# PoloWlg/Joint-Multimodal-Transformer-6th-ABAW

Measured on AMD Instinct MI355X. Metric: train windows/sec + CCC parity, B=64 T=300 A/V fusion, 1/2/4/8 MI355X, higher is better.
Workload: dtype bf16; 1 GPU; configs[2]: FcLayer(1024,512) + Two_transformers(TRANSFORMER,FC,H=1,L=1,vision_in_ft=2048) + 2x CCCLoss + SGD-nesterov; global_batch=64, per_gpu_batch=64, seq_len=300, D_a=1024, D_v=2048, parallelism=dp1

## Files before the change

### include/jmt.h

```cpp
#ifndef JMT_H_
#define JMT_H_

#include <stddef.h>
#include <stdint.h>

#ifdef __cplusplus
extern "C" {
#endif

#define JMT_ABI_VERSION 7

enum { JMT_F32 = 0, JMT_BF16 = 1, JMT_F16 = 2 };
enum { JMT_OK = 0, JMT_ERR_ARG = -1, JMT_ERR_HIP = -2, JMT_ERR_UNSUPPORTED = -3 };

int jmt_abi_version(void);
const char* jmt_last_error(void);
int jmt_kernel_count(void);
long long jmt_bounds_violations(int reset);

typedef struct jmt_gemm_desc {
  int ab_dtype, c_dtype, aux_dtype;
  int M, N, K;
  const void* a[8];
  const void* b[8];
// ... 65 lines not shown
                              void* stream);
int jmt_layernorm_bwd_grouped(int dt_in, int dt_dy, int dt_dx, int G, int64_t rows, int D,
                              const void* x, int64_t ldx, int64_t sx, const void* r, int64_t ldr,
                              int64_t sr, const void* dy, int64_t lddy, int64_t sdy,
                              const float* mean, const float* rstd, const float* const* gamma,
                              void* dx, int64_t lddx, int64_t sdx, float* const* dgamma,
                              float* const* dbeta, float* const* dsum, int beta_acc,
                              float* partials, void* stream);
int jmt_layernorm_bwd_grouped_blocks(int64_t rows);

int jmt_softmax_fwd(int p_dt, int64_t rows, int n, const float* s, int64_t lds, float scale,
                    void* p, int64_t ldp, void* stream);
int jmt_softmax_bwd(int p_dt, int ds_dt, int64_t rows, int n, const void* p, int64_t ldp,
                    const float* dp, int64_t lddp, float scale, void* ds, int64_t ldds,
                    void* stream);

int jmt_attn_supported(int dt, int dh);
int jmt_attn_fwd(int dt, int N, int H, int Lq, int Lk, int dh, const void* q, int64_t sq_l,
                 int64_t sq_n, const void* k, int64_t sk_l, int64_t sk_n, const void* v,
                 int64_t sv_l, int64_t sv_n, void* o, int64_t so_l, int64_t so_n, float scale,
                 float* lse, void* stream);
int jmt_attn_bwd(int dt, int N, int H, int Lq, int Lk, int dh, const void* go, int64_t sgo_l,
                 int64_t sgo_n, const void* o, int64_t so_l, int64_t so_n, const void* q,
                 int64_t sq_l, int64_t sq_n, const void* k, int64_t sk_l, int64_t sk_n,
                 const void* v, int64_t sv_l, int64_t sv_n, const float* lse, void* p_out,
                 void* ds_out, int64_t ldp, void* dq, int64_t sdq_l, int64_t sdq_n, float scale,
                 void* stream);

int jmt_attn_dkdv_plan(int Lq, int Lk, int H, int64_t sdk_l, int64_t sdv_l, int64_t sdq_l,
                       int has_dq);
int jmt_attn_dkdv(int dt, int N, int H, int Lq, int Lk, int dh, const void* p, const void* ds,
                  int64_t ldp, const void* go, int64_t sgo_l, int64_t sgo_n, const void* q,
                  int64_t sq_l, int64_t sq_n, const void* k, int64_t sk_l, int64_t sk_n, void* dk,
                  int64_t sdk_l, int64_t sdk_n, void* dv, int64_t sdv_l, int64_t sdv_n, void* dq,
                  int64_t sdq_l, int64_t sdq_n, void* stream);

int jmt_attn_fwd_sq(int dt, int N, int H, int Lq, int Lk, int dh, const void* q, int64_t sq_l,
                    int64_t sq_n, const void* k, int64_t sk_l, int64_t sk_n, const void* v,
                    int64_t sv_l, int64_t sv_n, void* o, int64_t so_l, int64_t so_n, float scale,
                    float* lse, int spp, const int* qtab, int npair, void* stream);
int jmt_attn_bwd_sq(int dt, int N, int H, int Lq, int Lk, int dh, const void* go, int64_t sgo_l,
                    int64_t sgo_n, const void* o, int64_t so_l, int64_t so_n, const void* q,
                    int64_t sq_l, int64_t sq_n, const void* k, int64_t sk_l, int64_t sk_n,
                    const void* v, int64_t sv_l, int64_t sv_n, const float* lse, void* p_out,
                    void* ds_out, int64_t ldp, float scale, int spp, const int* qtab, int npair,
                    void* stream);
int jmt_attn_dkdv_sq(int dt, int N, int H, int Lq, int Lk, int dh, const void* p, const void* ds,
                     int64_t ldp, const void* go, int64_t sgo_l, int64_t sgo_n, const void* q,
                     int64_t sq_l, int64_t sq_n, const void* k, int64_t sk_l, int64_t sk_n,
                     void* dk, int64_t sdk_l, int64_t sdk_n, void* dv, int64_t sdv_l,
                     int64_t sdv_n, void* dq, int64_t sdq_l, int64_t sdq_n, int spp,
                     const int* qtab, int npair, int merge_dq, void* stream);

int jmt_attn_fwd_rows_ok(int N, int H, int Lq, int Lk, int64_t sk_l, int64_t sv_l);
int jmt_attn_bwd_pds_ok(int N, int H, int Lq, int Lk, int64_t ldp, int64_t sk_l, int64_t sv_l);
int jmt_attn_dkdv_ok(int N, int H, int Lq, int Lk, int64_t ldp, int64_t sgo_l, int64_t sq_l,
                     int64_t sk_l, int64_t sdk_l, int64_t sdv_l, int64_t sdq_l, int has_dq);

int jmt_attn_short_supported(int dt, int dh, int Lq, int Lk);
int jmt_attn_short_fwd(int dt, int N, int H, int Lq, int Lk, int dh, const void* q, int64_t sq_l,
                       int64_t sq_n, const void* k, int64_t sk_l, int64_t sk_n, const void* v,
                       int64_t sv_l, int64_t sv_n, void* o, int64_t so_l, int64_t so_n,
                       float scale, float* lse, void* stream);
int jmt_attn_short_bwd(int dt, int N, int H, int Lq, int Lk, int dh, const void* go,
                       int64_t sgo_l, int64_t sgo_n, const void* o, int64_t so_l, int64_t so_n,
                       const void* q, int64_t sq_l, int64_t sq_n, const void* k, int64_t sk_l,
                       int64_t sk_n, const void* v, int64_t sv_l, int64_t sv_n, const float* lse,
                       void* dq, int64_t sdq_l, int64_t sdq_n, void* dk, int64_t sdk_l,
                       int64_t sdk_n, void* dv, int64_t sdv_l, int64_t sdv_n, float scale,
                       void* stream);

int jmt_small_attn_fwd(int dt, int N, int H, int Lq, int Lk, int E, const void* q, int64_t sq_l,
                       int64_t sq_n, const void* k, int64_t sk_l, int64_t sk_n, const void* v,
                       int64_t sv_l, int64_t sv_n, void* o, int64_t so_l, int64_t so_n,
                       float scale, float* p_out, void* stream);
int jmt_small_attn_bwd(int dt, int N, int H, int Lq, int Lk, int E, const void* go,
                       int64_t sgo_l, int64_t sgo_n, const void* q, int64_t sq_l, int64_t sq_n,
                       const void* k, int64_t sk_l, int64_t sk_n, const void* v, int64_t sv_l,
                       int64_t sv_n, const float* p, void* dq, int64_t sdq_l, int64_t sdq_n,
                       void* dk, int64_t sdk_l, int64_t sdk_n, void* dv, int64_t sdv_l,
                       int64_t sdv_n, float scale, void* stream);

int jmt_colsum_blocks(int64_t rows);
int jmt_colsum(int dt, int64_t rows, int N, const void* dy, int64_t ld, float* db, int beta_acc,
               float* partials, void* stream);
int jmt_colsum_grouped(int dt, int G, int64_t rows, int N, const void* dy, int64_t ld,
                       int64_t sdy, float* const* db_tab, int beta_acc, float* partials,
                       void* stream);

int jmt_noop(void* stream);

int jmt_copy2d(int src_dt, int dst_dt, int64_t rows, int64_t cols, const void* src,
               int64_t src_rs, int64_t src_cs, void* dst, int64_t dst_rs, int64_t dst_cs,
               int accumulate, void* stream);

int jmt_head_fwd(int h_dt, int y_dt, int64_t rows, int hid, int k, const void* h, int64_t ldh,
                 const void* w2_0, const void* w2_1, const float* b2_0, const float* b2_1,
                 void* y_0, void* y_1, int64_t ldy, void* stream);
int jmt_head_bwd(int h_dt, int gy_dt, int64_t rows, int hid, int k, const void* h, int64_t ldh,
                 const void* w2_0, const void* w2_1, const void* gy_0, const void* gy_1,
                 int64_t ldgy, void* dh, int64_t lddh, float* dw2_0, float* dw2_1, float* db2_0,
                 float* db2_1, float* partials, void* stream);
size_t jmt_head_bwd_workspace_bytes(int64_t rows);

int jmt_dropout_next(uint32_t* state, uint32_t* out, void* stream);
int jmt_dropout(int dt, const void* x, int64_t ldx, void* y, int64_t ldy, int64_t rows,
// ... 81 lines not shown
```

### joint-multimodal-transformer-6th-abaw_amd/csrc/abi_check.cpp

```cpp
#include <stdio.h>
#include <string.h>

#include "../../include/jmt.h"

static int g_fail = 0;

static void expect_msg(const char* what, const char* needle) {
  const char* e = jmt_last_error();
  if (!e || !strstr(e, needle)) {
    fprintf(stderr, "FAIL %s: err='%s' lacks '%s'\n", what, e ? e : "(null)", needle);
    ++g_fail;
  }
}

static void expect_err(const char* what, int rc) {
  const char* e = jmt_last_error();
  const size_t n = e ? strnlen(e, 1024) : 0;
  if (rc >= 0 || n == 0 || n >= 512) {
    fprintf(stderr, "FAIL %s: rc=%d err='%s'\n", what, rc, e ? e : "(null)");
    ++g_fail;
  }
}

static void expect_eq(const char* what, int got, int want) {
// ... 322 lines not shown
  }
  {
    const int id2[2] = {0, 1}, fwd[2] = {1, 1}, chain[3] = {0, 0, 1}, three[3] = {0, 0, 0};
    const int big[9] = {0, 1, 2, 3, 4, 5, 6, 7, 8};
    expect_err("attn_fwd_sq fp32", jmt_attn_fwd_sq(JMT_F32, 2, 1, 300, 300, 512, algn, 512, 512,
                                                   algn, 512, 512, algn, 512, 512, algn, 512, 512,
                                                   0.1f, fnull, 1, id2, 2, nullptr));
    expect_err("attn_fwd_sq Lq 64", jmt_attn_fwd_sq(JMT_BF16, 2, 1, 64, 300, 512, algn, 512, 512,
                                                    algn, 512, 512, algn, 512, 512, algn, 512,
                                                    512, 0.1f, fnull, 1, id2, 2, nullptr));
    expect_err("attn_fwd_sq null table", jmt_attn_fwd_sq(JMT_BF16, 2, 1, 300, 300, 512, algn, 512,
                                                         512, algn, 512, 512, algn, 512, 512,
                                                         algn, 512, 512, 0.1f, fnull, 1, nullptr,
                                                         2, nullptr));
    expect_err("attn_fwd_sq N != npair spp", jmt_attn_fwd_sq(JMT_BF16, 3, 1, 300, 300, 512, algn,
                                                             512, 512, algn, 512, 512, algn, 512,
                                                             512, algn, 512, 512, 0.1f, fnull, 1,
                                                             id2, 2, nullptr));
    expect_err("attn_fwd_sq 9 pairs", jmt_attn_fwd_sq(JMT_BF16, 9, 1, 300, 300, 512, algn, 512,
                                                      512, algn, 512, 512, algn, 512, 512, algn,
                                                      512, 512, 0.1f, fnull, 1, big, 9, nullptr));
    expect_err("attn_fwd_sq forward source", jmt_attn_fwd_sq(JMT_BF16, 2, 1, 300, 300, 512, algn,
                                                             512, 512, algn, 512, 512, algn, 512,
                                                             512, algn, 512, 512, 0.1f, fnull, 1,
                                                             fwd, 2, nullptr));
    expect_err("attn_bwd_sq chained source", jmt_attn_bwd_sq(JMT_BF16, 3, 1, 300, 300, 512, algn,
                                                             512, 512, algn, 512, 512, algn, 512,
                                                             512, algn, 512, 512, algn, 512, 512,
                                                             fnull, algn, algn, 384, 0.1f, 1,
                                                             chain, 3, nullptr));
    expect_err("attn_bwd_sq ldp", jmt_attn_bwd_sq(JMT_BF16, 2, 1, 300, 300, 512, algn, 512, 512,
                                                  algn, 512, 512, algn, 512, 512, algn, 512, 512,
                                                  algn, 512, 512, fnull, algn, algn, 300, 0.1f, 1,
                                                  id2, 2, nullptr));
    expect_err("attn_dkdv_sq dq null", jmt_attn_dkdv_sq(JMT_BF16, 2, 1, 300, 300, 512, algn, algn,
                                                        384, algn, 512, 512, algn, 512, 512, algn,
                                                        512, 512, algn, 512, 512, algn, 512, 512,
                                                        nullptr, 0, 0, 1, id2, 2, 0, nullptr));
    expect_err("attn_dkdv_sq spp 0", jmt_attn_dkdv_sq(JMT_BF16, 2, 1, 300, 300, 512, algn, algn,
                                                      384, algn, 512, 512, algn, 512, 512, algn,
                                                      512, 512, algn, 512, 512, algn, 512, 512,
                                                      algn, 512, 512, 0, id2, 2, 0, nullptr));
    expect_err("attn_dkdv_sq merge 3 uses", jmt_attn_dkdv_sq(JMT_BF16, 3, 1, 300, 300, 512, algn,
                                                             algn, 384, algn, 512, 512, algn, 512,
                                                             512, algn, 512, 512, algn, 512, 512,
                                                             algn, 512, 512, algn, 512, 512, 1,
                                                             three, 3, 1, nullptr));
    expect_err("attn_dkdv_sq merge 1 use", jmt_attn_dkdv_sq(JMT_BF16, 2, 1, 300, 300, 512, algn,
                                                            algn, 384, algn, 512, 512, algn, 512,
                                                            512, algn, 512, 512, algn, 512, 512,
                                                            algn, 512, 512, algn, 512, 512, 1, id2,
                                                            2, 1, nullptr));
  }
  expect_err("small_attn_fwd null", jmt_small_attn_fwd(JMT_BF16, 4, 1, 6, 6, 512, nullptr, 512,
                                                       512, nullptr, 512, 512, nullptr, 512, 512,
                                                       nullptr, 512, 512, 0.1f, fnull, nullptr));

  expect_err("ccc_stats kind", jmt_ccc_stats(3, JMT_F32, 10, 1, misal, fnull, 0.f, -1.f, 1.f,
                                             nullptr, nullptr));
  expect_err("ccc_stats bins", jmt_ccc_stats(0, JMT_F32, 10, 100, misal, fnull, 0.f, -1.f, 1.f,
                                             (double*)buf, nullptr));
  expect_err("ccc_finish null", jmt_ccc_finish(0, 0, nullptr, 1, 1e-8f, fnull, nullptr, nullptr));
  expect_err("ccc_finish_add null", jmt_ccc_finish_add(0, 1, nullptr, 1, 1e-8f, fnull, fnull,
                                                       nullptr, nullptr));
  expect_err("ce_stats bins", jmt_ce_stats(JMT_F32, 10, 1, misal, fnull, -1.f, 1.f, fnull,
                                           (double*)buf, nullptr));
  expect_err("ce_bwd null", jmt_ce_bwd(JMT_F32, 10, 5, nullptr, fnull, -1.f, 1.f, fnull, nullptr,
                                       fnull, nullptr, nullptr));
  expect_err("ce_labels null", jmt_ce_labels(10, 5, fnull, -1.f, 1.f, nullptr, nullptr));
  expect_err("mask_indices null", jmt_mask_indices(10, fnull, -5.f, nullptr, nullptr, nullptr));

  expect_err("sgd null", jmt_sgd_step(10, fnull, fnull, fnull, 0.1f, 0.9f, 0.f, 0.f, 1, 1, 1.f,
                                      nullptr, JMT_BF16, nullptr));
  expect_err("sgd_zero null", jmt_sgd_step_zero(10, fnull, nullptr, fnull, 0.1f, 0.9f, 0.f, 0.f,
                                                1, 1, 1.f, nullptr, JMT_BF16, nullptr));
  expect_err("sgd_amp_zero null", jmt_sgd_step_amp_zero(10, fnull, fnull, fnull, 0.1f, 0.9f,
                                                        0.f, 0.f, 1, 1, nullptr, nullptr,
                                                        JMT_BF16, nullptr));
  float* fal = (float*)algn;
  expect_err("opt_tick null state", jmt_opt_tick(nullptr, 0.9, 0.999, nullptr, nullptr));
  expect_msg("opt_tick null state", "null state");
  expect_err("opt_tick beta", jmt_opt_tick(fal, 1.0, 0.999, nullptr, nullptr));
  expect_err("adam null param", jmt_adam_step(10, fnull, fal, fal, fal, nullptr, fal, 0.9, 0.999,
                                              1e-8f, 0.f, 1.f, nullptr, 0, nullptr, JMT_BF16,
                                              nullptr));
  expect_msg("adam null param", "null pointer");
  expect_err("adam null moments", jmt_adam_step(10, fal, fal, fnull, fnull, nullptr, fal, 0.9,
                                                0.999, 1e-8f, 0.f, 1.f, nullptr, 0, nullptr,
                                                JMT_BF16, nullptr));
  expect_err("adam null state", jmt_adam_step(10, fal, fal, fal, fal, nullptr, nullptr, 0.9,
                                              0.999, 1e-8f, 0.f, 1.f, nullptr, 0, nullptr,
                                              JMT_BF16, nullptr));
  expect_msg("adam null state", "null state");
  expect_err("adam amsgrad null state", jmt_adam_step(10, fal, fal, fal, fal, fal, nullptr, 0.9,
                                                      0.999, 1e-8f, 0.f, 1.f, nullptr, 1, nullptr,
                                                      JMT_BF16, nullptr));
  expect_msg("adam amsgrad null state", "null state");
  expect_err("adam misaligned param", jmt_adam_step(10, (float*)(buf + 4), fal, fal, fal, nullptr,
                                                    fal, 0.9, 0.999, 1e-8f, 0.f, 1.f, nullptr, 0,
                                                    nullptr, JMT_BF16, nullptr));
  expect_msg("adam misaligned param", "16-B aligned");
  expect_err("adam shadow_dt", jmt_adam_step(10, fal, fal, fal, fal, nullptr, fal, 0.9, 0.999,
                                             1e-8f, 0.f, 1.f, nullptr, 0, algn, JMT_F32, nullptr));
  expect_msg("adam shadow_dt", "shadow_dt");
  expect_err("adam misaligned shadow", jmt_adam_step(10, fal, fal, fal, fal, nullptr, fal, 0.9,
                                                     0.999, 1e-8f, 0.f, 1.f, nullptr, 0,
// ... 124 lines not shown
```

### joint-multimodal-transformer-6th-abaw_amd/csrc/attn.hip

```cpp
#include "attn_common.h"

namespace jmt {

constexpr int AT_QT = 64;
constexpr int AF_KT = 64;
constexpr int AB_KT = 32;
constexpr int AT_XCH = 4096;
constexpr int AF_LDS = 2 * AF_KT * AT_ROWB + 8 * AT_XCH;
constexpr int AB_LDS = 4 * AB_KT * AT_ROWB + 8 * AT_XCH;

struct AttnFwdArgs {
  const void* q;
  const void* k;
  const void* v;
  void* o;
  float* lse;
  int64_t sq_l, sq_n, sk_l, sk_n, sv_l, sv_n, so_l, so_n;
  int Lq, Lk, H, nitems;
  float scale_log2;
  uint64_t* stamps;
  QShare qs;
};

template <bool STAMP>
__device__ __forceinline__ void stamp(uint64_t* buf, int idx) {
  if constexpr (STAMP) {
    if (buf && blockIdx.x == gridDim.x / 2 && ((threadIdx.x >> 6) & 3) == 0) {
      const uint64_t t = __builtin_amdgcn_s_memtime();
      buf[((threadIdx.x >> 8) * 256 + idx) * 64 + (threadIdx.x & 63)] = t;
    }
  }
}

template <typename T, bool STAMP = false, int OPT = 0>
__global__ __launch_bounds__(512, 2) void attn_fwd_kernel(AttnFwdArgs p) {
  typedef typename Frag16<T>::t F;
  typedef typename Frag16<T>::h Hf;
  extern __shared__ __attribute__((aligned(16))) char smem[];
  char* kimg = smem;
  char* vimg = smem + AF_KT * AT_ROWB;
  char* xch = smem + 2 * AF_KT * AT_ROWB;

  const int lane = threadIdx.x & 63, w = threadIdx.x >> 6;
  const int g = lane >> 4, li = lane & 15, rg = w & 3, h = w >> 2;
  const int nqt = (p.Lq + AT_QT - 1) / AT_QT;
  const int nkt = (p.Lk + AF_KT - 1) / AF_KT;
  int item, iend, istride;
  item_range(p.nitems, item, iend, istride);
  if (item >= iend) return;
  if constexpr ((OPT & 2) != 0)
    if (__builtin_amdgcn_readfirstlane(threadIdx.x >> 6) >= 4) __builtin_amdgcn_s_setprio(1);

  int nh = item / nqt, n = nh / p.H, hd = nh % p.H, q0 = (item % nqt) * AT_QT;
  const T* kb = (const T*)p.k + (int64_t)n * p.sk_n + hd * AT_DH;
  const T* vb = (const T*)p.v + (int64_t)n * p.sv_n + hd * AT_DH;

  F qf[8];
  auto load_q = [&](int n_, int hd_, int q0_) {
    const T* qrow = (const T*)p.q + (int64_t)n_ * p.sq_n + hd_ * AT_DH +
                    (int64_t)min(q0_ + 16 * rg + li, p.Lq - 1) * p.sq_l + 256 * h + 8 * g;
#pragma unroll
    for (int ks = 0; ks < 8; ++ks) qf[ks] = *(const F*)(qrow + 32 * ks);
  };
  load_q(n, hd, q0);
  stage_rows<T, AF_KT, 8, true>(kimg, kb, p.sk_l, 0, p.Lk);
  stage_rows<T, AF_KT, 8, true>(vimg, vb, p.sv_l, 0, p.Lk);

  f32x4* xmine = (f32x4*)(xch + w * AT_XCH) + lane;
  const f32x4* xpart = (const f32x4*)(xch + (w ^ 4) * AT_XCH) + lane;
  int kb4[4], tb8[8];
#pragma unroll
  for (int m = 0; m < 4; ++m) kb4[m] = row_base(m, li, g, h);
#pragma unroll
  for (int c = 0; c < 8; ++c) tb8[c] = tr_base(c, li, g, h);
// ... 382 lines not shown
          else *(uint2*)(prow_ds + key) = *(const uint2*)ds4;
        }
      }
      if constexpr ((OPT & 16) != 0) pend_on = true;
      {
        F fa[4], fb[4];
        auto kbatch = [&](F* dst, int b) {
#pragma unroll
          for (int i = 0; i < 4; ++i) {
            const int t = 4 * b + i;
            const char* a = kimg + tb8[t & 7] + 256 * (t >> 3);
            const Hf lo = tr_read<Hf>(a);
            const Hf hi = tr_read<Hf>(a + 16384);
            dst[i] = __builtin_shufflevector(lo, hi, 0, 1, 2, 3, 4, 5, 6, 7);
          }
        };
        kbatch(fa, 0);
#pragma unroll
        for (int b = 0; b < 4; b += 2) {
          kbatch(fb, b + 1);
          __builtin_amdgcn_sched_barrier(0);
#pragma unroll
          for (int i = 0; i < 4; ++i) acc[4 * b + i] = mfma16(fa[i], dsf, acc[4 * b + i]);
          __builtin_amdgcn_sched_barrier(0);
          if (b + 2 < 4) kbatch(fa, b + 2);
          __builtin_amdgcn_sched_barrier(0);
#pragma unroll
          for (int i = 0; i < 4; ++i) acc[4 * b + 4 + i] = mfma16(fb[i], dsf, acc[4 * b + 4 + i]);
          __builtin_amdgcn_sched_barrier(0);
        }
      }
      if (j + 1 < nkt) {
        wait_vmcnt<0>();
        lds_barrier();
      }
      buf ^= 1;
    }
    if constexpr ((OPT & 16) != 0) flush();
    store_acc_direct<T>(acc, 1.f,
                        (T*)p.dq + (int64_t)n * p.sdq_n + hd * AT_DH + (int64_t)qr * p.sdq_l +
                            256 * h,
                        qr < p.Lq);
    if (!more) break;
    load_o(n2, hd2, q02);
    lds_barrier();
    item = nxt; nh = nh2; n = n2; hd = hd2; q0 = q02; kb = kb2; vb = vb2;
  }
}

constexpr int AP_QT = 128;
constexpr int AP_KT = 32;
constexpr int AP_LDS = 4 * AP_KT * AT_ROWB;

template <typename T, int DBG = 0, bool SQ = false>
__global__ __launch_bounds__(512, 2) void attn_bwd_pds_kernel(AttnBwdArgs p) {
  int tcount = 0;
  auto st = [&](int phase) {
    if constexpr ((DBG & 64) != 0) {
      if (tcount < 31) stamp<true>((uint64_t*)p.dq, 8 * tcount + phase);
    }
  };
  typedef typename Frag16<T>::t F;
  typedef unsigned u32x4 __attribute__((ext_vector_type(4)));
  extern __shared__ __attribute__((aligned(16))) char smem[];
  constexpr int IMG = AP_KT * AT_ROWB;

  const int lane = threadIdx.x & 63, w = threadIdx.x >> 6;
  const int g = lane >> 4, li = lane & 15;
  const int nqt = (p.Lq + AP_QT - 1) / AP_QT;
  const int nkt = (p.Lk + AP_KT - 1) / AP_KT;
  int item, iend, istride;
  item_range(p.nitems, item, iend, istride);
  if (item >= iend) return;

  int nh = item / nqt, n = nh / p.H, hd = nh % p.H, q0 = (item % nqt) * AP_QT;
  const T* kb = (const T*)p.k + (int64_t)n * p.sk_n + hd * AT_DH;
  const T* vb = (const T*)p.v + (int64_t)n * p.sv_n + hd * AT_DH;

  F qf[16], df[16], of[16];
  auto load_qd = [&](int n_, int hd_, int q0_) {
    const int64_t qc_ = min(q0_ + 16 * w + li, p.Lq - 1), coff = (int64_t)hd_ * AT_DH + 8 * g;
    const T* qrow = (const T*)p.q + (int64_t)q_seq<SQ>(p.qs, n_) * p.sq_n + qc_ * p.sq_l + coff;
    const T* drow = (const T*)p.go + (int64_t)n_ * p.sgo_n + qc_ * p.sgo_l + coff;
#pragma unroll
    for (int ks = 0; ks < 16; ++ks) {
      qf[ks] = *(const F*)(qrow + 32 * ks);
      df[ks] = *(const F*)(drow + 32 * ks);
    }
  };
  auto load_o = [&](int n_, int hd_, int q0_) {
    const int64_t qc_ = min(q0_ + 16 * w + li, p.Lq - 1), coff = (int64_t)hd_ * AT_DH + 8 * g;
    const T* orow = (const T*)p.o + (int64_t)n_ * p.so_n + qc_ * p.so_l + coff;
#pragma unroll
    for (int ks = 0; ks < 16; ++ks) of[ks] = *(const F*)(orow + 32 * ks);
  };
  load_qd(n, hd, q0);
  load_o(n, hd, q0);
  int buf = 0;
  const int wu = __builtin_amdgcn_readfirstlane(w);
  const uint32_t lbase = (uint32_t)(uintptr_t)(__attribute__((address_space(3))) char*)smem;
  unsigned loff[4];
#pragma unroll
  for (int i = 0; i < 4; ++i) loff[i] = (unsigned)(lane ^ (((4 * wu + i) & 7) << 1)) << 4;
  const int ldk = (int)(p.sk_l * (int64_t)sizeof(T)), ldv = (int)(p.sv_l * (int64_t)sizeof(T));
  auto stage_tile = [&](int b, const T* kbase, const T* vbase, int k0) {
#pragma unroll
    for (int i = 0; i < 4; ++i) {
      const int r = 4 * wu + i;
      const int src = min(k0 + r, p.Lk - 1);
      const uint32_t dst = lbase + b * 2 * IMG + r * AT_ROWB;
      glds16_at((const char*)kbase + (unsigned)(src * ldk) + loff[i], dst);
      glds16_at((const char*)vbase + (unsigned)(src * ldv) + loff[i], dst + IMG);
    }
  };
  stage_tile(0, kb, vb, 0);

  int kb4[4];
#pragma unroll
  for (int m = 0; m < 4; ++m) kb4[m] = row_base(m, li, g, 0);

  while (true) {
    const int qr = q0 + 16 * w + li;
    const int qc = min(qr, p.Lq - 1);
    const bool wact = __builtin_amdgcn_readfirstlane(q0 + 16 * w) < p.Lq;
    const int nxt = item + istride;
    const bool more = nxt < iend;
    const int nh2 = nxt / nqt, n2 = nh2 / p.H, hd2 = nh2 % p.H, q02 = (nxt % nqt) * AP_QT;
    const T* kb2 = (const T*)p.k + (int64_t)n2 * p.sk_n + hd2 * AT_DH;
    const T* vb2 = (const T*)p.v + (int64_t)n2 * p.sv_n + hd2 * AT_DH;

    float delta;
    {
      float dp = 0.f;
#pragma unroll
      for (int ks = 0; ks < 16; ++ks)
#pragma unroll
        for (int e = 0; e < 8; ++e) dp += (float)of[ks][e] * (float)df[ks][e];
      delta = pl_pair_sum(dp);
    }
    const float lse2 = p.lse[(int64_t)nh * p.Lq + qc] * 1.4426950408889634f;
    const int64_t region = (int64_t)nh * p.Lq * p.ldp;
    const int nbytes = (int)((int64_t)p.Lq * p.ldp * (int64_t)sizeof(T));
    auto mk_rsrc = [&](void* base) {
      const uint64_t ba = (uint64_t)(uintptr_t)((T*)base + region);
      const uint32_t lo = __builtin_amdgcn_readfirstlane((uint32_t)ba);
      const uint32_t hi = __builtin_amdgcn_readfirstlane((uint32_t)(ba >> 32));
      return __builtin_amdgcn_make_buffer_rsrc((void*)(((uint64_t)hi << 32) | lo), 0,
                                               __builtin_amdgcn_readfirstlane(nbytes), 0x00020000);
    };
    const auto rs_p = mk_rsrc(p.pbuf);
    const auto rs_ds = mk_rsrc(p.dsbuf);
    const int rowoff = qr * AP_KT;

    wait_vmcnt<0>();
    lds_barrier();
    auto tile = [&](int j, auto last_c) {
      constexpr bool LAST = decltype(last_c)::value;
      st(0);
      const char* kimg = smem + buf * 2 * IMG;
      const char* vimg = kimg + IMG;
      if ((DBG & 8) == 0 && (!LAST || more))
        stage_tile(buf ^ 1, LAST ? kb2 : kb, LAST ? vb2 : vb, LAST ? 0 : AP_KT * (j + 1));
      st(1);
      f32x4 s[2], d[2];
#pragma unroll
      for (int kt = 0; kt < 2; ++kt) {
        s[kt] = f32x4{0.f, 0.f, 0.f, 0.f};
        d[kt] = f32x4{0.f, 0.f, 0.f, 0.f};
      }
      if ((DBG & 2) == 0 && wact) {
        F fa[4], fb[4];
        auto batch = [&](F* dst, int ks) {
#pragma unroll
          for (int kt = 0; kt < 2; ++kt) {
            const int o = kb4[ks & 3] + 256 * (ks >> 2) + 16384 * kt;
            dst[kt] = *(const F*)(kimg + o);
            dst[2 + kt] = *(const F*)(vimg + o);
          }
        };
        batch(fa, 0);
#pragma unroll
        for (int ks = 0; ks < 16; ks += 2) {
          batch(fb, ks + 1);
          __builtin_amdgcn_sched_barrier(0);
#pragma unroll
          for (int kt = 0; kt < 2; ++kt) {
            s[kt] = mfma16(fa[kt], qf[ks], s[kt]);
            d[kt] = mfma16(fa[2 + kt], df[ks], d[kt]);
          }
          __builtin_amdgcn_sched_barrier(0);
          if (ks + 2 < 16) batch(fa, ks + 2);
          __builtin_amdgcn_sched_barrier(0);
#pragma unroll
          for (int kt = 0; kt < 2; ++kt) {
            s[kt] = mfma16(fb[kt], qf[ks + 1], s[kt]);
            d[kt] = mfma16(fb[2 + kt], df[ks + 1], d[kt]);
          }
          __builtin_amdgcn_sched_barrier(0);
        }
      }
      st(2);
      if constexpr (LAST && (DBG & 1) == 0) {
        if (more) load_qd(n2, hd2, q02);
      }
      if ((DBG & 4) == 0 && wact) {
        const int kbase = AP_KT * j + 4 * g;
        uint32_t pk[2][2][2];
#pragma unroll
        for (int kt = 0; kt < 2; ++kt) {
          T pv4[4], ds4[4];
#pragma unroll
          for (int r = 0; r < 4; ++r) {
            const bool in = kbase + 16 * kt + r < p.Lk;
            const float pv = in ? __builtin_amdgcn_exp2f(s[kt][r] * p.scale_log2 - lse2) : 0.f;
            pv4[r] = from_f<T>(pv);
            ds4[r] = from_f<T>(p.scale * pv * (d[kt][r] - delta));
          }
#pragma unroll
          for (int q = 0; q < 2; ++q) {
            pk[0][kt][q] = ((const uint32_t*)pv4)[q];
            pk[1][kt][q] = ((const uint32_t*)ds4)[q];
          }
        }
        const int off = qr < p.Lq ? (rowoff + j * p.Lq * AP_KT + 16 * (g & 1) + 8 * (g >> 1)) *
                                        (int)sizeof(T)
                                  : 0x7ffffff0;
        JMT_DCHECK(AP_KT * j + AP_KT <= p.ldp);
#pragma unroll
        for (int a = 0; a < 2; ++a) {
          const auto r0 = __builtin_amdgcn_permlane16_swap(pk[a][0][0], pk[a][1][0], false, false);
          const auto r1 = __builtin_amdgcn_permlane16_swap(pk[a][0][1], pk[a][1][1], false, false);
          const u32x4 v = {r0[0], r1[0], r0[1], r1[1]};
          if constexpr ((DBG & 16) != 0) {
            asm volatile("" ::"v"(v[0]), "v"(v[1]), "v"(v[2]), "v"(v[3]));
          } else {
            __builtin_amdgcn_raw_buffer_store_b128(v, a == 0 ? rs_p : rs_ds, off, 0,
                                                   (DBG & 32) ? 2 : 0);
          }
        }
      }
      st(3);
      if constexpr (!LAST) {
        if ((DBG & 20) == 0 && wact) wait_vmcnt<2>();
        else wait_vmcnt<0>();
        st(4);
        lds_barrier();
        st(5);
      }
      ++tcount;
      buf ^= 1;
    };
    for (int j = 0; j + 1 < nkt; ++j) tile(j, std::false_type{});
    tile(nkt - 1, std::true_type{});
    if (!more) break;
    if constexpr ((DBG & 1) == 0) load_o(n2, hd2, q02);
    item = nxt; nh = nh2; n = n2; hd = hd2; q0 = q02; kb = kb2; vb = vb2;
  }
}

constexpr int AR_QT = 128;
constexpr int AR_KT = 32;
constexpr int AR_LDS = 4 * AR_KT * AT_ROWB;
constexpr int AR_VB = 4;

template <typename T, int DBG = 0, bool SQ = false>
__global__ __launch_bounds__(512, 2) void attn_fwd_rows_kernel(AttnFwdArgs p) {
  typedef typename Frag16<T>::t F;
  typedef typename Frag16<T>::h Hf;
  extern __shared__ __attribute__((aligned(16))) char smem[];
  constexpr int IMG = AR_KT * AT_ROWB;

  const int lane = threadIdx.x & 63, w = threadIdx.x >> 6;
  const int g = lane >> 4, li = lane & 15;
  const int nqt = (p.Lq + AR_QT - 1) / AR_QT;
  const int nkt = (p.Lk + AR_KT - 1) / AR_KT;
  int item, iend, istride;
  item_range(p.nitems, item, iend, istride);
  if (item >= iend) return;

  int nh = item / nqt, n = nh / p.H, hd = nh % p.H, q0 = (item % nqt) * AR_QT;
  const T* kb = (const T*)p.k + (int64_t)n * p.sk_n + hd * AT_DH;
  const T* vb = (const T*)p.v + (int64_t)n * p.sv_n + hd * AT_DH;

  F qf[16];
  auto load_q = [&](int n_, int hd_, int q0_) {
    const T* qrow = (const T*)p.q + (int64_t)q_seq<SQ>(p.qs, n_) * p.sq_n + hd_ * AT_DH +
                    (int64_t)min(q0_ + 16 * w + li, p.Lq - 1) * p.sq_l + 8 * g;
#pragma unroll
    for (int ks = 0; ks < 16; ++ks) qf[ks] = *(const F*)(qrow + 32 * ks);
  };
  load_q(n, hd, q0);
  int buf = 0;
  const int wu = __builtin_amdgcn_readfirstlane(w);
  const uint32_t lbase = (uint32_t)(uintptr_t)(__attribute__((address_space(3))) char*)smem;
  unsigned loff[4];
#pragma unroll
  for (int i = 0; i < 4; ++i) loff[i] = (unsigned)(lane ^ (((4 * wu + i) & 7) << 1)) << 4;
  const int ldk = (int)(p.sk_l * (int64_t)sizeof(T)), ldv = (int)(p.sv_l * (int64_t)sizeof(T));
  auto stage_tile = [&](int b, const T* kbase, const T* vbase, int k0) {
#pragma unroll
    for (int i = 0; i < 4; ++i) {
      const int r = 4 * wu + i;
      const int src = min(k0 + r, p.Lk - 1);
      JMT_DCHECK(src >= 0 && src < p.Lk);
      const uint32_t dst = lbase + b * 2 * IMG + r * AT_ROWB;
      glds16_sv((const char*)kbase + (unsigned)(src * ldk), loff[i], dst);
      glds16_sv((const char*)vbase + (unsigned)(src * ldv), loff[i], dst + IMG);
    }
  };
  stage_tile(0, kb, vb, 0);
  const int kb0 = row_base(0, li, g, 0), tb0 = tr_base(0, li, g, 0);
  auto lane_base = [](int base, int bits) __attribute__((always_inline)) {
#if !defined(__OPTIMIZE__)
    return base ^ bits;
#else
    int r;
    asm volatile("v_xor_b32 %0, %2, %1" : "=v"(r) : "v"(base), "i"(bits));
    return r;
#endif
  };

  while (true) {
    const int qr = q0 + 16 * w + li;
    const bool wact = __builtin_amdgcn_readfirstlane(q0 + 16 * w) < p.Lq;
    const int nxt = item + istride;
    const bool more = nxt < iend;
    const int nh2 = nxt / nqt, n2 = nh2 / p.H, hd2 = nh2 % p.H, q02 = (nxt % nqt) * AR_QT;
    const T* kb2 = (const T*)p.k + (int64_t)n2 * p.sk_n + hd2 * AT_DH;
    const T* vb2 = (const T*)p.v + (int64_t)n2 * p.sv_n + hd2 * AT_DH;

    f32x4 o[32];
#pragma unroll
    for (int t = 0; t < 32; ++t) o[t] = f32x4{0.f, 0.f, 0.f, 0.f};
    float m_run = -INFINITY, l_run = 0.f;

    wait_vmcnt<0>();
#pragma unroll
    for (int ks = 0; ks < 16; ++ks) asm volatile("" : "+v"(qf[ks]));
    lds_barrier();
    auto tile = [&](int j, auto last_c) {
      constexpr bool LAST = decltype(last_c)::value;
      const char* kimg = smem + buf * 2 * IMG;
      const char* vimg = kimg + IMG;
      if ((!LAST && (DBG & 8) == 0) || (LAST && more))
        stage_tile(buf ^ 1, LAST ? kb2 : kb, LAST ? vb2 : vb, LAST ? 0 : AR_KT * (j + 1));
      f32x4 sl[2], sh[2];
#pragma unroll
      for (int kt = 0; kt < 2; ++kt) {
        sl[kt] = f32x4{0.f, 0.f, 0.f, 0.f};
        sh[kt] = f32x4{0.f, 0.f, 0.f, 0.f};
      }
      if ((DBG & 2) == 0 && wact) {
        F fa[2], fb[2];
        auto batch = [&](F* dst, const char* a) {
#pragma unroll
          for (int kt = 0; kt < 2; ++kt) dst[kt] = *(const F*)(a + 16384 * kt);
        };
        const char* a = kimg + lane_base(kb0, 0);
        batch(fa, a);
#pragma unroll
        for (int ks = 0; ks < 8; ++ks) {
          batch(fb, a + 512);
          __builtin_amdgcn_sched_barrier(0);
#pragma unroll
          for (int kt = 0; kt < 2; ++kt) sl[kt] = mfma16(fa[kt], qf[ks], sl[kt]);
          __builtin_amdgcn_sched_barrier(0);
          if (ks + 1 < 8) {
            a = kimg + lane_base(kb0, ((ks + 1) & 3) << 6) + 256 * ((ks + 1) >> 2);
            batch(fa, a);
          }
          __builtin_amdgcn_sched_barrier(0);
#pragma unroll
          for (int kt = 0; kt < 2; ++kt) sh[kt] = mfma16(fb[kt], qf[ks + 8], sh[kt]);
          __builtin_amdgcn_sched_barrier(0);
        }
      }
      if constexpr (LAST) {
        if (more) load_q(n2, hd2, q02);
      }
      if (wact) {
        F pf;
        if constexpr ((DBG & 4) != 0) {
#pragma unroll
          for (int e = 0; e < 8; ++e) pf[e] = from_f<T>(0.f);
#pragma unroll
          for (int kt = 0; kt < 2; ++kt)
            asm volatile("" ::"v"(sl[kt][0]), "v"(sl[kt][3]), "v"(sh[kt][0]), "v"(sh[kt][3]));
        } else {
        const int kbase = AR_KT * j + 4 * g;
        float mx = -INFINITY;
#pragma unroll
        for (int kt = 0; kt < 2; ++kt) {
          const f32x4 full = sl[kt] + sh[kt];
#pragma unroll
          for (int r = 0; r < 4; ++r) {
            const float x = (kbase + 16 * kt + r < p.Lk) ? full[r] * p.scale_log2 : -INFINITY;
// ... 124 lines not shown
    if (hipGetDevice(&dev) != hipSuccess ||
        hipDeviceGetAttribute(&v, hipDeviceAttributeMultiprocessorCount, dev) != hipSuccess || v < 8)
      v = 8;
    ncu = v / 8 * 8;
    const char* e = getenv("JMT_ATTN_PERSIST");
    if (e && e[0] == '0') ncu = 1 << 30;
  }
  return (unsigned)(nitems > ncu ? ncu : nitems);
}

extern "C" int jmt_attn_set_stamps(void* buf) {
#if JMT_DIAG
  g_stamps = buf;
  return JMT_OK;
#else
  return buf ? set_error(JMT_ERR_UNSUPPORTED, "jmt_attn_set_stamps: diagnostic build only "
                                              "(make diag)") : JMT_OK;
#endif
}

static int g_fwd_rows = -1;
static bool fwd_rows_on() {
  static const bool env_on = [] {
    const char* e = getenv("JMT_ATTN_FWD_ROWS");
    return !(e && e[0] == '0');
  }();
  return g_fwd_rows < 0 ? env_on : g_fwd_rows != 0;
}
extern "C" int jmt_attn_set_fwd_rows(int on) {
  g_fwd_rows = on < 0 ? -1 : (on != 0);
  return JMT_OK;
}

extern "C" int jmt_attn_supported(int dt, int dh) {
  return (dt == JMT_BF16 || dt == JMT_F16) && dh == AT_DH;
}

static bool fwd_rows(int Lq, int Lk, int64_t sk_l, int64_t sv_l) {
  return fwd_rows_on() && Lq > AT_QT && rows_fit(Lk, sk_l) && rows_fit(Lk, sv_l);
}

extern "C" int jmt_attn_fwd_rows_ok(int N, int H, int Lq, int Lk, int64_t sk_l, int64_t sv_l) {
  return fwd_rows(Lq, Lk, sk_l, sv_l) && sizes_ok(N, H, Lq, Lk, AR_QT);
}

extern "C" int jmt_attn_bwd_pds_ok(int N, int H, int Lq, int Lk, int64_t ldp, int64_t sk_l,
                                   int64_t sv_l) {
  return pds_range(N, H, Lq, Lk, ldp, sk_l, sv_l) == nullptr;
}

static int attn_fwd_impl(int dt, int N, int H, int Lq, int Lk, int dh, const void* q,
                         int64_t sq_l, int64_t sq_n, const void* k, int64_t sk_l, int64_t sk_n,
                         const void* v, int64_t sv_l, int64_t sv_n, void* o, int64_t so_l,
                         int64_t so_n, float scale, float* lse, const QShare* qs, void* stream) {
  if (N == 0 || Lq == 0) return JMT_OK;
  if (!jmt_attn_supported(dt, dh))
    return set_error(JMT_ERR_UNSUPPORTED, "jmt_attn_fwd: dtype %d / head dim %d not supported",
                     dt, dh);
  const void* ptrs[] = {q, k, v, o};
  const int64_t strides[] = {sq_l, sq_n, sk_l, sk_n, sv_l, sv_n, so_l, so_n};
  const bool rows = fwd_rows(Lq, Lk, sk_l, sv_l);
  if (qs && !rows)
    return set_error(JMT_ERR_UNSUPPORTED, "jmt_attn_fwd_sq: the whole-row kernel only (Lq > %d, "
                                          "Lk K / V rows below 2 GiB, JMT_ATTN_FWD_ROWS on)",
                     AT_QT);
  const int qt = rows ? AR_QT : AT_QT;
  int rc = check_common("jmt_attn_fwd", N, H, Lq, Lk, qt, ptrs, 4, strides, 8);
  if (rc != JMT_OK) return rc;
  AttnFwdArgs a = {};
  if (qs) a.qs = *qs;
  a.q = q; a.k = k; a.v = v; a.o = o; a.lse = lse;
  a.sq_l = sq_l; a.sq_n = sq_n; a.sk_l = sk_l; a.sk_n = sk_n; a.sv_l = sv_l; a.sv_n = sv_n;
  a.so_l = so_l; a.so_n = so_n;
  a.Lq = Lq; a.Lk = Lk; a.H = H;
  a.scale_log2 = scale * 1.4426950408889634f;
  hipStream_t st = as_stream(stream);
  a.nitems = ((Lq + qt - 1) / qt) * N * H;
  const dim3 grid(persistent_grid(a.nitems));
  const char* name = qs ? "jmt_attn_fwd_sq" : "jmt_attn_fwd";
#if JMT_DIAG
  static const int dbg =
      getenv("JMT_ATTN_FWD_ROWS_DBG") ? atoi(getenv("JMT_ATTN_FWD_ROWS_DBG")) : 0;
  if (rows && dbg && dt == JMT_BF16) {
#define JMT_ROWS_DBG(D) \
  case D: attn_launch<attn_fwd_rows_kernel<__bf16, D>, AR_LDS>(grid, st, a); break;
    switch (dbg) {
      JMT_ROWS_DBG(2) JMT_ROWS_DBG(4) JMT_ROWS_DBG(8) JMT_ROWS_DBG(16) JMT_ROWS_DBG(32)
      JMT_ROWS_DBG(18) JMT_ROWS_DBG(22) JMT_ROWS_DBG(54) JMT_ROWS_DBG(62)
      default: return set_error(JMT_ERR_ARG, "JMT_ATTN_FWD_ROWS_DBG=%d not built", dbg);
    }
#undef JMT_ROWS_DBG
    JMT_LAUNCH_CHECK("jmt_attn_fwd");
    return JMT_OK;
  }
  if (!rows && g_stamps && dt == JMT_BF16) {
    a.stamps = (uint64_t*)g_stamps;
    attn_launch<attn_fwd_kernel<__bf16, true, ATTN_FWD_OPT>, AF_LDS>(grid, st, a);
    JMT_LAUNCH_CHECK("jmt_attn_fwd");
    return JMT_OK;
  }
#endif
  by_elem(dt, [&](auto e) {
    using T = typename decltype(e)::type;
    if (!rows) attn_launch<attn_fwd_kernel<T, false, ATTN_FWD_OPT>, AF_LDS>(grid, st, a);
    else if (qs) attn_launch<attn_fwd_rows_kernel<T, 0, true>, AR_LDS>(grid, st, a);
    else attn_launch<attn_fwd_rows_kernel<T>, AR_LDS>(grid, st, a);
  });
  JMT_LAUNCH_CHECK(name);
  return JMT_OK;
}

extern "C" int jmt_attn_fwd(int dt, int N, int H, int Lq, int Lk, int dh, const void* q,
                            int64_t sq_l, int64_t sq_n, const void* k, int64_t sk_l, int64_t sk_n,
                            const void* v, int64_t sv_l, int64_t sv_n, void* o, int64_t so_l,
                            int64_t so_n, float scale, float* lse, void* stream) {
  return attn_fwd_impl(dt, N, H, Lq, Lk, dh, q, sq_l, sq_n, k, sk_l, sk_n, v, sv_l, sv_n, o, so_l,
                       so_n, scale, lse, nullptr, stream);
}

extern "C" int jmt_attn_fwd_sq(int dt, int N, int H, int Lq, int Lk, int dh, const void* q,
                               int64_t sq_l, int64_t sq_n, const void* k, int64_t sk_l,
                               int64_t sk_n, const void* v, int64_t sv_l, int64_t sv_n, void* o,
                               int64_t so_l, int64_t so_n, float scale, float* lse, int spp,
                               const int* qtab, int npair, void* stream) {
  if (N == 0 || Lq == 0) return JMT_OK;
  if (!jmt_attn_supported(dt, dh))
    return set_error(JMT_ERR_UNSUPPORTED, "jmt_attn_fwd_sq: dtype %d / head dim %d not supported",
                     dt, dh);
  QShare qs = {};
  int rc = qshare_pack("jmt_attn_fwd_sq", N, spp, qtab, npair, &qs);
  if (rc != JMT_OK) return rc;
  return attn_fwd_impl(dt, N, H, Lq, Lk, dh, q, sq_l, sq_n, k, sk_l, sk_n, v, sv_l, sv_n, o, so_l,
                       so_n, scale, lse, &qs, stream);
}

static int attn_bwd_impl(int dt, int N, int H, int Lq, int Lk, int dh, const void* go,
                         int64_t sgo_l, int64_t sgo_n, const void* o, int64_t so_l, int64_t so_n,
                         const void* q, int64_t sq_l, int64_t sq_n, const void* k, int64_t sk_l,
                         int64_t sk_n, const void* v, int64_t sv_l, int64_t sv_n,
                         const float* lse, void* p_out, void* ds_out, int64_t ldp, void* dq,
                         int64_t sdq_l, int64_t sdq_n, float scale, const QShare* qs,
                         void* stream) {
  if (N == 0 || Lq == 0) return JMT_OK;
  if (!jmt_attn_supported(dt, dh))
    return set_error(JMT_ERR_UNSUPPORTED, "jmt_attn_bwd: dtype %d / head dim %d not supported",
                     dt, dh);
  const void* ptrs[] = {go, o, q, k, v, p_out, ds_out, dq};
  const int64_t strides[] = {sgo_l, sgo_n, so_l, so_n, sq_l, sq_n, sk_l, sk_n, sv_l, sv_n, ldp,
                             sdq_l, sdq_n};
  const bool pds = dq == nullptr;
  const int qt = pds ? AP_QT : AT_QT;
  int rc = check_common("jmt_attn_bwd", N, H, Lq, Lk, qt, ptrs, pds ? 7 : 8, strides,
                        pds ? 11 : 13);
  if (rc != JMT_OK) return rc;
  JMT_CHECK_ARG(lse && ldp >= Lk, "jmt_attn_bwd: lse missing or ldp < Lk");
  if (pds) {
    const char* why = pds_range(N, H, Lq, Lk, ldp, sk_l, sv_l);
    JMT_CHECK_ARG(!why, "jmt_attn_bwd (dq = NULL): %s", why);
  }
  AttnBwdArgs a = {};
  if (qs) a.qs = *qs;
  a.go = go; a.o = o; a.q = q; a.k = k; a.v = v; a.lse = lse;
  a.pbuf = p_out; a.dsbuf = ds_out; a.dq = dq;
  a.sgo_l = sgo_l; a.sgo_n = sgo_n; a.so_l = so_l; a.so_n = so_n; a.sq_l = sq_l; a.sq_n = sq_n;
  a.sk_l = sk_l; a.sk_n = sk_n; a.sv_l = sv_l; a.sv_n = sv_n;
  if (!pds) { a.sdq_l = sdq_l; a.sdq_n = sdq_n; }
  a.ldp = ldp;
  a.Lq = Lq; a.Lk = Lk; a.H = H;
  a.scale = scale;
  a.scale_log2 = scale * 1.4426950408889634f;
  a.nitems = ((Lq + qt - 1) / qt) * N * H;
  const dim3 grid(persistent_grid(a.nitems));
  hipStream_t st = as_stream(stream);
  const char* name = qs ? "jmt_attn_bwd_sq" : "jmt_attn_bwd";
#if JMT_DIAG
  static const int dbg = getenv("JMT_ATTN_PDS_DBG") ? atoi(getenv("JMT_ATTN_PDS_DBG")) : 0;
  if (pds && dbg && dt == JMT_BF16) {
    if (dbg & 64) a.dq = g_stamps;
#define JMT_PDS_DBG(D) \
  case D: attn_launch<attn_bwd_pds_kernel<__bf16, D>, AP_LDS>(grid, st, a); break;
    switch (dbg) {
      JMT_PDS_DBG(1) JMT_PDS_DBG(2) JMT_PDS_DBG(3) JMT_PDS_DBG(4) JMT_PDS_DBG(6)
      JMT_PDS_DBG(7) JMT_PDS_DBG(8) JMT_PDS_DBG(15) JMT_PDS_DBG(16) JMT_PDS_DBG(32)
      JMT_PDS_DBG(17) JMT_PDS_DBG(18) JMT_PDS_DBG(64)
      default: return set_error(JMT_ERR_ARG, "JMT_ATTN_PDS_DBG=%d not built", dbg);
    }
#undef JMT_PDS_DBG
    JMT_LAUNCH_CHECK("jmt_attn_bwd");
    return JMT_OK;
  }
#endif
  by_elem(dt, [&](auto e) {
    using T = typename decltype(e)::type;
    if (!pds) attn_launch<attn_bwd_kernel<T, ATTN_BWD_OPT>, AB_LDS>(grid, st, a);
    else if (qs) attn_launch<attn_bwd_pds_kernel<T, 0, true>, AP_LDS>(grid, st, a);
    else attn_launch<attn_bwd_pds_kernel<T>, AP_LDS>(grid, st, a);
  });
  JMT_LAUNCH_CHECK(name);
  return JMT_OK;
}

extern "C" int jmt_attn_bwd(int dt, int N, int H, int Lq, int Lk, int dh, const void* go,
                            int64_t sgo_l, int64_t sgo_n, const void* o, int64_t so_l,
                            int64_t so_n, const void* q, int64_t sq_l, int64_t sq_n,
                            const void* k, int64_t sk_l, int64_t sk_n, const void* v,
                            int64_t sv_l, int64_t sv_n, const float* lse, void* p_out,
                            void* ds_out, int64_t ldp, void* dq, int64_t sdq_l, int64_t sdq_n,
                            float scale, void* stream) {
  return attn_bwd_impl(dt, N, H, Lq, Lk, dh, go, sgo_l, sgo_n, o, so_l, so_n, q, sq_l, sq_n, k,
                       sk_l, sk_n, v, sv_l, sv_n, lse, p_out, ds_out, ldp, dq, sdq_l, sdq_n, scale,
                       nullptr, stream);
}

extern "C" int jmt_attn_bwd_sq(int dt, int N, int H, int Lq, int Lk, int dh, const void* go,
                               int64_t sgo_l, int64_t sgo_n, const void* o, int64_t so_l,
                               int64_t so_n, const void* q, int64_t sq_l, int64_t sq_n,
                               const void* k, int64_t sk_l, int64_t sk_n, const void* v,
                               int64_t sv_l, int64_t sv_n, const float* lse, void* p_out,
                               void* ds_out, int64_t ldp, float scale, int spp, const int* qtab,
                               int npair, void* stream) {
  if (N == 0 || Lq == 0) return JMT_OK;
  if (!jmt_attn_supported(dt, dh))
    return set_error(JMT_ERR_UNSUPPORTED, "jmt_attn_bwd_sq: dtype %d / head dim %d not supported",
                     dt, dh);
  QShare qs = {};
  int rc = qshare_pack("jmt_attn_bwd_sq", N, spp, qtab, npair, &qs);
  if (rc != JMT_OK) return rc;
  return attn_bwd_impl(dt, N, H, Lq, Lk, dh, go, sgo_l, sgo_n, o, so_l, so_n, q, sq_l, sq_n, k,
                       sk_l, sk_n, v, sv_l, sv_n, lse, p_out, ds_out, ldp, nullptr, 0, 0, scale,
                       &qs, stream);
}
```

### joint-multimodal-transformer-6th-abaw_amd/csrc/attn_common.h

```cpp
#pragma once
#include "common.h"

namespace jmt {

constexpr int AT_DH = 512;
constexpr int AT_ROWB = 1024;

struct QShare {
  int spp;
  uint32_t tab;
};
template <bool SQ>
__device__ __forceinline__ int q_seq(const QShare& s, int n) {
  if constexpr (!SQ) return n;
  const int p = n / s.spp;
  return (int)((s.tab >> (4 * p)) & 15u) * s.spp + (n - p * s.spp);
}

static inline int qshare_pack(const char* name, int N, int spp, const int* tab, int npair,
                              QShare* out) {
  JMT_CHECK_ARG(tab != nullptr && spp > 0 && npair >= 1 && npair <= 8 &&
                    (int64_t)spp * npair == N,
                "%s: query table needs 1-8 pairs of spp sequences with npair * spp == N", name);
  uint32_t bits = 0;
  for (int p = 0; p < npair; ++p) {
    JMT_CHECK_ARG(tab[p] >= 0 && tab[p] <= p && tab[tab[p]] == tab[p],
                  "%s: query table entry %d (%d) is not an earlier first use", name, p, tab[p]);
    bits |= (uint32_t)tab[p] << (4 * p);
  }
  out->spp = spp;
  out->tab = bits;
  return JMT_OK;
}

template <auto K, int LDS, int BLOCK = 512, typename A>
static void attn_launch(dim3 grid, hipStream_t st, const A& a) {
  static bool once = ((void)hipFuncSetAttribute((const void*)K,
                                                hipFuncAttributeMaxDynamicSharedMemorySize, LDS),
                      true);
  (void)once;
  hipLaunchKernelGGL(K, grid, dim3(BLOCK), (size_t)LDS, st, a);
}
template <typename T>
struct Elem {
  using type = T;
};
template <typename F>
static void by_elem(int dt, F f) {
  if (dt == JMT_BF16) f(Elem<__bf16>{});
  else f(Elem<_Float16>{});
}

struct AttnBwdArgs {
  const void* go;
  const void* o;
  const void* q;
  const void* k;
  const void* v;
  const float* lse;
  void* pbuf;
  void* dsbuf;
  void* dq;
  int64_t sgo_l, sgo_n, so_l, so_n, sq_l, sq_n, sk_l, sk_n, sv_l, sv_n, sdq_l, sdq_n, ldp;
  int Lq, Lk, H, nitems;
  float scale, scale_log2;
  QShare qs;
};

__device__ __forceinline__ int img_off(int row, int b) {
  return row * AT_ROWB + ((((b >> 4) ^ ((row & 7) << 1))) << 4) + (b & 15);
}
__device__ __forceinline__ int row_base(int m, int li, int g, int h) {
  return li * AT_ROWB + ((((4 * m + g) ^ ((li & 7) << 1))) << 4) + 512 * h;
}
__device__ __forceinline__ int tr_base(int c, int li, int g, int h) {
  const int r = 4 * g + (li >> 2);
  return r * AT_ROWB + ((((2 * c + ((li & 3) >> 1)) ^ ((r & 7) << 1))) << 4) + 8 * (li & 1) +
         512 * h;
}

__device__ __forceinline__ void lds_barrier() {
  asm volatile("s_waitcnt lgkmcnt(0)" ::: "memory");
  __builtin_amdgcn_s_barrier();
}

template <typename T, int R, int NW = 8, bool ASM = false>
__device__ __forceinline__ void stage_rows(char* img, const T* base, int64_t ld, int k0, int Lk) {
  constexpr int NI = R / NW;
  const int lane = threadIdx.x & 63;
  const int wu = __builtin_amdgcn_readfirstlane(threadIdx.x >> 6);
#pragma unroll
  for (int i = 0; i < NI; ++i) {
    const int r = wu * NI + i;
    const int src = min(k0 + r, Lk - 1);
    JMT_DCHECK(src >= 0 && src < Lk);
    const char* row = (const char*)(base + (int64_t)src * ld);
    const unsigned off = (unsigned)(lane ^ ((r & 7) << 1)) << 4;
    if constexpr (ASM) glds16_asm(row + off, img + r * AT_ROWB);
    else glds16(row + off, img + r * AT_ROWB);
  }
}

template <typename T, int R, int NW = 8, bool ASM = false>
__device__ __forceinline__ void stage_rows_part(char* img, const T* base, int64_t ld, int k0,
                                                int Lk, int i0, int i1) {
  constexpr int NI = R / NW;
  const int lane = threadIdx.x & 63;
  const int wu = __builtin_amdgcn_readfirstlane(threadIdx.x >> 6);
#pragma unroll
  for (int i = 0; i < NI; ++i) {
    if (i < i0 || i >= i1) continue;
    const int r = wu * NI + i;
    const int src = min(k0 + r, Lk - 1);
    JMT_DCHECK(src >= 0 && src < Lk);
    const char* row = (const char*)(base + (int64_t)src * ld);
    const unsigned off = (unsigned)(lane ^ ((r & 7) << 1)) << 4;
    if constexpr (ASM) glds16_asm(row + off, img + r * AT_ROWB);
    else glds16(row + off, img + r * AT_ROWB);
  }
// ... 68 lines not shown
```

### joint-multimodal-transformer-6th-abaw_amd/csrc/attn_dkdv.hip

```cpp
#include "attn_common.h"

namespace jmt {

constexpr int DK_QC = 32;
constexpr int DK_IMG = DK_QC * AT_ROWB;
#ifndef JMT_DKDV_NS
#define JMT_DKDV_NS 4
#endif

template <int NKG>
struct DkGeo {
  static constexpr int KT = 16 * NKG;
  static constexpr int PROW = 2 * KT;
  static constexpr int PIMG = DK_QC * PROW;
  static constexpr int STAGE = DK_IMG + PIMG;
  static constexpr int NS = NKG == 8 ? JMT_DKDV_NS : 3;
  static constexpr int LDS = NS * STAGE;
  static constexpr int NPD = (PIMG / 1024 + 7) / 8;
  static constexpr int PLANES = PIMG / 16 / 8 / NPD;
  static constexpr int NDMA = DK_QC / 8 + NPD;
  static constexpr int NST = 2 * NKG;
  static_assert(NKG == 8 || NKG == 10, "128- or 160-row items");
  static_assert(NS >= 2 && NS <= 4, "2-4 stages (the wait table covers 0-2 later stages)");
  static_assert(LDS <= 160 * 1024, "stages exceed the LDS");
  static_assert(8 * NPD * PLANES * 16 == PIMG && PLANES <= 64, "P / dS DMA split");
  static_assert((NS - 2) * NDMA + (NS - 1) * NST < 64, "vmcnt range");
};

struct AttnDkdvArgs {
  const void* p;
  const void* ds;
  const void* go;
  const void* q;
  const void* k;
  void* dk;
  void* dv;
  void* dq;
  int64_t ldp, sgo_l, sgo_n, sq_l, sq_n, sk_l, sk_n, sdk_l, sdk_n, sdv_l, sdv_n, sdq_l, sdq_n;
  int Lq, Lk, H, nkt, nqd, ipn, nitems;
  QShare qs;
  int mrg;
  uint32_t mg_first, mg_second;
};

__device__ __forceinline__ int pimg_off(int r, int c) {
  return r * DkGeo<8>::PROW + ((c ^ ((r & 7) << 1)) << 4);
}

__device__ __forceinline__ int simg_off(int r, int c) {
  return r * 64 + ((c ^ ((r >> 1) & 2)) << 4);
}

__device__ __forceinline__ int qimg_off(int r, int c) {
  return r * 64 + ((c ^ ((r >> 2) & 3)) << 4);
}

struct DkItem {
  int nh, n, hd, role, k0, nch, nch1, n2, nh2;
};
template <int KT, bool SQ>
__device__ __forceinline__ DkItem dk_decode(const AttnDkdvArgs& a, int it) {
  DkItem d;
  if (SQ && a.mrg) {
    const int gi = it / a.ipn;
    int r = it - gi * a.ipn;
    const int sb = gi / a.H;
    d.hd = gi - sb * a.H;
    const int u = sb / a.qs.spp, b = sb - u * a.qs.spp;
    const int n1 = (int)((a.mg_first >> (4 * u)) & 15u) * a.qs.spp + b;
    const int n2 = (int)((a.mg_second >> (4 * u)) & 15u) * a.qs.spp + b;
    if (r < a.nqd) {
      d.role = 2;
      d.k0 = r * KT;
      d.nch1 = (a.Lk + DK_QC - 1) / DK_QC;
      d.nch = 2 * d.nch1;
      d.n = n1;
      d.n2 = n2;
    } else {
      r -= a.nqd;
      const int second = r >= 2 * a.nkt;
      r -= second * 2 * a.nkt;
      d.role = r >= a.nkt;
      d.k0 = (r - d.role * a.nkt) * KT;
      d.nch = d.nch1 = (a.Lq + DK_QC - 1) / DK_QC;
      d.n = d.n2 = second ? n2 : n1;
    }
    d.nh = d.n * a.H + d.hd;
    d.nh2 = d.n2 * a.H + d.hd;
    return d;
  }
  d.nh = it / a.ipn;
  const int r = it - d.nh * a.ipn;
  if (r < 2 * a.nkt) {
    d.role = r >= a.nkt;
    d.k0 = (r - d.role * a.nkt) * KT;
    d.nch = (a.Lq + DK_QC - 1) / DK_QC;
  } else {
    d.role = 2;
    d.k0 = (r - 2 * a.nkt) * KT;
    d.nch = (a.Lk + DK_QC - 1) / DK_QC;
  }
  d.n = d.nh / a.H;
  d.hd = d.nh - d.n * a.H;
  d.nch1 = d.nch;
  d.n2 = d.n;
  d.nh2 = d.nh;
  return d;
}

template <typename T, bool SQ>
__device__ __forceinline__ void dkdv_stage(char* st, const AttnDkdvArgs& a, const DkItem& d,
                                           int c) {
  const int lane = threadIdx.x & 63;
  const int wu = __builtin_amdgcn_readfirstlane(threadIdx.x >> 6);
  const bool second = SQ && c >= d.nch1;
  const int q0 = DK_QC * (second ? c - d.nch1 : c);
  if (d.role == 2) {
    const int sn = second ? d.n2 : d.n, snh = second ? d.nh2 : d.nh;
    const char* kb = (const char*)((const T*)a.k + (int64_t)sn * a.sk_n + d.hd * AT_DH);
    const int ldk = (int)(a.sk_l * (int64_t)sizeof(T));
#pragma unroll
    for (int i = 0; i < DK_QC / 8; ++i) {
      const int r = wu * (DK_QC / 8) + i;
      const int src = min(q0 + r, a.Lk - 1);
      const unsigned off = (unsigned)(lane ^ ((r & 7) << 1)) << 4;
      glds16_asm(kb + (unsigned)(src * ldk) + off, st + r * AT_ROWB);
    }
    const int r = 16 * wu + (lane >> 2);
    const int lc = (lane & 3) ^ ((r >> 2) & 3);
    const int src_row = min(d.k0 + r, a.Lq - 1);
    JMT_DCHECK(src_row >= 0 && q0 + 8 * lc + 8 <= a.ldp);
    const char* pb = (const char*)((const T*)a.ds + (int64_t)snh * a.Lq * a.ldp);
    glds16_asm(pb + (unsigned)(((q0 >> 5) * a.Lq + src_row) * 64) + 16 * lc,
               st + DK_IMG + wu * 1024);
    return;
  }
  const char* rb;
  int ldb;
  if (d.role == 0) {
    rb = (const char*)((const T*)a.go + (int64_t)d.n * a.sgo_n + d.hd * AT_DH);
    ldb = (int)(a.sgo_l * (int64_t)sizeof(T));
  } else {
    rb = (const char*)((const T*)a.q + (int64_t)q_seq<SQ>(a.qs, d.n) * a.sq_n + d.hd * AT_DH);
    ldb = (int)(a.sq_l * (int64_t)sizeof(T));
  }
#pragma unroll
  for (int i = 0; i < DK_QC / 8; ++i) {
    const int r = wu * (DK_QC / 8) + i;
    const int src = min(q0 + r, a.Lq - 1);
    const unsigned off = (unsigned)(lane ^ ((r & 7) << 1)) << 4;
    glds16_asm(rb + (unsigned)(src * ldb) + off, st + r * AT_ROWB);
  }
  const int r = 4 * wu + (lane >> 4);
  const int cs = (lane & 15) ^ ((r & 7) << 1);
  const int src_row = min(q0 + r, a.Lq - 1);
  JMT_DCHECK(src_row >= 0 && d.k0 + 8 * cs + 8 <= a.ldp);
  if (a.dq) {
    const char* pb = (const char*)((const T*)(d.role == 0 ? a.p : a.ds) +
                                   (int64_t)d.nh * a.Lq * a.ldp);
    glds16_asm(pb + (unsigned)((((d.k0 >> 5) + (cs >> 2)) * a.Lq + src_row) * 64) +
                   16 * (cs & 3),
               st + DK_IMG + wu * 1024);
    return;
  }
  const char* pb = (const char*)((const T*)(d.role == 0 ? a.p : a.ds) +
                                 (int64_t)d.nh * a.Lq * a.ldp + d.k0);
  glds16_asm(pb + (unsigned)(src_row * (int)(a.ldp * sizeof(T))) + 16 * cs,
             st + DK_IMG + wu * 1024);
}

template <typename T, bool SQ>
__device__ __forceinline__ void dkdv_stage160(uint32_t st, const AttnDkdvArgs& a, const DkItem& d,
                                              int ch) {
  typedef DkGeo<10> G;
  const int lane = threadIdx.x & 63;
  const int wu = __builtin_amdgcn_readfirstlane(threadIdx.x >> 6);
  const bool second = SQ && ch >= d.nch1;
  const int q0 = DK_QC * (second ? ch - d.nch1 : ch);
  const int snh = second ? d.nh2 : d.nh;
  const char* rb;
  int ldb, clen;
  if (d.role == 0) {
    rb = (const char*)((const T*)a.go + (int64_t)d.n * a.sgo_n + d.hd * AT_DH);
    ldb = (int)(a.sgo_l * (int64_t)sizeof(T));
    clen = a.Lq;
  } else if (d.role == 1) {
    rb = (const char*)((const T*)a.q + (int64_t)q_seq<SQ>(a.qs, d.n) * a.sq_n + d.hd * AT_DH);
    ldb = (int)(a.sq_l * (int64_t)sizeof(T));
    clen = a.Lq;
  } else {
    rb = (const char*)((const T*)a.k + (int64_t)(second ? d.n2 : d.n) * a.sk_n + d.hd * AT_DH);
    ldb = (int)(a.sk_l * (int64_t)sizeof(T));
    clen = a.Lk;
  }
#pragma unroll
  for (int i = 0; i < DK_QC / 8; ++i) {
    const int r = wu * (DK_QC / 8) + i;
    const int src = min(q0 + r, clen - 1);
    JMT_DCHECK(src >= 0 && src < clen);
    const unsigned off = (unsigned)(lane ^ ((r & 7) << 1)) << 4;
    glds16_sv(rb + (unsigned)(src * ldb), off, st + r * AT_ROWB);
  }
  const char* pb = (const char*)((const T*)(d.role == 0 ? a.p : a.ds) +
                                 (int64_t)snh * a.Lq * a.ldp);
  const int ntile = (int)(a.ldp >> 5);
  if (lane < G::PLANES) {
#pragma unroll
    for (int j = 0; j < G::NPD; ++j) {
      const int b0 = (wu * G::NPD + j) * (16 * G::PLANES);
      const int b = b0 + 16 * lane;
      const int pc = (b >> 4) & 3;
      int tile, row, c;
      if (d.role == 2) {
        const int r = b >> 6;
        c = pc ^ ((r >> 2) & 3);
        tile = q0 >> 5;
        row = min(d.k0 + r, a.Lq - 1);
      } else {
        const int r = (b >> 6) & 31;
        c = pc ^ ((r >> 1) & 2);
        tile = min((d.k0 >> 5) + (b >> 11), ntile - 1);
        row = min(q0 + r, a.Lq - 1);
      }
      JMT_DCHECK(row >= 0 && tile >= 0 && tile < ntile);
      glds16_sv(pb, (unsigned)((tile * a.Lq + row) * 64 + 16 * c), st + DK_IMG + b0);
    }
  }
}

template <int NKG, int S>
__device__ __forceinline__ void dkdv_wait_s(int stores) {
  typedef DkGeo<NKG> G;
  if constexpr (S <= G::NS - 2) {
    if (stores == 0) wait_vmcnt<S * G::NDMA>();
    else if (stores == 1 || G::NS == 2) wait_vmcnt<S * G::NDMA + G::NST>();
    else if constexpr (G::NS >= 3) {
      if (stores == 2 || G::NS == 3) wait_vmcnt<S * G::NDMA + 2 * G::NST>();
      else if constexpr (G::NS >= 4) wait_vmcnt<S * G::NDMA + 3 * G::NST>();
    }
  } else {
    wait_vmcnt<0>();
  }
}
template <int NKG>
__device__ __forceinline__ void dkdv_wait(int stages, int stores) {
  if (stages == 0) dkdv_wait_s<NKG, 0>(stores);
  else if (stages == 1) dkdv_wait_s<NKG, 1>(stores);
  else dkdv_wait_s<NKG, 2>(stores);
}

#define DK_NO_MERGE() asm volatile("" ::: "memory")

template <typename T, int NKG, bool SQ>
__global__ __launch_bounds__(512, 2) void attn_dkdv_kernel(AttnDkdvArgs a) {
  typedef typename Frag16<T>::t F;
  typedef typename Frag16<T>::h Hf;
  typedef unsigned u32x4 __attribute__((ext_vector_type(4)));
  typedef DkGeo<NKG> G;
  constexpr int KT = G::KT, NS = G::NS, STAGE = G::STAGE;
  constexpr int KB = NKG == 8 ? 8 : 5;
  extern __shared__ __attribute__((aligned(16))) char smem[];
  const int lane = threadIdx.x & 63, w = threadIdx.x >> 6;
  const int g = lane >> 4, li = lane & 15;
  int item, iend, istride;
  item_range(a.nitems, item, iend, istride);
  if (item >= iend) return;

  int tb[NKG == 8 ? 4 : 1], pb[NKG == 8 ? 8 : 1];
  if constexpr (NKG == 8) {
#pragma unroll
    for (int t = 0; t < 4; ++t) tb[t] = tr_base(4 * (w & 1) + t, li, g, 0) + 256 * (w >> 1);
#pragma unroll
    for (int kg = 0; kg < 8; ++kg)
      pb[kg] = pimg_off(4 * g + (li >> 2), 2 * kg + ((li & 3) >> 1)) + 8 * (li & 1);
  } else {
    tb[0] = tr_base(4 * (w & 1), li, g, 0) + 256 * (w >> 1);
    pb[0] = simg_off(4 * g + (li >> 2), (li & 3) >> 1) + 8 * (li & 1);
  }
  auto lane_base = [](int base, int bits) __attribute__((always_inline)) {
#if !defined(__OPTIMIZE__)
    return base ^ bits;
#else
    int r;
    asm volatile("v_xor_b32 %0, %2, %1" : "=v"(r) : "v"(base), "i"(bits));
    return r;
#endif
  };
  const int qb0 = qimg_off(li, g >> 1) + 8 * (g & 1);
  const int qb1 = NKG == 8 ? qimg_off(li, 2 + (g >> 1)) + 8 * (g & 1) : 0;
  const uint32_t lbase = (uint32_t)(uintptr_t)(__attribute__((address_space(3))) char*)smem;

  int is_item = item, is_c = 0;
  DkItem is_d = dk_decode<KT, SQ>(a, item);
  bool is_ok = true;
  int is_buf = 0;
  unsigned after = 0;
  int inflight = 0;
  auto issue = [&]() {
    if (is_ok) {
      if constexpr (NKG == 8) dkdv_stage<T, SQ>(smem + is_buf * STAGE, a, is_d, is_c);
      else dkdv_stage160<T, SQ>(lbase + is_buf * STAGE, a, is_d, is_c);
      after &= ~(15u << (4 * is_buf));
      ++inflight;
      if (++is_c == is_d.nch) {
        is_c = 0;
        is_item += istride;
        is_ok = is_item < iend;
        if (is_ok) is_d = dk_decode<KT, SQ>(a, is_item);
      }
    }
    is_buf = is_buf == NS - 1 ? 0 : is_buf + 1;
  };
  for (int i = 0; i < NS - 1; ++i) issue();
  int buf = 0;

  while (true) {
    const DkItem d = dk_decode<KT, SQ>(a, item);
    const bool more = item + istride < iend;
    f32x4 acc[NKG][4];
#pragma unroll
    for (int kg = 0; kg < NKG; ++kg)
#pragma unroll
      for (int t = 0; t < 4; ++t) acc[kg][t] = f32x4{0.f, 0.f, 0.f, 0.f};

    for (int c = 0; c < d.nch; ++c) {
      const char* cur = smem + buf * STAGE;
      dkdv_wait<NKG>(inflight - 1, (after >> (4 * buf)) & 15);
      --inflight;
      lds_barrier();
      issue();
      const int c0 = DK_QC * (SQ && c >= d.nch1 ? c - d.nch1 : c);
      const int clen = d.role == 2 ? a.Lk : a.Lq;
      F df[4];
#pragma unroll
      for (int k0 = 0; k0 < NKG; k0 += KB) {
        F kf[KB];
        if (d.role != 2) {
#pragma unroll
          for (int j = 0; j < KB; ++j) {
            const int kg = k0 + j;
            const char* pa;
            if constexpr (NKG == 8) pa = cur + DK_IMG + pb[kg];
            else pa = cur + DK_IMG + lane_base(pb[0], (kg & 1) << 5) + 2048 * (kg >> 1);
            const Hf lo = tr_read<Hf>(pa);
            const Hf hi = tr_read<Hf>(pa + (NKG == 8 ? 16 * G::PROW : 16 * 64));
            kf[j] = __builtin_shufflevector(lo, hi, 0, 1, 2, 3, 4, 5, 6, 7);
          }
        } else {
          const char* qa0 = cur + DK_IMG + qb0;
          const char* qa1;
          if constexpr (NKG == 8) qa1 = cur + DK_IMG + qb1;
          else qa1 = cur + DK_IMG + lane_base(qb0, 32);
#pragma unroll
          for (int j = 0; j < KB; ++j) {
            const Hf lo = *(const Hf*)(qa0 + 1024 * (k0 + j));
            DK_NO_MERGE();
            const Hf hi = *(const Hf*)(qa1 + 1024 * (k0 + j));
            DK_NO_MERGE();
            kf[j] = __builtin_shufflevector(lo, hi, 0, 1, 2, 3, 4, 5, 6, 7);
          }
        }
        if (c0 + DK_QC > clen) {
#pragma unroll
          for (int e = 0; e < 8; ++e) {
            const bool in = c0 + 16 * (e >> 2) + 4 * g + (e & 3) < clen;
#pragma unroll
            for (int j = 0; j < KB; ++j) kf[j][e] = in ? kf[j][e] : from_f<T>(0.f);
          }
        }
        if (k0 == 0) {
// ... 68 lines not shown
  }
  return nitems > ncu ? ncu : nitems;
}

static int64_t dkdv_cost(int Lq, int Lk, int KT) {
  const auto cdiv = [](int x, int d) { return ((int64_t)x + d - 1) / d; };
  return (2 * cdiv(Lk, KT) * cdiv(Lq, DK_QC) + cdiv(Lq, KT) * cdiv(Lk, DK_QC)) * KT;
}

static int g_dkdv_tile = -1;
static int dkdv_tile_pref() {
  static const int env = [] {
    const char* e = getenv("JMT_ATTN_DKDV_KT");
    const int v = e ? atoi(e) : 0;
    return v == 128 || v == 160 ? v : 0;
  }();
  return g_dkdv_tile < 0 ? env : g_dkdv_tile;
}

static int dkdv_plan(int Lq, int Lk, int64_t sdk_l, int64_t sdv_l, int64_t sdq_l, bool has_dq) {
  constexpr int64_t KT = DkGeo<10>::KT;
  if (!has_dq || Lq <= 0 || Lk <= 0 || KT * sdk_l * 2 >= (1LL << 31) ||
      KT * sdv_l * 2 >= (1LL << 31) || KT * sdq_l * 2 >= (1LL << 31))
    return 128;
  const int pref = dkdv_tile_pref();
  if (pref) return pref;
  return dkdv_cost(Lq, Lk, 160) < dkdv_cost(Lq, Lk, 128) ? 160 : 128;
}

static const char* dkdv_range(int N, int H, int Lq, int Lk, int64_t ldp, int64_t sgo_l,
                              int64_t sq_l, int64_t sk_l, int64_t sdk_l, int64_t sdv_l,
                              int64_t sdq_l, bool has_dq) {
  constexpr int64_t DK_KT = DkGeo<8>::KT;
  constexpr int64_t LIM = 1LL << 31;
  if (!(N > 0 && H > 0 && Lq > 0 && Lk > 0)) return "bad sizes";
  if (ldp < (Lk + DK_KT - 1) / DK_KT * DK_KT) return "ldp must cover 128-key tiles";
  if (sdk_l < H * AT_DH || sdv_l < H * AT_DH || DK_KT * sdk_l * 2 >= LIM ||
      DK_KT * sdv_l * 2 >= LIM)
    return "dK / dV row stride out of range";
  if (has_dq) {
    if (sdq_l < H * AT_DH || DK_KT * sdq_l * 2 >= LIM || Lk * sk_l * 2 >= LIM)
      return "dQ / K row stride out of range";
    if (ldp % 32 != 0) return "tile-major P / dS need ldp % 32 == 0";
  }
  const int kt = dkdv_plan(Lq, Lk, sdk_l, sdv_l, has_dq ? sdq_l : 0, has_dq);
  const int nkt = (Lk + kt - 1) / kt;
  const int nqd = has_dq ? (Lq + kt - 1) / kt : 0;
  if ((int64_t)N * H * (2 * nkt + nqd) >= LIM) return "too many items";
  if (Lq * sgo_l * 2 >= LIM || Lq * sq_l * 2 >= LIM || Lq * ldp * 2 >= LIM)
    return "Lq rows of dO / Q / P exceed 2 GiB";
  return nullptr;
}

template <typename T, int NKG, bool SQ>
static void dkdv_launch_sq(const AttnDkdvArgs& a, int grid, hipStream_t st) {
  constexpr int lds = DkGeo<NKG>::LDS;
  static bool once = ((void)hipFuncSetAttribute((const void*)attn_dkdv_kernel<T, NKG, SQ>,
                                                hipFuncAttributeMaxDynamicSharedMemorySize, lds),
                      true);
  (void)once;
  hipLaunchKernelGGL((attn_dkdv_kernel<T, NKG, SQ>), dim3(grid), dim3(512), (size_t)lds, st, a);
}
template <typename T, int NKG>
static void dkdv_launch(const AttnDkdvArgs& a, int grid, hipStream_t st, bool sq) {
  if (sq) dkdv_launch_sq<T, NKG, true>(a, grid, st);
  else dkdv_launch_sq<T, NKG, false>(a, grid, st);
}

}

using namespace jmt;

extern "C" int jmt_attn_dkdv_set_tile(int kt) {
  if (!(kt < 0 || kt == 0 || kt == 128 || kt == 160))
    return set_error(JMT_ERR_ARG, "jmt_attn_dkdv_set_tile: %d is not 0, 128 or 160", kt);
  g_dkdv_tile = kt < 0 ? -1 : kt;
  return JMT_OK;
}

extern "C" int jmt_attn_dkdv_plan(int Lq, int Lk, int H, int64_t sdk_l, int64_t sdv_l,
                                  int64_t sdq_l, int has_dq) {
  (void)H;
  return dkdv_plan(Lq, Lk, sdk_l, sdv_l, sdq_l, has_dq != 0);
}

extern "C" int jmt_attn_dkdv_ok(int N, int H, int Lq, int Lk, int64_t ldp, int64_t sgo_l,
                                int64_t sq_l, int64_t sk_l, int64_t sdk_l, int64_t sdv_l,
                                int64_t sdq_l, int has_dq) {
  return dkdv_range(N, H, Lq, Lk, ldp, sgo_l, sq_l, sk_l, sdk_l, sdv_l, sdq_l, has_dq != 0) ==
         nullptr;
}

static int dkdv_impl(int dt, int N, int H, int Lq, int Lk, int dh, const void* p, const void* ds,
                     int64_t ldp, const void* go, int64_t sgo_l, int64_t sgo_n, const void* q,
                     int64_t sq_l, int64_t sq_n, const void* k, int64_t sk_l, int64_t sk_n,
                     void* dk, int64_t sdk_l, int64_t sdk_n, void* dv, int64_t sdv_l,
                     int64_t sdv_n, void* dq, int64_t sdq_l, int64_t sdq_n, const QShare* qs,
                     const int* qtab, int npair, int merge, void* stream) {
  if (N == 0 || Lk == 0) return JMT_OK;
  if (!((dt == JMT_BF16 || dt == JMT_F16) && dh == AT_DH))
    return set_error(JMT_ERR_UNSUPPORTED, "jmt_attn_dkdv: dtype %d / head dim %d not supported",
                     dt, dh);
  const void* ptrs[] = {p, ds, go, q, dk, dv};
  for (int i = 0; i < 6; ++i)
    JMT_CHECK_ARG(ptrs[i] != nullptr && ((uintptr_t)ptrs[i] & 15) == 0,
                  "jmt_attn_dkdv: operand %d null or not 16-B aligned", i);
  const int64_t strides[] = {ldp, sgo_l, sgo_n, sq_l, sq_n, sdk_l, sdk_n, sdv_l, sdv_n};
  for (int i = 0; i < 9; ++i)
    JMT_CHECK_ARG(strides[i] % 8 == 0, "jmt_attn_dkdv: stride %d not a multiple of 8", i);
  if (dq)
    JMT_CHECK_ARG(k != nullptr && ((uintptr_t)k & 15) == 0 && ((uintptr_t)dq & 15) == 0 &&
                      sk_l % 8 == 0 && sk_n % 8 == 0 && sdq_l % 8 == 0 && sdq_n % 8 == 0,
                  "jmt_attn_dkdv: k / dq null, misaligned or strides not multiples of 8");
  const char* why = dkdv_range(N, H, Lq, Lk, ldp, sgo_l, sq_l, sk_l, sdk_l, sdv_l, sdq_l,
                               dq != nullptr);
  JMT_CHECK_ARG(!why, "jmt_attn_dkdv: %s", why);
  const int kt = dkdv_plan(Lq, Lk, sdk_l, sdv_l, dq ? sdq_l : 0, dq != nullptr);
  const int nkt = (Lk + kt - 1) / kt;
  const int nqd = dq ? (Lq + kt - 1) / kt : 0;
  AttnDkdvArgs a = {};
  if (qs) a.qs = *qs;
  a.p = p; a.ds = ds; a.go = go; a.q = q; a.k = k; a.dk = dk; a.dv = dv; a.dq = dq;
  a.ldp = ldp; a.sgo_l = sgo_l; a.sgo_n = sgo_n; a.sq_l = sq_l; a.sq_n = sq_n;
  a.sk_l = sk_l; a.sk_n = sk_n;
  a.sdk_l = sdk_l; a.sdk_n = sdk_n; a.sdv_l = sdv_l; a.sdv_n = sdv_n;
  a.sdq_l = sdq_l; a.sdq_n = sdq_n;
  a.Lq = Lq; a.Lk = Lk; a.H = H; a.nkt = nkt; a.nqd = nqd; a.ipn = 2 * nkt + nqd;
  a.nitems = N * H * a.ipn;
  if (merge) {
    int ng = 0;
    for (int f = 0; f < npair; ++f) {
      if (qtab[f] != f) continue;
      int second = -1, uses = 0;
      for (int j = 0; j < npair; ++j)
        if (j != f && qtab[j] == f) { second = j; ++uses; }
      if (uses != 1)
        return set_error(JMT_ERR_UNSUPPORTED, "jmt_attn_dkdv_sq: merged dQ needs every query "
                                              "used exactly twice (pair %d: %d more uses)",
                         f, uses);
      a.mg_first |= (uint32_t)f << (4 * ng);
      a.mg_second |= (uint32_t)second << (4 * ng);
      ++ng;
    }
    a.mrg = 1;
    a.ipn = nqd + 4 * nkt;
    a.nitems = ng * a.qs.spp * H * a.ipn;
  }
  const int grid = dkdv_grid(a.nitems);
  hipStream_t st = as_stream(stream);
  if (kt == 160) {
    if (dt == JMT_BF16) dkdv_launch<__bf16, 10>(a, grid, st, qs != nullptr);
    else dkdv_launch<_Float16, 10>(a, grid, st, qs != nullptr);
  } else {
    if (dt == JMT_BF16) dkdv_launch<__bf16, 8>(a, grid, st, qs != nullptr);
    else dkdv_launch<_Float16, 8>(a, grid, st, qs != nullptr);
  }
  JMT_LAUNCH_CHECK("jmt_attn_dkdv");
  return JMT_OK;
}

extern "C" int jmt_attn_dkdv(int dt, int N, int H, int Lq, int Lk, int dh, const void* p,
                             const void* ds, int64_t ldp, const void* go, int64_t sgo_l,
                             int64_t sgo_n, const void* q, int64_t sq_l, int64_t sq_n,
                             const void* k, int64_t sk_l, int64_t sk_n, void* dk, int64_t sdk_l,
                             int64_t sdk_n, void* dv, int64_t sdv_l, int64_t sdv_n, void* dq,
                             int64_t sdq_l, int64_t sdq_n, void* stream) {
  return dkdv_impl(dt, N, H, Lq, Lk, dh, p, ds, ldp, go, sgo_l, sgo_n, q, sq_l, sq_n, k, sk_l,
                   sk_n, dk, sdk_l, sdk_n, dv, sdv_l, sdv_n, dq, sdq_l, sdq_n, nullptr, nullptr,
                   0, 0, stream);
}

extern "C" int jmt_attn_dkdv_sq(int dt, int N, int H, int Lq, int Lk, int dh, const void* p,
                                const void* ds, int64_t ldp, const void* go, int64_t sgo_l,
                                int64_t sgo_n, const void* q, int64_t sq_l, int64_t sq_n,
                                const void* k, int64_t sk_l, int64_t sk_n, void* dk,
                                int64_t sdk_l, int64_t sdk_n, void* dv, int64_t sdv_l,
                                int64_t sdv_n, void* dq, int64_t sdq_l, int64_t sdq_n, int spp,
                                const int* qtab, int npair, int merge_dq, void* stream) {
  if (N == 0 || Lk == 0) return JMT_OK;
  if (!((dt == JMT_BF16 || dt == JMT_F16) && dh == AT_DH))
    return set_error(JMT_ERR_UNSUPPORTED,
                     "jmt_attn_dkdv_sq: dtype %d / head dim %d not supported", dt, dh);
  if (dq == nullptr)
    return set_error(JMT_ERR_UNSUPPORTED, "jmt_attn_dkdv_sq: the tile-major form only (dq != "
                                          "NULL: P / dS from jmt_attn_bwd_sq)");
  QShare qs = {};
  int rc = qshare_pack("jmt_attn_dkdv_sq", N, spp, qtab, npair, &qs);
  if (rc != JMT_OK) return rc;
  return dkdv_impl(dt, N, H, Lq, Lk, dh, p, ds, ldp, go, sgo_l, sgo_n, q, sq_l, sq_n, k, sk_l,
                   sk_n, dk, sdk_l, sdk_n, dv, sdv_l, sdv_n, dq, sdq_l, sdq_n, &qs, qtab, npair,
                   merge_dq != 0, stream);
}
```

### joint-multimodal-transformer-6th-abaw_amd/jmt/_lib.py

```python
from __future__ import annotations

import ctypes as C
import os

_HERE = os.path.dirname(os.path.abspath(__file__))
LIB_PATH = os.environ.get("JMT_LIB") or os.path.join(_HERE, "libjmt_hip.so")

F32, BF16, F16 = 0, 1, 2
OK, ERR_ARG, ERR_HIP, ERR_UNSUPPORTED = 0, -1, -2, -3

c_i64 = C.c_int64
c_vp = C.c_void_p
c_int = C.c_int
c_f = C.c_float
c_fp = C.POINTER(C.c_float)


class GemmDesc(C.Structure):
    _fields_ = [
        ("ab_dtype", c_int), ("c_dtype", c_int), ("aux_dtype", c_int),
        ("M", c_int), ("N", c_int), ("K", c_int),
        ("a", c_vp * 8), ("b", c_vp * 8), ("c", c_vp * 8),
        ("n_a", c_int), ("n_b", c_int), ("n_c", c_int),
        ("a_mode", c_int), ("b_mode", c_int), ("c_mode", c_int),
# ... 31 lines not shown
    "jmt_l2norm_fwd": (c_int, [c_int, c_int, c_i64, c_int, c_vp, c_i64, c_vp, c_i64, c_vp, c_f,
                               c_vp]),
    "jmt_l2norm_bwd": (c_int, [c_int, c_int, c_int, c_i64, c_int, c_vp, c_i64, c_vp, c_i64, c_vp,
                               c_f, c_vp, c_i64, c_vp]),
    "jmt_layernorm_fwd": (c_int, [c_int, c_int, c_i64, c_int, c_vp, c_i64, c_vp, c_i64, c_vp,
                                  c_vp, c_f, c_vp, c_i64, c_vp, c_vp, c_vp]),
    "jmt_layernorm_bwd_blocks": (c_int, [c_i64]),
    "jmt_layernorm_bwd": (c_int, [c_int, c_int, c_int, c_i64, c_int, c_vp, c_i64, c_vp, c_i64,
                                  c_vp, c_i64, c_vp, c_vp, c_vp, c_vp, c_i64, c_vp, c_vp, c_int,
                                  c_vp, c_vp]),
    "jmt_layernorm_bwd_dsum": (c_int, [c_int, c_int, c_int, c_i64, c_int, c_vp, c_i64, c_vp,
                                       c_i64, c_vp, c_i64, c_vp, c_vp, c_vp, c_vp, c_i64, c_vp,
                                       c_vp, c_vp, c_int, c_vp, c_vp]),
    "jmt_layernorm_fwd_grouped": (c_int, [c_int, c_int, c_int, c_i64, c_int, c_vp, c_i64, c_i64,
                                          c_vp, c_i64, c_i64, c_vp, c_vp, c_f, c_vp, c_i64, c_i64,
                                          c_vp, c_vp, c_vp]),
    "jmt_layernorm_bwd_grouped": (c_int, [c_int, c_int, c_int, c_int, c_i64, c_int, c_vp, c_i64,
                                          c_i64, c_vp, c_i64, c_i64, c_vp, c_i64, c_i64, c_vp,
                                          c_vp, c_vp, c_vp, c_i64, c_i64, c_vp, c_vp, c_vp, c_int,
                                          c_vp, c_vp]),
    "jmt_softmax_fwd": (c_int, [c_int, c_i64, c_int, c_vp, c_i64, c_f, c_vp, c_i64, c_vp]),
    "jmt_softmax_bwd": (c_int, [c_int, c_int, c_i64, c_int, c_vp, c_i64, c_vp, c_i64, c_f, c_vp,
                                c_i64, c_vp]),
    "jmt_attn_supported": (c_int, [c_int, c_int]),
    "jmt_attn_fwd": (c_int, [c_int, c_int, c_int, c_int, c_int, c_int, c_vp, c_i64, c_i64, c_vp,
                             c_i64, c_i64, c_vp, c_i64, c_i64, c_vp, c_i64, c_i64, c_f, c_vp,
                             c_vp]),
    "jmt_attn_set_fwd_rows": (c_int, [c_int]),
    "jmt_attn_bwd": (c_int, [c_int, c_int, c_int, c_int, c_int, c_int, c_vp, c_i64, c_i64, c_vp,
                             c_i64, c_i64, c_vp, c_i64, c_i64, c_vp, c_i64, c_i64, c_vp, c_i64,
                             c_i64, c_vp, c_vp, c_vp, c_i64, c_vp, c_i64, c_i64, c_f, c_vp]),
    "jmt_attn_short_supported": (c_int, [c_int, c_int, c_int, c_int]),
    "jmt_attn_short_fwd": (c_int, [c_int, c_int, c_int, c_int, c_int, c_int, c_vp, c_i64, c_i64,
                                   c_vp, c_i64, c_i64, c_vp, c_i64, c_i64, c_vp, c_i64, c_i64,
                                   c_f, c_vp, c_vp]),
    "jmt_attn_short_bwd": (c_int, [c_int, c_int, c_int, c_int, c_int, c_int, c_vp, c_i64, c_i64,
                                   c_vp, c_i64, c_i64, c_vp, c_i64, c_i64, c_vp, c_i64, c_i64,
                                   c_vp, c_i64, c_i64, c_vp, c_vp, c_i64, c_i64, c_vp, c_i64,
                                   c_i64, c_vp, c_i64, c_i64, c_f, c_vp]),
    "jmt_attn_dkdv": (c_int, [c_int, c_int, c_int, c_int, c_int, c_int, c_vp, c_vp, c_i64, c_vp,
                              c_i64, c_i64, c_vp, c_i64, c_i64, c_vp, c_i64, c_i64, c_vp, c_i64,
                              c_i64, c_vp, c_i64, c_i64, c_vp, c_i64, c_i64, c_vp]),
    "jmt_attn_fwd_sq": (c_int, [c_int, c_int, c_int, c_int, c_int, c_int, c_vp, c_i64, c_i64,
                                c_vp, c_i64, c_i64, c_vp, c_i64, c_i64, c_vp, c_i64, c_i64, c_f,
                                c_vp, c_int, C.POINTER(c_int), c_int, c_vp]),
    "jmt_attn_bwd_sq": (c_int, [c_int, c_int, c_int, c_int, c_int, c_int, c_vp, c_i64, c_i64,
                                c_vp, c_i64, c_i64, c_vp, c_i64, c_i64, c_vp, c_i64, c_i64, c_vp,
                                c_i64, c_i64, c_vp, c_vp, c_vp, c_i64, c_f, c_int,
                                C.POINTER(c_int), c_int, c_vp]),
    "jmt_attn_dkdv_sq": (c_int, [c_int, c_int, c_int, c_int, c_int, c_int, c_vp, c_vp, c_i64,
                                 c_vp, c_i64, c_i64, c_vp, c_i64, c_i64, c_vp, c_i64, c_i64, c_vp,
                                 c_i64, c_i64, c_vp, c_i64, c_i64, c_vp, c_i64, c_i64, c_int,
                                 C.POINTER(c_int), c_int, c_int, c_vp]),
    "jmt_attn_dkdv_plan": (c_int, [c_int, c_int, c_int, c_i64, c_i64, c_i64, c_int]),
    "jmt_attn_fwd_rows_ok": (c_int, [c_int, c_int, c_int, c_int, c_i64, c_i64]),
    "jmt_attn_bwd_pds_ok": (c_int, [c_int, c_int, c_int, c_int, c_i64, c_i64, c_i64]),
    "jmt_attn_dkdv_ok": (c_int, [c_int, c_int, c_int, c_int, c_i64, c_i64, c_i64, c_i64, c_i64,
                                 c_i64, c_i64, c_int]),
    "jmt_attn_dkdv_set_tile": (c_int, [c_int]),
    "jmt_noop": (c_int, [c_vp]),
    "jmt_small_attn_fwd": (c_int, [c_int, c_int, c_int, c_int, c_int, c_int, c_vp, c_i64, c_i64,
                                   c_vp, c_i64, c_i64, c_vp, c_i64, c_i64, c_vp, c_i64, c_i64,
                                   c_f, c_vp, c_vp]),
    "jmt_small_attn_bwd": (c_int, [c_int, c_int, c_int, c_int, c_int, c_int, c_vp, c_i64, c_i64,
                                   c_vp, c_i64, c_i64, c_vp, c_i64, c_i64, c_vp, c_i64, c_i64,
                                   c_vp, c_vp, c_i64, c_i64, c_vp, c_i64, c_i64, c_vp, c_i64,
                                   c_i64, c_f, c_vp]),
    "jmt_colsum_blocks": (c_int, [c_i64]),
    "jmt_layernorm_bwd_grouped_blocks": (c_int, [c_i64]),
    "jmt_colsum": (c_int, [c_int, c_i64, c_int, c_vp, c_i64, c_vp, c_int, c_vp, c_vp]),
    "jmt_colsum_grouped": (c_int, [c_int, c_int, c_i64, c_int, c_vp, c_i64, c_i64, c_vp, c_int,
                                   c_vp, c_vp]),
    "jmt_copy2d": (c_int, [c_int, c_int, c_i64, c_i64, c_vp, c_i64, c_i64, c_vp, c_i64, c_i64,
                           c_int, c_vp]),
    "jmt_ccc_stats": (c_int, [c_int, c_int, c_i64, c_int, c_vp, c_vp, c_f, c_f, c_f, c_vp, c_vp]),
    "jmt_ccc_finish": (c_int, [c_int, c_int, c_vp, c_i64, c_f, c_vp, c_vp, c_vp]),
    "jmt_ccc_finish_add": (c_int, [c_int, c_int, c_vp, c_i64, c_f, c_vp, c_vp, c_vp, c_vp]),
    "jmt_ccc_bwd": (c_int, [c_int, c_int, c_i64, c_int, c_vp, c_vp, c_f, c_f, c_f, c_vp, c_vp,
                            c_vp, c_vp]),
    "jmt_mask_indices": (c_int, [c_i64, c_vp, c_f, c_vp, c_vp, c_vp]),
    "jmt_vp_scatter": (c_int, [c_i64] + [c_vp] * 9 + [c_f, c_i64] + [c_vp] * 6),
    "jmt_vp_smooth": (c_int, [c_i64, c_int, c_vp, c_vp, c_vp, c_int, c_vp, c_vp]),
    "jmt_head_fwd": (c_int, [c_int, c_int, c_i64, c_int, c_int, c_vp, c_i64, c_vp, c_vp, c_vp,
                             c_vp, c_vp, c_vp, c_i64, c_vp]),
    "jmt_head_bwd": (c_int, [c_int, c_int, c_i64, c_int, c_int, c_vp, c_i64, c_vp, c_vp, c_vp,
                             c_vp, c_i64, c_vp, c_i64, c_vp, c_vp, c_vp, c_vp, c_vp, c_vp]),
    "jmt_head_bwd_workspace_bytes": (C.c_size_t, [c_i64]),
    "jmt_dropout_next": (c_int, [c_vp, c_vp, c_vp]),
    "jmt_dropout": (c_int, [c_int, c_vp, c_i64, c_vp, c_i64, c_i64, c_i64, c_i64, c_f, c_f, c_vp,
                            c_vp]),
    "jmt_head_fwd_drop": (c_int, [c_int, c_int, c_i64, c_int, c_int, c_vp, c_i64, c_vp, c_vp,
                                  c_vp, c_vp, c_vp, c_vp, c_i64, c_f, c_f, c_vp, c_vp]),
    "jmt_head_bwd_drop": (c_int, [c_int, c_int, c_i64, c_int, c_int, c_vp, c_i64, c_vp, c_vp,
                                  c_vp, c_vp, c_i64, c_vp, c_i64, c_vp, c_vp, c_vp, c_vp, c_vp,
                                  c_f, c_f, c_vp, c_vp]),
    "jmt_dropout_reference": (c_int, [C.POINTER(C.c_uint32), c_i64, c_i64, c_i64, c_f, c_f,
                                      c_fp]),
    "jmt_ce_stats": (c_int, [c_int, c_i64, c_int, c_vp, c_vp, c_f, c_f, c_vp, c_vp, c_vp]),
    "jmt_ce_finish": (c_int, [c_int, c_vp, c_vp, c_vp, c_vp]),
    "jmt_ce_bwd": (c_int, [c_int, c_i64, c_int, c_vp, c_vp, c_f, c_f, c_vp, c_vp, c_vp, c_vp,
                           c_vp]),
    "jmt_ce_labels": (c_int, [c_i64, c_int, c_vp, c_f, c_f, c_vp, c_vp]),
    "jmt_vp_ccc": (c_int, [c_i64] + [c_vp] * 6),
    "jmt_amp_check": (c_int, [c_i64, c_vp, c_vp, c_vp]),
    "jmt_sgd_step_amp": (c_int, [c_i64, c_vp, c_vp, c_vp, c_f, c_f, c_f, c_f, c_int, c_int, c_vp,
                                 c_vp, c_int, c_vp]),
# ... 60 lines not shown
```

### joint-multimodal-transformer-6th-abaw_amd/jmt/functional.py

```python
from __future__ import annotations

import collections
import contextlib

import math
import os
from typing import NamedTuple, Optional

import torch
from torch.autograd import Function
from torch.autograd.function import once_differentiable

from . import linear_gemm as lg
from . import ops
from . import streams
from ._lib import F32, JMTError

_policy = {"dtype": None}


def set_compute_dtype(dtype: Optional[torch.dtype]):
    assert dtype in (None, torch.float32, torch.bfloat16, torch.float16)
    _policy["dtype"] = dtype

# ... 601 lines not shown
    def forward(ctx, q_src, k_src, v_src, E, H, qcol, kcol, vcol):
        o, saved = attn_forward(q_src, k_src, v_src, E, H, qcol, kcol, vcol)
        owner = (0, 0 if k_src is q_src else 1,
                 0 if v_src is q_src else (1 if v_src is k_src else 2))
        ctx.save_for_backward(*saved[0])
        ctx.meta = (saved[1], owner)
        return o

    @staticmethod
    @once_differentiable
    def backward(ctx, go):
        tensors = ctx.saved_tensors
        meta, owner = ctx.meta
        q_src, k_src, v_src = tensors[:3]
        cd = meta.cd
        srcs = (q_src, k_src, v_src)
        bufs = [None, None, None]
        E, cols = meta.E, (meta.qcol, meta.kcol, meta.vcol)
        for i in range(3):
            if owner[i] == i:
                width = srcs[i].shape[-1]
                bufs[i] = Rows(srcs[i]).like(width, cd)
                covered = set()
                for j in range(3):
                    if owner[j] == i:
                        covered.update(range(cols[j], cols[j] + E))
                if len(covered) < width:
                    bufs[i].zero_()
        attn_backward((tensors, meta), go, bufs[owner[0]], bufs[owner[1]], bufs[owner[2]])
        grads = [bufs[i] if owner[i] == i else None for i in range(3)]
        return (*grads, None, None, None, None, None)


def _small_aligned(t, col, cd):
    es = t.element_size()
    return ((t.data_ptr() + col * es) % (32 if es == 4 else 16) == 0
            and t.stride(0) % 8 == 0 and t.stride(1) % 8 == 0)


class AttnOperand(NamedTuple):
    aligned: bool
    stride: int


def _operand(t, col, cd) -> AttnOperand:
    return AttnOperand(_small_aligned(t, col, cd), t.stride(0))


class AttnPlan(NamedTuple):
    fwd: str
    rows: bool
    bwd: Optional[str]
    shared_q: bool


AttnMeta = collections.namedtuple("AttnMeta", "E H qcol kcol vcol ldS scale cd fwd")


def attn_plan(cd, N, H, Lq, Lk, E, q, k, v, o, go=None, dq=None, dk=None, dv=None,
              fwd=None) -> AttnPlan:
    dh = E // H
    half = cd != torch.float32
    if fwd is None:
        aligned = q.aligned and k.aligned and v.aligned and o.aligned
        if aligned and ops.small_attn_ok(E, H, Lq, Lk):
            fwd = "small"
        elif half and aligned and ops.attn_short_ok(_dc(cd), dh, Lq, Lk):
            fwd = "short"
        elif half and ops.attn_supported(_dc(cd), dh):
            fwd = "fused"
        else:
            fwd = "gemm"
    rows = fwd == "fused" and ops.attn_fwd_rows_ok(N, H, Lq, Lk, k.stride, v.stride)
    bwd = None
    if None not in (go, dq, dk, dv):
        bwd = fwd
        if fwd == "fused":
            ldp = ops.attn_dkdv_ldp(Lk)
            bwd = "bwd64_gemm"
            if (ops._attn_dkdv["on"] and dk.aligned and dv.aligned and
                    ops.attn_dkdv_ok(N, H, Lq, Lk, ldp, go.stride, q.stride, dk.stride,
                                     dv.stride)):
                bwd = "bwd64_dkdv"
                if (ops._attn_pds["on"] and dq.aligned and k.aligned and
                        ops.attn_bwd_pds_ok(N, H, Lq, Lk, ldp, k.stride, v.stride) and
                        ops.attn_dkdv_ok(N, H, Lq, Lk, ldp, go.stride, q.stride, dk.stride,
                                         dv.stride, k.stride, dq.stride)):
                    bwd = "pds_dkdv"
    return AttnPlan(fwd, rows, bwd, rows and bwd == "pds_dkdv")


def attn_forward(q_src, k_src, v_src, E, H, qcol, kcol, vcol, qshare=None):
    cd = compute_dtype()
    for t in (q_src, k_src, v_src):
        assert t.dtype == cd and t.stride(-1) == 1
    Lq, N = q_src.shape[0], q_src.shape[1]
    Lk = k_src.shape[0]
    dh = E // H
    dev = q_src.device
    ldS = _round_up(Lk, 8)
    bS = (H * Lq * ldS, Lq * ldS)
    scale = 1.0 / math.sqrt(dh)
    o = Rows(q_src).like(E, cd)
    plan = attn_plan(cd, N, H, Lq, Lk, E, _operand(q_src, qcol, cd), _operand(k_src, kcol, cd),
                     _operand(v_src, vcol, cd), _operand(o, 0, cd))
    if qshare is not None and not (plan.fwd == "fused" and plan.rows):
        raise JMTError("attn_forward: qshare on an unsupported shape")
    if plan.fwd == "small":
        P = torch.empty(N * H * Lq * Lk, dtype=torch.float32, device=dev)
        ops.small_attn_fwd(_dc(cd), N, H, Lq, Lk, E,
                           _ptr(q_src, qcol), (q_src.stride(0), q_src.stride(1)),
                           _ptr(k_src, kcol), (k_src.stride(0), k_src.stride(1)),
                           _ptr(v_src, vcol), (v_src.stride(0), v_src.stride(1)),
                           o.data_ptr(), (o.stride(0), o.stride(1)), scale, P)
        tensors = (q_src, k_src, v_src, P, None, None)
    elif plan.fwd in ("short", "fused"):
        lse = torch.empty(N * H * Lq, dtype=torch.float32, device=dev)
        (ops.attn_short_fwd if plan.fwd == "short" else
         ops.attn_fwd_sq if qshare is not None else ops.attn_fwd)(
                     _dc(cd), N, H, Lq, Lk, dh,
                     _ptr(q_src, qcol), (q_src.stride(0), q_src.stride(1)),
                     _ptr(k_src, kcol), (k_src.stride(0), k_src.stride(1)),
                     _ptr(v_src, vcol), (v_src.stride(0), v_src.stride(1)),
                     o.data_ptr(), (o.stride(0), o.stride(1)), scale, lse,
                     *(qshare if qshare is not None else ()))
        tensors = (q_src, k_src, v_src, None, o, lse)
    else:
        P = AttnCoreFn._probs(q_src, k_src, E, H, qcol, kcol, ldS, scale, cd)
        ops.gemm(M=Lq, N=dh, K=Lk, ab_dtype=_dc(cd), c_dtype=_dc(cd),
                 a=[P.data_ptr()], lda=ldS, a_kmajor=True, sA=bS,
                 b=[_ptr(v_src, vcol)], ldb=v_src.stride(0), b_kmajor=False,
                 sB=(v_src.stride(1), dh),
                 c=[o.data_ptr()], ldc=o.stride(0), sC=(o.stride(1), dh),
                 batch0=N, batch1=H, device=dev)
        tensors = (q_src, k_src, v_src, P, None, None)
    return o, (tensors, AttnMeta(E, H, qcol, kcol, vcol, ldS, scale, cd, plan.fwd))


def attn_backward(saved, go, dq, dk, dv, qshare=None, merge_dq=False):
    (q_src, k_src, v_src, *_), meta = saved
    E, H, qcol, kcol, vcol, _, _, cd, fwd = meta
    Lq, N = q_src.shape[0], q_src.shape[1]
    Lk = k_src.shape[0]
    v8 = _vec(cd)
    if go.dtype != cd or go.stride(-1) != 1 or go.stride(0) % v8 or go.stride(1) % v8:
        go = _cast_keep_layout(go if go.stride(-1) == 1 else go.contiguous(), cd)
    if fwd != "gemm" and not _small_aligned(go, 0, cd):
        go = go.clone(memory_format=torch.contiguous_format)
    bwd = attn_plan(cd, N, H, Lq, Lk, E, _operand(q_src, qcol, cd), _operand(k_src, kcol, cd),
                    _operand(v_src, vcol, cd), None, _operand(go, 0, cd), _operand(dq, qcol, cd),
                    _operand(dk, kcol, cd), _operand(dv, vcol, cd), fwd=fwd).bwd
    if qshare is not None and bwd != "pds_dkdv":
        raise JMTError("attn_backward: qshare with buffers the P / dS + dK / dV / dQ kernels "
                       f"do not take (attn_plan: {bwd})")
    outs, tmps = [], {}
    for buf, col in ((dq, qcol), (dk, kcol), (dv, vcol)):
        if bwd == "gemm" or _small_aligned(buf, col, cd):
            outs.append(buf)
            continue
        key = (buf.data_ptr(), tuple(buf.shape), tuple(buf.stride()))
        if key not in tmps:
            tmps[key] = (buf, buf.clone(memory_format=torch.contiguous_format))
        outs.append(tmps[key][1])
    _attn_backward_launch(bwd, saved, go, *outs, qshare, merge_dq)
    for buf, tmp in tmps.values():
        buf.copy_(tmp)


def _attn_backward_launch(bwd, saved, go, dq, dk, dv, qshare, merge_dq):
    (q_src, k_src, v_src, P, o, lse), meta = saved
    E, H, qcol, kcol, vcol, ldS, scale, cd, _ = meta
    Lq, N = q_src.shape[0], q_src.shape[1]
    Lk = k_src.shape[0]
    dh = E // H
    dev = q_src.device
    sq_l, sq_n = q_src.stride(0), q_src.stride(1)
    sk_l, sk_n = k_src.stride(0), k_src.stride(1)
    sv_l, sv_n = v_src.stride(0), v_src.stride(1)
    so_l, so_n = go.stride(0), go.stride(1)
    if bwd in ("small", "short"):
        gouts = [a for t, c in ((dq, qcol), (dk, kcol), (dv, vcol))
                 for a in (_ptr(t, c), (t.stride(0), t.stride(1)))]
        if bwd == "small":
            ops.small_attn_bwd(_dc(cd), N, H, Lq, Lk, E, go.data_ptr(), (so_l, so_n),
                               _ptr(q_src, qcol), (sq_l, sq_n), _ptr(k_src, kcol), (sk_l, sk_n),
                               _ptr(v_src, vcol), (sv_l, sv_n), P, *gouts, scale)
        else:
            ops.attn_short_bwd(_dc(cd), N, H, Lq, Lk, dh, go.data_ptr(), (so_l, so_n),
                               o.data_ptr(), (o.stride(0), o.stride(1)),
                               _ptr(q_src, qcol), (sq_l, sq_n), _ptr(k_src, kcol), (sk_l, sk_n),
                               _ptr(v_src, vcol), (sv_l, sv_n), lse, *gouts, scale)
        return
    if bwd in ("pds_dkdv", "bwd64_dkdv"):
        ldp = ops.attn_dkdv_ldp(Lk)
        P = torch.empty(N * H * Lq * ldp, dtype=cd, device=dev)
        dS = torch.empty(N * H * Lq * ldp, dtype=cd, device=dev)
        pds = bwd == "pds_dkdv"
        dq_args = (_ptr(dq, qcol), (dq.stride(0), dq.stride(1)))
        if qshare is not None:
            ops.attn_bwd_sq(_dc(cd), N, H, Lq, Lk, dh, go.data_ptr(), (so_l, so_n),
                            o.data_ptr(), (o.stride(0), o.stride(1)),
                            _ptr(q_src, qcol), (sq_l, sq_n), _ptr(k_src, kcol), (sk_l, sk_n),
                            _ptr(v_src, vcol), (sv_l, sv_n), lse, P, dS, ldp, scale, *qshare)
            ops.attn_dkdv_sq(_dc(cd), N, H, Lq, Lk, dh, P, dS, ldp, go.data_ptr(), (so_l, so_n),
                             _ptr(q_src, qcol), (sq_l, sq_n), _ptr(dk, kcol),
                             (dk.stride(0), dk.stride(1)), _ptr(dv, vcol),
                             (dv.stride(0), dv.stride(1)), _ptr(k_src, kcol), (sk_l, sk_n),
                             *dq_args, *qshare, merge_dq)
            return
        ops.attn_bwd(_dc(cd), N, H, Lq, Lk, dh, go.data_ptr(), (so_l, so_n),
                     o.data_ptr(), (o.stride(0), o.stride(1)),
                     _ptr(q_src, qcol), (sq_l, sq_n), _ptr(k_src, kcol), (sk_l, sk_n),
                     _ptr(v_src, vcol), (sv_l, sv_n), lse, P, dS, ldp,
                     *((None, (0, 0)) if pds else dq_args), scale)
        ops.attn_dkdv(_dc(cd), N, H, Lq, Lk, dh, P, dS, ldp, go.data_ptr(), (so_l, so_n),
                      _ptr(q_src, qcol), (sq_l, sq_n), _ptr(dk, kcol),
                      (dk.stride(0), dk.stride(1)), _ptr(dv, vcol), (dv.stride(0), dv.stride(1)),
                      *((_ptr(k_src, kcol), (sk_l, sk_n)) + dq_args if pds else ()))
        return
    bS = (H * Lq * ldS, Lq * ldS)
    dS = torch.empty(N * H * Lq * ldS, dtype=cd, device=dev)
    if bwd == "bwd64_gemm":
        P = torch.empty(N * H * Lq * ldS, dtype=cd, device=dev)
        ops.attn_bwd(_dc(cd), N, H, Lq, Lk, dh, go.data_ptr(), (so_l, so_n),
                     o.data_ptr(), (o.stride(0), o.stride(1)),
                     _ptr(q_src, qcol), (sq_l, sq_n), _ptr(k_src, kcol), (sk_l, sk_n),
                     _ptr(v_src, vcol), (sv_l, sv_n), lse, P, dS, ldS,
                     _ptr(dq, qcol), (dq.stride(0), dq.stride(1)), scale)
    else:
        dP = torch.empty(N * H * Lq * ldS, dtype=torch.float32, device=dev)
        ops.gemm(M=Lq, N=Lk, K=dh, ab_dtype=_dc(cd), c_dtype=F32,
                 a=[go.data_ptr()], lda=so_l, a_kmajor=True, sA=(so_n, dh),
                 b=[_ptr(v_src, vcol)], ldb=sv_l, b_kmajor=True, sB=(sv_n, dh),
                 c=[dP.data_ptr()], ldc=ldS, sC=bS, batch0=N, batch1=H, device=dev)
        ops.softmax_bwd(P, ldS, dP, ldS, N * H * Lq, Lk, scale, dS, ldS)
        del dP
        ops.gemm(M=Lq, N=dh, K=Lk, ab_dtype=_dc(cd), c_dtype=_dc(cd),
                 a=[dS.data_ptr()], lda=ldS, a_kmajor=True, sA=bS,
                 b=[_ptr(k_src, kcol)], ldb=sk_l, b_kmajor=False, sB=(sk_n, dh),
                 c=[_ptr(dq, qcol)], ldc=dq.stride(0), sC=(dq.stride(1), dh), batch0=N,
                 batch1=H, device=dev)
    ops.gemm(M=Lk, N=dh, K=Lq, ab_dtype=_dc(cd), c_dtype=_dc(cd),
             a=[dS.data_ptr()], lda=ldS, a_kmajor=False, sA=bS,
             b=[_ptr(q_src, qcol)], ldb=sq_l, b_kmajor=False, sB=(sq_n, dh),
             c=[_ptr(dk, kcol)], ldc=dk.stride(0), sC=(dk.stride(1), dh), batch0=N,
             batch1=H, device=dev)
    ops.gemm(M=Lk, N=dh, K=Lq, ab_dtype=_dc(cd), c_dtype=_dc(cd),
             a=[P.data_ptr()], lda=ldS, a_kmajor=False, sA=bS,
             b=[go.data_ptr()], ldb=so_l, b_kmajor=False, sB=(so_n, dh),
             c=[_ptr(dv, vcol)], ldc=dv.stride(0), sC=(dv.stride(1), dh), batch0=N,
             batch1=H, device=dev)
# ... 240 lines not shown
```

### joint-multimodal-transformer-6th-abaw_amd/jmt/grouped.py

```python
from __future__ import annotations

import functools
import os
from typing import List

import torch
from torch.autograd import Function

from . import linear_gemm as lg
from . import ops, streams
from .functional import (AttnOperand, Rows, _cast_keep_layout, _grad_buffer, _grad_done, _match,
                         _operand, _out, _ptr, attn_backward, attn_forward, attn_plan,
                         compute_dtype, weight_as, wgrad_defer_ok, wgrad_scope)

_enabled = {"on": os.environ.get("JMT_GROUPED", "1") != "0"}
_PAR_STREAM_DGRAD = os.environ.get("JMT_PAR_STREAM_DGRAD", "0") == "1"

CROSS_PAIRS = ((0, 0, 1), (1, 1, 0), (2, 2, 0), (0, 0, 2), (2, 2, 1), (1, 1, 2))


def enabled() -> bool:
    return _enabled["on"]


def set_enabled(on: bool) -> None:
    _enabled["on"] = bool(on)


def _kcat_ok(rows: int, n_ptrs: int, cd) -> bool:
    return (_merge_wgrads["on"] and cd != torch.float32 and rows % 64 == 0 and n_ptrs <= 8)


_merge_wgrads = {"on": os.environ.get("JMT_WGRAD_MERGE", "1") != "0"}


def _contig(t: torch.Tensor, cd) -> torch.Tensor:
    if t.dtype != cd:
        t = ops.cast(t.contiguous(), cd)
    return t if t.is_contiguous() else t.contiguous()


class StackGroupsFn(Function):

    @staticmethod
    def forward(ctx, *xs):
        cd = compute_dtype()
        x0 = xs[0]
        B, T, E = x0.shape
        X = torch.empty(len(xs), B, T, E, dtype=cd, device=x0.device)
        for g, x in enumerate(xs):
            assert tuple(x.shape) == (B, T, E), "StackGroupsFn: streams must share (B, T, E)"
            if x.stride(-1) != 1 or x.stride(1) != E * x.stride(2) or x.stride(0) != T * x.stride(1):
                x = x.contiguous()
            ops.copy2d(x.data_ptr(), ops.dt(x), X[g].data_ptr(), ops.dt(X), B * T, E,
                       x.stride(1), 1, E, 1)
        return X

    @staticmethod
    def backward(ctx, dX):
        return tuple(dX[g] for g in range(dX.shape[0]))


def stack_groups(*xs) -> torch.Tensor:
    return StackGroupsFn.apply(*xs)


class StackJointFn(Function):

    @staticmethod
    def forward(ctx, v, p, W, b):
        cd = compute_dtype()
        B, T, E = v.shape
        assert tuple(p.shape) == (B, T, E) and W.shape == (E, 2 * E), (v.shape, p.shape, W.shape)
        X = torch.empty(3, B, T, E, dtype=cd, device=v.device)
        for g, x in enumerate((v, p)):
            if x.stride(-1) != 1 or x.stride(1) != E * x.stride(2) or \
                    x.stride(0) != T * x.stride(1):
                x = x.contiguous()
            ops.copy2d(x.data_ptr(), ops.dt(x), X[g].data_ptr(), ops.dt(X), B * T, E,
                       x.stride(1), 1, E, 1)
        lg.fwd(lg.kcat([X[0], X[1]], E, E), B * T, W, b, lg.strided(X[2], E), cd)
        ctx.save_for_backward(X, W, b)
        ctx.meta = (cd, v.dtype, p.dtype)
        return X

    @staticmethod
    def backward(ctx, dX):
        X, W, b = ctx.saved_tensors
        cd, vdt, pdt = ctx.meta
        G3, B, T, E = X.shape
        dX = _contig(dX, cd)
        G = Rows(dX[2])
# ... 67 lines not shown
        cd, xdt, xperm, xlperm, operm = ctx.meta
        L, N, E = x.shape
        O = Rows(o)
        G = _match(gy.unsqueeze(0), Rows(O.like(E, cd)), cd)
        do = O.like(E, cd)
        lg.dgrad(G.op(), G.rows, E, Wout, _out(do, O.perm), cd)
        lg.wgrad(G.op(), O.op(), G.rows, E, Wout, cd, bout)
        X = Rows(x)
        dkv = X.like(2 * E, cd)
        dq = Rows(q).like(E, cd)
        attn_backward(ctx.asaved, do, dq, dkv, dkv)
        DKV = Rows(dkv)
        dx = X.like(E, cd)
        lg.dgrad(DKV.op(), DKV.rows, 2 * E, Win, _out(dx, X.perm), cd, E)
        lg.wgrad(DKV.op(), X.op(), DKV.rows, 2 * E, Win, cd, bin_, E)
        DQ = Rows(dq)
        XL = Rows(x[-1:])
        dxl = dx[-1:]
        lg.dgrad(DQ.op(), DQ.rows, E, Win, _out(dxl, XL.perm), cd, beta=1.0)
        lg.wgrad(DQ.op(), XL.op(), DQ.rows, E, Win, cd, bin_)
        if xdt != cd:
            dx = _cast_keep_layout(dx, xdt)
        ctx.asaved = None
        return dx, None, None, None, None, None


def last_query_mha(enc, mha) -> torch.Tensor:
    return LastQueryMHAFn.apply(enc, mha.in_proj_weight, mha.in_proj_bias, mha.out_proj.weight,
                                mha.out_proj.bias, mha.num_heads)


def encoder_layer_params(layer) -> List[torch.Tensor]:
    a, ff = layer.attention, layer.feed_forward
    return [a.in_proj_weight, a.in_proj_bias, a.out_proj.weight, a.out_proj.bias,
            ff[0].weight, ff[0].bias, ff[len(ff) - 1].weight, ff[len(ff) - 1].bias,
            layer.layer_norm1.weight, layer.layer_norm1.bias,
            layer.layer_norm2.weight, layer.layer_norm2.bias]


class EncoderGroupFn(Function):

    @staticmethod
    def forward(ctx, X, meta, *params):
        H, eps1, eps2, batch_axis = meta
        cd = compute_dtype()
        X = _contig(X, cd)
        G, B, T, E = X.shape
        R = B * T
        dev = X.device
        P = [params[12 * g:12 * g + 12] for g in range(G)]
        hid = P[0][4].shape[0]
        col = lambda k: [p[k] for p in P]
        sd = lambda t: lg.strided(t, t.shape[-1], R * t.shape[-1])
        QKV = torch.empty(G, B, T, 3 * E, dtype=cd, device=dev)
        lg.fwd(sd(X), R, col(0), col(1), sd(QKV), cd)
        if batch_axis:
            outs = [attn_forward(QKV[g], QKV[g], QKV[g], E, H, 0, E, 2 * E) for g in range(G)]
            O = [o for o, _ in outs]
            asaved = [sv for _, sv in outs]
        else:
            sf = QKV.view(G * B, T, 3 * E).permute(1, 0, 2)
            o, asaved = attn_forward(sf, sf, sf, E, H, 0, E, 2 * E)
            O = o.permute(1, 0, 2)
        A1 = torch.empty(G, B, T, E, dtype=cd, device=dev)
        lg.fwd(lg.table(O, E) if batch_axis else lg.strided(O, E, R * E), R, col(2), col(3),
               sd(A1), cd)
        H1 = torch.empty_like(A1)
        st1 = torch.empty(2, G * R, dtype=torch.float32, device=dev)
        if not ops.layernorm_fwd_grouped(X, A1, [p[8] for p in P], [p[9] for p in P], eps1, H1,
                                         st1[0], st1[1]):
            for g in range(G):
                ops.layernorm_fwd(X[g], E, A1[g], E, P[g][8], P[g][9], eps1, H1[g], E,
                                  st1[0, g * R:], st1[1, g * R:], R, E)
        F1 = torch.empty(G, B, T, hid, dtype=cd, device=dev)
        lg.fwd(sd(H1), R, col(4), col(5), sd(F1), cd, relu=True)
        F2 = torch.empty(G, B, T, E, dtype=cd, device=dev)
        lg.fwd(sd(F1), R, col(6), col(7), sd(F2), cd)
        Y = torch.empty_like(A1)
        st2 = torch.empty(2, G * R, dtype=torch.float32, device=dev)
        if not ops.layernorm_fwd_grouped(H1, F2, [p[10] for p in P], [p[11] for p in P], eps2, Y,
                                         st2[0], st2[1]):
            for g in range(G):
                ops.layernorm_fwd(H1[g], E, F2[g], E, P[g][10], P[g][11], eps2, Y[g], E,
                                  st2[0, g * R:], st2[1, g * R:], R, E)
        ctx.params = params
        ctx.state = (X, QKV, asaved, O, A1, H1, st1, F1, F2, st2)
        ctx.meta = (G, B, T, E, hid, cd, batch_axis)
        return Y

    @staticmethod
    def backward(ctx, dY):
        G, B, T, E, hid, cd, batch_axis = ctx.meta
        X, QKV, asaved, O, A1, H1, st1, F1, F2, st2 = ctx.state
        o_reads = tuple(O) if batch_axis else (O,)
        params = ctx.params
        P = [params[12 * g:12 * g + 12] for g in range(G)]
        R = B * T
        dev = X.device
        col = lambda k: [p[k] for p in P]
        sd = lambda t: lg.strided(t, t.shape[-1], R * t.shape[-1])
        dY = _contig(dY, cd)

        def ln_bwd(x, r, dy, st, gamma, beta, dx, bias=None):
            fused = bias is not None
            gb = [_grad_buffer(t) for t in gamma]
            bb = [_grad_buffer(t) for t in beta]
            sb = [_grad_buffer(t) for t in bias] if fused else []
            if all(t is not None for t in gb + bb + sb) and ops.layernorm_bwd_grouped(
                    x, r, dy, st[0], st[1], gamma, dx, gb, bb, sb if fused else None,
                    True) is not None:
                for g in range(G):
                    _grad_done(gamma[g], beta[g], *([bias[g]] if fused else []))
                return fused
            for g in range(G):
                bufs = [_grad_buffer(gamma[g]), _grad_buffer(beta[g])]
                if fused:
                    bufs.append(_grad_buffer(bias[g]))
                tmp = None
                if any(b is None for b in bufs):
                    tmp = torch.zeros(3, E, dtype=torch.float32, device=dev)
                outs = bufs if tmp is None else [tmp[0], tmp[1], tmp[2]]
                args = (x[g], E, r[g], E, dy[g], E, st[0, g * R:], st[1, g * R:], gamma[g], dx[g],
                        E, outs[0], outs[1])
                done = fused and ops.layernorm_bwd_dsum(
                    *args, outs[2] if tmp is None else tmp[2], tmp is None, R, E) is not None
                if not done:
                    ops.layernorm_bwd(*args, tmp is None, R, E)
                if tmp is not None:
                    for b, t in zip(bufs[:3 if done else 2], tmp):
                        if b is not None:
                            b.add_(t)
                if done:
                    _grad_done(gamma[g], beta[g], bias[g])
                    continue
                _grad_done(gamma[g], beta[g])
                if fused:
                    lg.bias_grad(lg.strided(dx[g].view(R, E), E), R, E, [bias[g]])
            return fused

        dS = torch.empty(G, B, T, E, dtype=cd, device=dev)
        b2_done = ln_bwd(H1, F2, dY, st2, [p[10] for p in P], [p[11] for p in P], dS,
                         bias=[p[7] for p in P])
        dF1 = torch.empty(G, B, T, hid, dtype=cd, device=dev)
        lg.dgrad(sd(dS), R, E, col(6), sd(dF1), cd, aux=F1, ldaux=hid)
        merged = _merge_wgrads["on"] and hid == E and 2 * G <= 8 and cd != torch.float32
        late = wgrad_defer_ok(cd)
        if merged:
            bsw = ([None] * G if b2_done else col(7)) + col(5)
            each = lambda *ts: lg.table([(t, g * R * E) for t in ts for g in range(G)], E)
            if not lg.wgrad(each(dS, dF1), each(F1, H1), R, E, col(6) + col(4), cd, bsw,
                            intact=late, fallback=False):
                if not b2_done:
                    lg.bias_grad(sd(dS), R, E, col(7))
                lg.bias_grad(sd(dF1), R, hid, col(5))
        else:
            lg.wgrad(sd(dS), sd(F1), R, E, col(6), cd, None if b2_done else col(7), intact=late)
        dH1 = torch.empty_like(dS) if late else dS
        lg.dgrad(sd(dF1), R, hid, col(4), sd(dH1), cd, beta=1.0, c_in=dS if late else None)

        def w1_grads():
            lg.wgrad(sd(dF1), sd(H1), R, hid, col(4), cd, col(5), intact=late)

        if not merged:
            streams.run_side(w1_grads, reads=(dF1, H1))
        dS1 = torch.empty_like(dS)
        bo_done = ln_bwd(X, A1, dH1, st1, [p[8] for p in P], [p[9] for p in P], dS1,
                         bias=[p[3] for p in P])
        dO = dH1
        lg.dgrad(sd(dS1), R, E, col(2), sd(dO), cd)

        def out_proj_grads():
            lg.wgrad(sd(dS1), lg.table(O, E) if batch_axis else lg.strided(O, E, R * E), R, E,
                     col(2), cd, None if bo_done else col(3), intact=late)

        streams.run_side(out_proj_grads, reads=(dS1,) + o_reads)
        dQKV = torch.empty(G, B, T, 3 * E, dtype=cd, device=dev)
        if batch_axis:
            for g in range(G):
                attn_backward(asaved[g], dO[g], dQKV[g], dQKV[g], dQKV[g])
        else:
            dsf = dQKV.view(G * B, T, 3 * E).permute(1, 0, 2)
            attn_backward(asaved, dO.view(G * B, T, E).permute(1, 0, 2), dsf, dsf, dsf)
        streams.wait_side()
        dX = torch.empty_like(dS1) if late else dS1
        lg.dgrad(sd(dQKV), R, 3 * E, col(0), sd(dX), cd, beta=1.0, c_in=dS1 if late else None)

        def in_proj_grads():
            lg.wgrad(sd(dQKV), sd(X), R, 3 * E, col(0), cd, col(1), intact=late)

        streams.run_side(in_proj_grads, reads=(dQKV, X))
        ctx.state = None
        return (dX, None) + (None,) * len(params)


def encoder_group(X, layers, num_heads: int, batch_axis: bool = False):
    params = [p for layer in layers for p in encoder_layer_params(layer)]
    meta = (num_heads, layers[0].layer_norm1.eps, layers[0].layer_norm2.eps, bool(batch_axis))
    return EncoderGroupFn.apply(X, meta, *params)


CROSS_PAIRS_WO_JR = ((0, 0, 1), (1, 1, 0))


def mha_params(mha) -> List[torch.Tensor]:
    return [mha.in_proj_weight, mha.in_proj_bias, mha.out_proj.weight, mha.out_proj.bias]


_shared_q = {"on": os.environ.get("JMT_CA_SHARED_Q", "1") != "0",
             "merge": os.environ.get("JMT_CA_DQ_MERGE", "1") != "0"}


def shared_query_table(pairs):
    first, qtab = {}, []
    for i, (m, q, _) in enumerate(pairs):
        qtab.append(first.setdefault((m, q), i))
    return qtab if any(t != i for i, t in enumerate(qtab)) and len(pairs) <= 8 else None


class CrossAttention6Fn(Function):

    @staticmethod
    def forward(ctx, Y, meta, *params):
        H, pairs = meta
        cd = compute_dtype()
        Y = _contig(Y, cd)
        S, B, T, E = Y.shape
        R = B * T
        dev = Y.device
# ... 214 lines not shown
```

### joint-multimodal-transformer-6th-abaw_amd/jmt/ops.py

```python
from __future__ import annotations

import ctypes as C
import math
import os
from typing import Optional, Sequence

import torch

from . import _lib
from ._lib import BF16, F16, F32, GemmDesc

_DT = {torch.float32: F32, torch.bfloat16: BF16, torch.float16: F16}


def dt(t_or_dtype) -> int:
    d = t_or_dtype if isinstance(t_or_dtype, torch.dtype) else t_or_dtype.dtype
    try:
        return _DT[d]
    except KeyError:
        raise _lib.JMTError(f"unsupported dtype {d}") from None


def stream() -> int:
    return torch.cuda.current_stream().cuda_stream
# ... 465 lines not shown
    _hooked({"family": "attn_dkdv", "flops": 2.0 * nprod * N * H * Lq * Lk * dh,
             "bytes": float(N * H) * ((2 * Lq + 2 * Lk) * dh * es +
                                      2 * Lq * attn_dkdv_ldp(Lk) * es + extra)}, launch)


def _qtab(qtab):
    return (C.c_int * len(qtab))(*qtab), len(qtab)


def attn_fwd_sq(dtype, N, H, Lq, Lk, dh, q_ptr, sq, k_ptr, sk, v_ptr, sv, o_ptr, so, scale, lse,
                spp, qtab):
    tab, npair = _qtab(qtab)
    launch = lambda: _lib.call("jmt_attn_fwd_sq", dtype, N, H, Lq, Lk, dh, q_ptr, sq[0], sq[1],
                               k_ptr, sk[0], sk[1], v_ptr, sv[0], sv[1], o_ptr, so[0], so[1],
                               scale, lse.data_ptr() if lse is not None else None, spp, tab,
                               npair, stream())
    es = 4 if dtype == F32 else 2
    _hooked({"family": "attn_fwd", "flops": 4.0 * N * H * Lq * Lk * dh, "shared_q": True,
             "bytes": float(N * H) * ((2 * Lq + 2 * Lk) * dh * es + 4 * Lq)}, launch)


def attn_bwd_sq(dtype, N, H, Lq, Lk, dh, go_ptr, sgo, o_ptr, so, q_ptr, sq, k_ptr, sk, v_ptr, sv,
                lse, p, ds, ldp, scale, spp, qtab):
    tab, npair = _qtab(qtab)
    launch = lambda: _lib.call("jmt_attn_bwd_sq", dtype, N, H, Lq, Lk, dh, go_ptr, sgo[0],
                               sgo[1], o_ptr, so[0], so[1], q_ptr, sq[0], sq[1], k_ptr, sk[0],
                               sk[1], v_ptr, sv[0], sv[1], lse.data_ptr(), p.data_ptr(),
                               ds.data_ptr(), ldp, scale, spp, tab, npair, stream())
    es = 4 if dtype == F32 else 2
    lw = -(-Lk // 32) * 32
    _hooked({"family": "attn_bwd", "flops": 4.0 * N * H * Lq * Lk * dh, "shared_q": True,
             "bytes": float(N * H) * ((3 * Lq + 2 * Lk) * dh * es + 4 * Lq +
                                      2 * Lq * lw * es)}, launch)


def attn_dkdv_sq(dtype, N, H, Lq, Lk, dh, p, ds, ldp, go_ptr, sgo, q_ptr, sq, dk_ptr, sdk, dv_ptr,
                 sdv, k_ptr, sk, dq_ptr, sdq, spp, qtab, merge_dq):
    tab, npair = _qtab(qtab)
    launch = lambda: _lib.call("jmt_attn_dkdv_sq", dtype, N, H, Lq, Lk, dh, p.data_ptr(),
                               ds.data_ptr(), ldp, go_ptr, sgo[0], sgo[1], q_ptr, sq[0], sq[1],
                               k_ptr, sk[0], sk[1], dk_ptr, sdk[0], sdk[1], dv_ptr, sdv[0],
                               sdv[1], dq_ptr, sdq[0], sdq[1], spp, tab, npair, int(merge_dq),
                               stream())
    es = 4 if dtype == F32 else 2
    nq = N // 2 if merge_dq else N
    extra = (Lk + Lq) * dh * es + Lq * (-(-Lk // 32) * 32) * es
    _hooked({"family": "attn_dkdv", "flops": 6.0 * N * H * Lq * Lk * dh, "shared_q": True,
             "merge_dq": bool(merge_dq),
             "bytes": float(N * H) * ((2 * Lq + 2 * Lk) * dh * es +
                                      2 * Lq * attn_dkdv_ldp(Lk) * es + extra) -
                      float((N - nq) * H) * Lq * dh * es}, launch)


def attn_short_ok(dtype: int, dh: int, Lq: int, Lk: int) -> bool:
    return (_attn_fused["on"] and _attn_short["on"] and
            bool(_lib.load().jmt_attn_short_supported(dtype, dh, Lq, Lk)))


_attn_short = {"on": os.environ.get("JMT_ATTN_SHORT", "1") != "0"}


def attn_short_fwd(dtype, N, H, Lq, Lk, dh, q_ptr, sq, k_ptr, sk, v_ptr, sv, o_ptr, so, scale,
                   lse):
    launch = lambda: _lib.call("jmt_attn_short_fwd", dtype, N, H, Lq, Lk, dh, q_ptr, sq[0], sq[1],
                               k_ptr, sk[0], sk[1], v_ptr, sv[0], sv[1], o_ptr, so[0], so[1],
                               scale, lse.data_ptr(), stream())
    es = 4 if dtype == F32 else 2
    _hooked({"family": "attn_short_fwd", "flops": 4.0 * N * H * Lq * Lk * dh,
             "bytes": float(N * H) * ((2 * Lq + 2 * Lk) * dh * es + 4 * Lq)}, launch)


def attn_short_bwd(dtype, N, H, Lq, Lk, dh, go_ptr, sgo, o_ptr, so, q_ptr, sq, k_ptr, sk, v_ptr,
                   sv, lse, dq_ptr, sdq, dk_ptr, sdk, dv_ptr, sdv, scale):
    launch = lambda: _lib.call("jmt_attn_short_bwd", dtype, N, H, Lq, Lk, dh, go_ptr, sgo[0],
                               sgo[1], o_ptr, so[0], so[1], q_ptr, sq[0], sq[1], k_ptr, sk[0],
                               sk[1], v_ptr, sv[0], sv[1], lse.data_ptr(), dq_ptr, sdq[0], sdq[1],
                               dk_ptr, sdk[0], sdk[1], dv_ptr, sdv[0], sdv[1], scale, stream())
    es = 4 if dtype == F32 else 2
    _hooked({"family": "attn_short_bwd", "flops": 8.0 * N * H * Lq * Lk * dh,
             "bytes": float(N * H) * ((4 * Lq + 4 * Lk) * dh * es + 4 * Lq)}, launch)


SMALL_ATTN_MAX_L = 8


def small_attn_ok(E: int, H: int, Lq: int, Lk: int) -> bool:
    g = E // 8 // H if H > 0 and E % (8 * H) == 0 else 0
    return (_attn_fused["on"] and E == 512 and g > 0 and (g & (g - 1)) == 0 and 1 <= Lq <= SMALL_ATTN_MAX_L
            and 1 <= Lk <= SMALL_ATTN_MAX_L)


def small_attn_fwd(dtype, N, H, Lq, Lk, E, q_ptr, sq, k_ptr, sk, v_ptr, sv, o_ptr, so, scale,
                   p):
    launch = lambda: _lib.call("jmt_small_attn_fwd", dtype, N, H, Lq, Lk, E, q_ptr, sq[0],
                               sq[1], k_ptr, sk[0], sk[1], v_ptr, sv[0], sv[1], o_ptr, so[0],
                               so[1], scale, p.data_ptr() if p is not None else None, stream())
    es = 4 if dtype == F32 else 2
    nbytes = float(N) * (2 * Lq + 2 * Lk) * E * es + (4.0 * N * H * Lq * Lk if p is not None
                                                       else 0.0)
    _hooked({"family": "small_attn_fwd", "flops": 4.0 * N * Lq * Lk * E, "bytes": nbytes},
            launch)


def small_attn_bwd(dtype, N, H, Lq, Lk, E, go_ptr, sgo, q_ptr, sq, k_ptr, sk, v_ptr, sv, p,
                   dq_ptr, sdq, dk_ptr, sdk, dv_ptr, sdv, scale):
    launch = lambda: _lib.call("jmt_small_attn_bwd", dtype, N, H, Lq, Lk, E, go_ptr, sgo[0],
# ... 170 lines not shown
```

Measured before the change: 18030 windows/s.

## Fold K/V projections into Q and output weights for single-head self-attention

```diff
diff --git a/include/jmt.h b/include/jmt.h
--- a/include/jmt.h
+++ b/include/jmt.h
@@ -141,6 +141,24 @@
                      int64_t sdv_n, void* dq, int64_t sdq_l, int64_t sdq_n, int spp,
                      const int* qtab, int npair, int merge_dq, void* stream);
 
+int jmt_attn_fwd_kt(int dt, int N, int H, int Lq, int Lk, int dh, const void* q, int64_t sq_l,
+                    int64_t sq_n, const void* k, int64_t sk_l, int64_t sk_n, void* o, int64_t so_l,
+                    int64_t so_n, float scale, float* lse, int spp, const int* qtab,
+                    const int* ktab, int npair, int kgroups, void* stream);
+int jmt_attn_bwd_kt(int dt, int N, int H, int Lq, int Lk, int dh, const void* go, int64_t sgo_l,
+                    int64_t sgo_n, const void* o, int64_t so_l, int64_t so_n, const void* q,
+                    int64_t sq_l, int64_t sq_n, const void* k, int64_t sk_l, int64_t sk_n,
+                    const float* lse, void* p_out, void* ds_out, int64_t ldp, float scale, int spp,
+                    const int* qtab, const int* ktab, int npair, int kgroups, void* stream);
+int jmt_attn_dkdv_kt(int dt, int N, int H, int Lq, int Lk, int dh, const void* p, const void* ds,
+                     int64_t ldp, const void* go, int64_t sgo_l, int64_t sgo_n, const void* q,
+                     int64_t sq_l, int64_t sq_n, const void* k, int64_t sk_l, int64_t sk_n,
+                     void* t, int64_t st_l, int64_t st_n, void* dq, int64_t sdq_l, int64_t sdq_n,
+                     int spp, const int* qtab, const int* ktab, int npair, int kgroups,
+                     int merge_dq, void* stream);
+int jmt_attn_kt_ok(int dt, int N, int H, int Lq, int Lk, int dh, int64_t ldp, int64_t sk_l,
+                   int npair, int kgroups);
+
 int jmt_attn_fwd_rows_ok(int N, int H, int Lq, int Lk, int64_t sk_l, int64_t sv_l);
 int jmt_attn_bwd_pds_ok(int N, int H, int Lq, int Lk, int64_t ldp, int64_t sk_l, int64_t sv_l);
 int jmt_attn_dkdv_ok(int N, int H, int Lq, int Lk, int64_t ldp, int64_t sgo_l, int64_t sq_l,
diff --git a/joint-multimodal-transformer-6th-abaw_amd/csrc/abi_check.cpp b/joint-multimodal-transformer-6th-abaw_amd/csrc/abi_check.cpp
--- a/joint-multimodal-transformer-6th-abaw_amd/csrc/abi_check.cpp
+++ b/joint-multimodal-transformer-6th-abaw_amd/csrc/abi_check.cpp
@@ -398,6 +398,40 @@
                                                             algn, 512, 512, algn, 512, 512, 1, id2,
                                                             2, 1, nullptr));
   }
+  {
+    const int id4[4] = {0, 1, 2, 3}, kt4[4] = {1, 0, 0, 2}, kbad[4] = {1, 0, 3, 2};
+    const int big[9] = {0, 1, 2, 3, 4, 5, 6, 7, 8};
+#define FWD_KT(dt, N, Lq, dh, ktab, np, kg)                                                   \
+    jmt_attn_fwd_kt(dt, N, 1, Lq, 300, dh, algn, 512, 512, algn, 512, 512, algn, 512, 512, 0.1f, \
+                    fnull, 1, np == 9 ? big : id4, ktab, np, kg, nullptr)
+#define BWD_KT(dt, N, Lq, dh, ktab, np, kg)                                                   \
+    jmt_attn_bwd_kt(dt, N, 1, Lq, 300, dh, algn, 512, 512, algn, 512, 512, algn, 512, 512, algn, \
+                    512, 512, fnull, algn, algn, 384, 0.1f, 1, np == 9 ? big : id4, ktab, np, kg, \
+                    nullptr)
+#define DKDV_KT(dt, N, Lq, dh, ktab, np, kg)                                                  \
+    jmt_attn_dkdv_kt(dt, N, 1, Lq, 300, dh, algn, algn, 384, algn, 512, 512, algn, 512, 512,  \
+                     algn, 512, 512, algn, 512, 512, algn, 512, 512, 1, np == 9 ? big : id4,  \
+                     ktab, np, kg, 0, nullptr)
+#define KT_ALL(what, dt, N, Lq, dh, ktab, np, kg, needle)                                     \
+    expect_rc("fwd_kt " what, FWD_KT(dt, N, Lq, dh, ktab, np, kg), JMT_ERR_UNSUPPORTED, needle); \
+    expect_rc("bwd_kt " what, BWD_KT(dt, N, Lq, dh, ktab, np, kg), JMT_ERR_UNSUPPORTED, needle); \
+    expect_rc("dkdv_kt " what, DKDV_KT(dt, N, Lq, dh, ktab, np, kg), JMT_ERR_UNSUPPORTED, needle)
+    KT_ALL("fp32", JMT_F32, 4, 300, 512, kt4, 4, 3, "16-bit");
+    KT_ALL("dh 256", JMT_BF16, 4, 300, 256, kt4, 4, 3, "16-bit");
+    KT_ALL("Lq 64", JMT_BF16, 4, 64, 512, kt4, 4, 3, "16-bit");
+    KT_ALL("entry >= groups", JMT_BF16, 4, 300, 512, kbad, 4, 3, "outside the key buffer");
+    KT_ALL("9 pairs", JMT_BF16, 9, 300, 512, big, 9, 9, "at most 8 pairs");
+    expect_eq("kt_ok in", jmt_attn_kt_ok(JMT_BF16, 4, 1, 300, 300, 512, 384, 512, 4, 3), 1);
+    expect_eq("kt_ok fp32", jmt_attn_kt_ok(JMT_F32, 4, 1, 300, 300, 512, 384, 512, 4, 3), 0);
+    expect_eq("kt_ok Lq 64", jmt_attn_kt_ok(JMT_BF16, 4, 1, 64, 300, 512, 384, 512, 4, 3), 0);
+    expect_eq("kt_ok 2 heads", jmt_attn_kt_ok(JMT_BF16, 4, 2, 300, 300, 512, 384, 1024, 4, 3), 0);
+    expect_eq("kt_ok 9 pairs", jmt_attn_kt_ok(JMT_BF16, 9, 1, 300, 300, 512, 384, 512, 9, 9), 0);
+    expect_err("fwd_kt null key table", FWD_KT(JMT_BF16, 4, 300, 512, nullptr, 4, 3));
+#undef KT_ALL
+#undef DKDV_KT
+#undef BWD_KT
+#undef FWD_KT
+  }
   expect_err("small_attn_fwd null", jmt_small_attn_fwd(JMT_BF16, 4, 1, 6, 6, 512, nullptr, 512,
                                                        512, nullptr, 512, 512, nullptr, 512, 512,
                                                        nullptr, 512, 512, 0.1f, fnull, nullptr));
diff --git a/joint-multimodal-transformer-6th-abaw_amd/csrc/attn.hip b/joint-multimodal-transformer-6th-abaw_amd/csrc/attn.hip
--- a/joint-multimodal-transformer-6th-abaw_amd/csrc/attn.hip
+++ b/joint-multimodal-transformer-6th-abaw_amd/csrc/attn.hip
@@ -20,6 +20,7 @@
   float scale_log2;
   uint64_t* stamps;
   QShare qs;
+  QShare ks;
 };
 
 template <bool STAMP>
@@ -508,7 +509,7 @@
 constexpr int AP_KT = 32;
 constexpr int AP_LDS = 4 * AP_KT * AT_ROWB;
 
-template <typename T, int DBG = 0, bool SQ = false>
+template <typename T, int DBG = 0, bool SQ = false, bool KV = false>
 __global__ __launch_bounds__(512, 2) void attn_bwd_pds_kernel(AttnBwdArgs p) {
   int tcount = 0;
   auto st = [&](int phase) {
@@ -530,8 +531,8 @@
   if (item >= iend) return;
 
   int nh = item / nqt, n = nh / p.H, hd = nh % p.H, q0 = (item % nqt) * AP_QT;
-  const T* kb = (const T*)p.k + (int64_t)n * p.sk_n + hd * AT_DH;
-  const T* vb = (const T*)p.v + (int64_t)n * p.sv_n + hd * AT_DH;
+  const T* kb = (const T*)p.k + (int64_t)k_seq<KV>(p.ks, n) * p.sk_n + hd * AT_DH;
+  const T* vb = KV ? kb : (const T*)p.v + (int64_t)n * p.sv_n + hd * AT_DH;
 
   F qf[16], df[16], of[16];
   auto load_qd = [&](int n_, int hd_, int q0_) {
@@ -566,7 +567,7 @@
       const int src = min(k0 + r, p.Lk - 1);
       const uint32_t dst = lbase + b * 2 * IMG + r * AT_ROWB;
       glds16_at((const char*)kbase + (unsigned)(src * ldk) + loff[i], dst);
-      glds16_at((const char*)vbase + (unsigned)(src * ldv) + loff[i], dst + IMG);
+      if constexpr (!KV) glds16_at((const char*)vbase + (unsigned)(src * ldv) + loff[i], dst + IMG);
     }
   };
   stage_tile(0, kb, vb, 0);
@@ -582,8 +583,8 @@
     const int nxt = item + istride;
     const bool more = nxt < iend;
     const int nh2 = nxt / nqt, n2 = nh2 / p.H, hd2 = nh2 % p.H, q02 = (nxt % nqt) * AP_QT;
-    const T* kb2 = (const T*)p.k + (int64_t)n2 * p.sk_n + hd2 * AT_DH;
-    const T* vb2 = (const T*)p.v + (int64_t)n2 * p.sv_n + hd2 * AT_DH;
+    const T* kb2 = (const T*)p.k + (int64_t)k_seq<KV>(p.ks, more ? n2 : n) * p.sk_n + hd2 * AT_DH;
+    const T* vb2 = KV ? kb2 : (const T*)p.v + (int64_t)n2 * p.sv_n + hd2 * AT_DH;
 
     float delta;
     {
@@ -631,7 +632,8 @@
           for (int kt = 0; kt < 2; ++kt) {
             const int o = kb4[ks & 3] + 256 * (ks >> 2) + 16384 * kt;
             dst[kt] = *(const F*)(kimg + o);
-            dst[2 + kt] = *(const F*)(vimg + o);
+            if constexpr (KV) dst[2 + kt] = dst[kt];
+            else dst[2 + kt] = *(const F*)(vimg + o);
           }
         };
         batch(fa, 0);
@@ -719,7 +721,7 @@
 constexpr int AR_LDS = 4 * AR_KT * AT_ROWB;
 constexpr int AR_VB = 4;
 
-template <typename T, int DBG = 0, bool SQ = false>
+template <typename T, int DBG = 0, bool SQ = false, bool KV = false>
 __global__ __launch_bounds__(512, 2) void attn_fwd_rows_kernel(AttnFwdArgs p) {
   typedef typename Frag16<T>::t F;
   typedef typename Frag16<T>::h Hf;
@@ -735,8 +737,8 @@
   if (item >= iend) return;
 
   int nh = item / nqt, n = nh / p.H, hd = nh % p.H, q0 = (item % nqt) * AR_QT;
-  const T* kb = (const T*)p.k + (int64_t)n * p.sk_n + hd * AT_DH;
-  const T* vb = (const T*)p.v + (int64_t)n * p.sv_n + hd * AT_DH;
+  const T* kb = (const T*)p.k + (int64_t)k_seq<KV>(p.ks, n) * p.sk_n + hd * AT_DH;
+  const T* vb = KV ? kb : (const T*)p.v + (int64_t)n * p.sv_n + hd * AT_DH;
 
   F qf[16];
   auto load_q = [&](int n_, int hd_, int q0_) {
@@ -761,7 +763,7 @@
       JMT_DCHECK(src >= 0 && src < p.Lk);
       const uint32_t dst = lbase + b * 2 * IMG + r * AT_ROWB;
       glds16_sv((const char*)kbase + (unsigned)(src * ldk), loff[i], dst);
-      glds16_sv((const char*)vbase + (unsigned)(src * ldv), loff[i], dst + IMG);
+      if constexpr (!KV) glds16_sv((const char*)vbase + (unsigned)(src * ldv), loff[i], dst + IMG);
     }
   };
   stage_tile(0, kb, vb, 0);
@@ -782,8 +784,8 @@
     const int nxt = item + istride;
     const bool more = nxt < iend;
     const int nh2 = nxt / nqt, n2 = nh2 / p.H, hd2 = nh2 % p.H, q02 = (nxt % nqt) * AR_QT;
-    const T* kb2 = (const T*)p.k + (int64_t)n2 * p.sk_n + hd2 * AT_DH;
-    const T* vb2 = (const T*)p.v + (int64_t)n2 * p.sv_n + hd2 * AT_DH;
+    const T* kb2 = (const T*)p.k + (int64_t)k_seq<KV>(p.ks, more ? n2 : n) * p.sk_n + hd2 * AT_DH;
+    const T* vb2 = KV ? kb2 : (const T*)p.v + (int64_t)n2 * p.sv_n + hd2 * AT_DH;
 
     f32x4 o[32];
 #pragma unroll
@@ -797,7 +799,7 @@
     auto tile = [&](int j, auto last_c) {
       constexpr bool LAST = decltype(last_c)::value;
       const char* kimg = smem + buf * 2 * IMG;
-      const char* vimg = kimg + IMG;
+      const char* vimg = KV ? kimg : kimg + IMG;
       if ((!LAST && (DBG & 8) == 0) || (LAST && more))
         stage_tile(buf ^ 1, LAST ? kb2 : kb, LAST ? vb2 : vb, LAST ? 0 : AR_KT * (j + 1));
       f32x4 sl[2], sh[2];
@@ -1028,7 +1030,8 @@
 static int attn_fwd_impl(int dt, int N, int H, int Lq, int Lk, int dh, const void* q,
                          int64_t sq_l, int64_t sq_n, const void* k, int64_t sk_l, int64_t sk_n,
                          const void* v, int64_t sv_l, int64_t sv_n, void* o, int64_t so_l,
-                         int64_t so_n, float scale, float* lse, const QShare* qs, void* stream) {
+                         int64_t so_n, float scale, float* lse, const QShare* qs, void* stream,
+                         const QShare* ks = nullptr) {
   if (N == 0 || Lq == 0) return JMT_OK;
   if (!jmt_attn_supported(dt, dh))
     return set_error(JMT_ERR_UNSUPPORTED, "jmt_attn_fwd: dtype %d / head dim %d not supported",
@@ -1045,6 +1048,7 @@
   if (rc != JMT_OK) return rc;
   AttnFwdArgs a = {};
   if (qs) a.qs = *qs;
+  if (ks) a.ks = *ks;
   a.q = q; a.k = k; a.v = v; a.o = o; a.lse = lse;
   a.sq_l = sq_l; a.sq_n = sq_n; a.sk_l = sk_l; a.sk_n = sk_n; a.sv_l = sv_l; a.sv_n = sv_n;
   a.so_l = so_l; a.so_n = so_n;
@@ -1053,7 +1057,7 @@
   hipStream_t st = as_stream(stream);
   a.nitems = ((Lq + qt - 1) / qt) * N * H;
   const dim3 grid(persistent_grid(a.nitems));
-  const char* name = qs ? "jmt_attn_fwd_sq" : "jmt_attn_fwd";
+  const char* name = ks ? "jmt_attn_fwd_kt" : qs ? "jmt_attn_fwd_sq" : "jmt_attn_fwd";
 #if JMT_DIAG
   static const int dbg =
       getenv("JMT_ATTN_FWD_ROWS_DBG") ? atoi(getenv("JMT_ATTN_FWD_ROWS_DBG")) : 0;
@@ -1079,6 +1083,7 @@
   by_elem(dt, [&](auto e) {
     using T = typename decltype(e)::type;
     if (!rows) attn_launch<attn_fwd_kernel<T, false, ATTN_FWD_OPT>, AF_LDS>(grid, st, a);
+    else if (ks) attn_launch<attn_fwd_rows_kernel<T, 0, true, true>, AR_LDS>(grid, st, a);
     else if (qs) attn_launch<attn_fwd_rows_kernel<T, 0, true>, AR_LDS>(grid, st, a);
     else attn_launch<attn_fwd_rows_kernel<T>, AR_LDS>(grid, st, a);
   });
@@ -1116,7 +1121,7 @@
                          int64_t sk_n, const void* v, int64_t sv_l, int64_t sv_n,
                          const float* lse, void* p_out, void* ds_out, int64_t ldp, void* dq,
                          int64_t sdq_l, int64_t sdq_n, float scale, const QShare* qs,
-                         void* stream) {
+                         void* stream, const QShare* ks = nullptr) {
   if (N == 0 || Lq == 0) return JMT_OK;
   if (!jmt_attn_supported(dt, dh))
     return set_error(JMT_ERR_UNSUPPORTED, "jmt_attn_bwd: dtype %d / head dim %d not supported",
@@ -1136,6 +1141,7 @@
   }
   AttnBwdArgs a = {};
   if (qs) a.qs = *qs;
+  if (ks) a.ks = *ks;
   a.go = go; a.o = o; a.q = q; a.k = k; a.v = v; a.lse = lse;
   a.pbuf = p_out; a.dsbuf = ds_out; a.dq = dq;
   a.sgo_l = sgo_l; a.sgo_n = sgo_n; a.so_l = so_l; a.so_n = so_n; a.sq_l = sq_l; a.sq_n = sq_n;
@@ -1148,7 +1154,7 @@
   a.nitems = ((Lq + qt - 1) / qt) * N * H;
   const dim3 grid(persistent_grid(a.nitems));
   hipStream_t st = as_stream(stream);
-  const char* name = qs ? "jmt_attn_bwd_sq" : "jmt_attn_bwd";
+  const char* name = ks ? "jmt_attn_bwd_kt" : qs ? "jmt_attn_bwd_sq" : "jmt_attn_bwd";
 #if JMT_DIAG
   static const int dbg = getenv("JMT_ATTN_PDS_DBG") ? atoi(getenv("JMT_ATTN_PDS_DBG")) : 0;
   if (pds && dbg && dt == JMT_BF16) {
@@ -1169,6 +1175,7 @@
   by_elem(dt, [&](auto e) {
     using T = typename decltype(e)::type;
     if (!pds) attn_launch<attn_bwd_kernel<T, ATTN_BWD_OPT>, AB_LDS>(grid, st, a);
+    else if (ks) attn_launch<attn_bwd_pds_kernel<T, 0, true, true>, AP_LDS>(grid, st, a);
     else if (qs) attn_launch<attn_bwd_pds_kernel<T, 0, true>, AP_LDS>(grid, st, a);
     else attn_launch<attn_bwd_pds_kernel<T>, AP_LDS>(grid, st, a);
   });
@@ -1206,3 +1213,57 @@
                        sk_l, sk_n, v, sv_l, sv_n, lse, p_out, ds_out, ldp, nullptr, 0, 0, scale,
                        &qs, stream);
 }
+
+static bool kt_range(int dt, int dh, int H, int Lq) {
+  return (dt == JMT_BF16 || dt == JMT_F16) && dh == AT_DH && H == 1 && Lq > AT_QT;
+}
+
+extern "C" int jmt_attn_kt_ok(int dt, int N, int H, int Lq, int Lk, int dh, int64_t ldp,
+                              int64_t sk_l, int npair, int kgroups) {
+  return kt_range(dt, dh, H, Lq) && npair >= 1 && npair <= 8 && kgroups >= 1 && kgroups <= 16 &&
+         N % npair == 0 && fwd_rows(Lq, Lk, sk_l, sk_l) && sizes_ok(N, H, Lq, Lk, AR_QT) &&
+         pds_range(N, H, Lq, Lk, ldp, sk_l, sk_l) == nullptr;
+}
+
+static int kt_tables(const char* name, int dt, int N, int H, int Lq, int dh, int spp,
+                     const int* qtab, const int* ktab, int npair, int kgroups, QShare* qs,
+                     QShare* ks) {
+  if (!kt_range(dt, dh, H, Lq))
+    return set_error(JMT_ERR_UNSUPPORTED, "%s: 16-bit, one head of dim %d and Lq > %d only "
+                                          "(dtype %d, H %d, dh %d, Lq %d)",
+                     name, AT_DH, AT_QT, dt, H, dh, Lq);
+  int rc = kshare_pack(name, N, spp, ktab, npair, kgroups, ks);
+  if (rc != JMT_OK) return rc;
+  return qshare_pack(name, N, spp, qtab, npair, qs);
+}
+
+extern "C" int jmt_attn_fwd_kt(int dt, int N, int H, int Lq, int Lk, int dh, const void* q,
+                               int64_t sq_l, int64_t sq_n, const void* k, int64_t sk_l,
+                               int64_t sk_n, void* o, int64_t so_l, int64_t so_n, float scale,
+                               float* lse, int spp, const int* qtab, const int* ktab, int npair,
+                               int kgroups, void* stream) {
+  if (N == 0 || Lq == 0) return JMT_OK;
+  QShare qs = {}, ks = {};
+  int rc = kt_tables("jmt_attn_fwd_kt", dt, N, H, Lq, dh, spp, qtab, ktab, npair, kgroups, &qs,
+                     &ks);
+  if (rc != JMT_OK) return rc;
+  return attn_fwd_impl(dt, N, H, Lq, Lk, dh, q, sq_l, sq_n, k, sk_l, sk_n, k, sk_l, sk_n, o, so_l,
+                       so_n, scale, lse, &qs, stream, &ks);
+}
+
+extern "C" int jmt_attn_bwd_kt(int dt, int N, int H, int Lq, int Lk, int dh, const void* go,
+                               int64_t sgo_l, int64_t sgo_n, const void* o, int64_t so_l,
+                               int64_t so_n, const void* q, int64_t sq_l, int64_t sq_n,
+                               const void* k, int64_t sk_l, int64_t sk_n, const float* lse,
+                               void* p_out, void* ds_out, int64_t ldp, float scale, int spp,
+                               const int* qtab, const int* ktab, int npair, int kgroups,
+                               void* stream) {
+  if (N == 0 || Lq == 0) return JMT_OK;
+  QShare qs = {}, ks = {};
+  int rc = kt_tables("jmt_attn_bwd_kt", dt, N, H, Lq, dh, spp, qtab, ktab, npair, kgroups, &qs,
+                     &ks);
+  if (rc != JMT_OK) return rc;
+  return attn_bwd_impl(dt, N, H, Lq, Lk, dh, go, sgo_l, sgo_n, o, so_l, so_n, q, sq_l, sq_n, k,
+                       sk_l, sk_n, k, sk_l, sk_n, lse, p_out, ds_out, ldp, nullptr, 0, 0, scale,
+                       &qs, stream, &ks);
+}
diff --git a/joint-multimodal-transformer-6th-abaw_amd/csrc/attn_common.h b/joint-multimodal-transformer-6th-abaw_amd/csrc/attn_common.h
--- a/joint-multimodal-transformer-6th-abaw_amd/csrc/attn_common.h
+++ b/joint-multimodal-transformer-6th-abaw_amd/csrc/attn_common.h
@@ -26,6 +26,33 @@
   for (int p = 0; p < npair; ++p) {
     JMT_CHECK_ARG(tab[p] >= 0 && tab[p] <= p && tab[tab[p]] == tab[p],
                   "%s: query table entry %d (%d) is not an earlier first use", name, p, tab[p]);
+    bits |= (uint32_t)tab[p] << (4 * p);
+  }
+  out->spp = spp;
+  out->tab = bits;
+  return JMT_OK;
+}
+
+template <bool KV>
+__device__ __forceinline__ int k_seq(const QShare& s, int n) {
+  if constexpr (!KV) return n;
+  const int p = n / s.spp;
+  return (int)((s.tab >> (4 * p)) & 15u) * s.spp + (n - p * s.spp);
+}
+
+static inline int kshare_pack(const char* name, int N, int spp, const int* tab, int npair,
+                              int kgroups, QShare* out) {
+  if (npair > 8 || kgroups > 16)
+    return set_error(JMT_ERR_UNSUPPORTED, "%s: at most 8 pairs over at most 16 key groups (%d, %d)",
+                     name, npair, kgroups);
+  JMT_CHECK_ARG(tab != nullptr && spp > 0 && npair >= 1 && kgroups >= 1 &&
+                    (int64_t)spp * npair == N,
+                "%s: key table needs 1-8 pairs of spp sequences with npair * spp == N", name);
+  uint32_t bits = 0;
+  for (int p = 0; p < npair; ++p) {
+    if (tab[p] < 0 || tab[p] >= kgroups)
+      return set_error(JMT_ERR_UNSUPPORTED, "%s: key table entry %d (%d) outside the key buffer's "
+                                            "%d groups", name, p, tab[p], kgroups);
     bits |= (uint32_t)tab[p] << (4 * p);
   }
   out->spp = spp;
@@ -65,6 +92,7 @@
   int Lq, Lk, H, nitems;
   float scale, scale_log2;
   QShare qs;
+  QShare ks;
 };
 
 __device__ __forceinline__ int img_off(int row, int b) {
diff --git a/joint-multimodal-transformer-6th-abaw_amd/csrc/attn_dkdv.hip b/joint-multimodal-transformer-6th-abaw_amd/csrc/attn_dkdv.hip
--- a/joint-multimodal-transformer-6th-abaw_amd/csrc/attn_dkdv.hip
+++ b/joint-multimodal-transformer-6th-abaw_amd/csrc/attn_dkdv.hip
@@ -39,6 +39,7 @@
   int64_t ldp, sgo_l, sgo_n, sq_l, sq_n, sk_l, sk_n, sdk_l, sdk_n, sdv_l, sdv_n, sdq_l, sdq_n;
   int Lq, Lk, H, nkt, nqd, ipn, nitems;
   QShare qs;
+  QShare ks;
   int mrg;
   uint32_t mg_first, mg_second;
 };
@@ -58,8 +59,10 @@
 struct DkItem {
   int nh, n, hd, role, k0, nch, nch1, n2, nh2;
 };
-template <int KT, bool SQ>
+template <int KT, bool SQ, bool KV = false>
 __device__ __forceinline__ DkItem dk_decode(const AttnDkdvArgs& a, int it) {
+  constexpr int NP = KV ? 1 : 2;
+  [[maybe_unused]] const int nchq = (a.Lq + DK_QC - 1) / DK_QC;
   DkItem d;
   if (SQ && a.mrg) {
     const int gi = it / a.ipn;
@@ -78,11 +81,12 @@
       d.n2 = n2;
     } else {
       r -= a.nqd;
-      const int second = r >= 2 * a.nkt;
-      r -= second * 2 * a.nkt;
-      d.role = r >= a.nkt;
+      const int second = r >= NP * a.nkt;
+      r -= second * NP * a.nkt;
+      d.role = KV ? 0 : r >= a.nkt;
       d.k0 = (r - d.role * a.nkt) * KT;
-      d.nch = d.nch1 = (a.Lq + DK_QC - 1) / DK_QC;
+      d.nch1 = nchq;
+      d.nch = KV ? 2 * nchq : nchq;
       d.n = d.n2 = second ? n2 : n1;
     }
     d.nh = d.n * a.H + d.hd;
@@ -91,24 +95,24 @@
   }
   d.nh = it / a.ipn;
   const int r = it - d.nh * a.ipn;
-  if (r < 2 * a.nkt) {
-    d.role = r >= a.nkt;
+  if (r < NP * a.nkt) {
+    d.role = KV ? 0 : r >= a.nkt;
     d.k0 = (r - d.role * a.nkt) * KT;
-    d.nch = (a.Lq + DK_QC - 1) / DK_QC;
+    d.nch = d.nch1 = nchq;
+    if constexpr (KV) d.nch = 2 * nchq;
   } else {
     d.role = 2;
-    d.k0 = (r - 2 * a.nkt) * KT;
-    d.nch = (a.Lk + DK_QC - 1) / DK_QC;
+    d.k0 = (r - NP * a.nkt) * KT;
+    d.nch = d.nch1 = (a.Lk + DK_QC - 1) / DK_QC;
   }
   d.n = d.nh / a.H;
   d.hd = d.nh - d.n * a.H;
-  d.nch1 = d.nch;
   d.n2 = d.n;
   d.nh2 = d.nh;
   return d;
 }
 
-template <typename T, bool SQ>
+template <typename T, bool SQ, bool KV = false>
 __device__ __forceinline__ void dkdv_stage(char* st, const AttnDkdvArgs& a, const DkItem& d,
                                            int c) {
   const int lane = threadIdx.x & 63;
@@ -117,7 +121,8 @@
   const int q0 = DK_QC * (second ? c - d.nch1 : c);
   if (d.role == 2) {
     const int sn = second ? d.n2 : d.n, snh = second ? d.nh2 : d.nh;
-    const char* kb = (const char*)((const T*)a.k + (int64_t)sn * a.sk_n + d.hd * AT_DH);
+    const char* kb = (const char*)((const T*)a.k + (int64_t)k_seq<KV>(a.ks, sn) * a.sk_n +
+                                   d.hd * AT_DH);
     const int ldk = (int)(a.sk_l * (int64_t)sizeof(T));
 #pragma unroll
     for (int i = 0; i < DK_QC / 8; ++i) {
@@ -137,7 +142,8 @@
   }
   const char* rb;
   int ldb;
-  if (d.role == 0) {
+  const bool dkr = d.role == 1 || (KV && second);
+  if (!dkr) {
     rb = (const char*)((const T*)a.go + (int64_t)d.n * a.sgo_n + d.hd * AT_DH);
     ldb = (int)(a.sgo_l * (int64_t)sizeof(T));
   } else {
@@ -156,20 +162,20 @@
   const int src_row = min(q0 + r, a.Lq - 1);
   JMT_DCHECK(src_row >= 0 && d.k0 + 8 * cs + 8 <= a.ldp);
   if (a.dq) {
-    const char* pb = (const char*)((const T*)(d.role == 0 ? a.p : a.ds) +
+    const char* pb = (const char*)((const T*)(dkr ? a.ds : a.p) +
                                    (int64_t)d.nh * a.Lq * a.ldp);
     glds16_asm(pb + (unsigned)((((d.k0 >> 5) + (cs >> 2)) * a.Lq + src_row) * 64) +
                    16 * (cs & 3),
                st + DK_IMG + wu * 1024);
     return;
   }
-  const char* pb = (const char*)((const T*)(d.role == 0 ? a.p : a.ds) +
+  const char* pb = (const char*)((const T*)(dkr ? a.ds : a.p) +
                                  (int64_t)d.nh * a.Lq * a.ldp + d.k0);
   glds16_asm(pb + (unsigned)(src_row * (int)(a.ldp * sizeof(T))) + 16 * cs,
              st + DK_IMG + wu * 1024);
 }
 
-template <typename T, bool SQ>
+template <typename T, bool SQ, bool KV = false>
 __device__ __forceinline__ void dkdv_stage160(uint32_t st, const AttnDkdvArgs& a, const DkItem& d,
                                               int ch) {
   typedef DkGeo<10> G;
@@ -180,16 +186,18 @@
   const int snh = second ? d.nh2 : d.nh;
   const char* rb;
   int ldb, clen;
-  if (d.role == 0) {
+  const bool dkr = d.role == 1 || (KV && d.role == 0 && second);
+  if (d.role == 0 && !dkr) {
     rb = (const char*)((const T*)a.go + (int64_t)d.n * a.sgo_n + d.hd * AT_DH);
     ldb = (int)(a.sgo_l * (int64_t)sizeof(T));
     clen = a.Lq;
-  } else if (d.role == 1) {
+  } else if (dkr) {
     rb = (const char*)((const T*)a.q + (int64_t)q_seq<SQ>(a.qs, d.n) * a.sq_n + d.hd * AT_DH);
     ldb = (int)(a.sq_l * (int64_t)sizeof(T));
     clen = a.Lq;
   } else {
-    rb = (const char*)((const T*)a.k + (int64_t)(second ? d.n2 : d.n) * a.sk_n + d.hd * AT_DH);
+    rb = (const char*)((const T*)a.k + (int64_t)k_seq<KV>(a.ks, second ? d.n2 : d.n) * a.sk_n +
+                       d.hd * AT_DH);
     ldb = (int)(a.sk_l * (int64_t)sizeof(T));
     clen = a.Lk;
   }
@@ -201,7 +209,7 @@
     const unsigned off = (unsigned)(lane ^ ((r & 7) << 1)) << 4;
     glds16_sv(rb + (unsigned)(src * ldb), off, st + r * AT_ROWB);
   }
-  const char* pb = (const char*)((const T*)(d.role == 0 ? a.p : a.ds) +
+  const char* pb = (const char*)((const T*)(d.role == 0 && !dkr ? a.p : a.ds) +
                                  (int64_t)snh * a.Lq * a.ldp);
   const int ntile = (int)(a.ldp >> 5);
   if (lane < G::PLANES) {
@@ -251,7 +259,7 @@
 
 #define DK_NO_MERGE() asm volatile("" ::: "memory")
 
-template <typename T, int NKG, bool SQ>
+template <typename T, int NKG, bool SQ, bool KV = false>
 __global__ __launch_bounds__(512, 2) void attn_dkdv_kernel(AttnDkdvArgs a) {
   typedef typename Frag16<T>::t F;
   typedef typename Frag16<T>::h Hf;
@@ -291,22 +299,22 @@
   const uint32_t lbase = (uint32_t)(uintptr_t)(__attribute__((address_space(3))) char*)smem;
 
   int is_item = item, is_c = 0;
-  DkItem is_d = dk_decode<KT, SQ>(a, item);
+  DkItem is_d = dk_decode<KT, SQ, KV>(a, item);
   bool is_ok = true;
   int is_buf = 0;
   unsigned after = 0;
   int inflight = 0;
   auto issue = [&]() {
     if (is_ok) {
-      if constexpr (NKG == 8) dkdv_stage<T, SQ>(smem + is_buf * STAGE, a, is_d, is_c);
-      else dkdv_stage160<T, SQ>(lbase + is_buf * STAGE, a, is_d, is_c);
+      if constexpr (NKG == 8) dkdv_stage<T, SQ, KV>(smem + is_buf * STAGE, a, is_d, is_c);
+      else dkdv_stage160<T, SQ, KV>(lbase + is_buf * STAGE, a, is_d, is_c);
       after &= ~(15u << (4 * is_buf));
       ++inflight;
       if (++is_c == is_d.nch) {
         is_c = 0;
         is_item += istride;
         is_ok = is_item < iend;
-        if (is_ok) is_d = dk_decode<KT, SQ>(a, is_item);
+        if (is_ok) is_d = dk_decode<KT, SQ, KV>(a, is_item);
       }
     }
     is_buf = is_buf == NS - 1 ? 0 : is_buf + 1;
@@ -315,7 +323,7 @@
   int buf = 0;
 
   while (true) {
-    const DkItem d = dk_decode<KT, SQ>(a, item);
+    const DkItem d = dk_decode<KT, SQ, KV>(a, item);
     const bool more = item + istride < iend;
     f32x4 acc[NKG][4];
 #pragma unroll
@@ -490,18 +498,20 @@
   return nullptr;
 }
 
-template <typename T, int NKG, bool SQ>
+template <typename T, int NKG, bool SQ, bool KV = false>
 static void dkdv_launch_sq(const AttnDkdvArgs& a, int grid, hipStream_t st) {
   constexpr int lds = DkGeo<NKG>::LDS;
-  static bool once = ((void)hipFuncSetAttribute((const void*)attn_dkdv_kernel<T, NKG, SQ>,
+  static bool once = ((void)hipFuncSetAttribute((const void*)attn_dkdv_kernel<T, NKG, SQ, KV>,
                                                 hipFuncAttributeMaxDynamicSharedMemorySize, lds),
                       true);
   (void)once;
-  hipLaunchKernelGGL((attn_dkdv_kernel<T, NKG, SQ>), dim3(grid), dim3(512), (size_t)lds, st, a);
+  hipLaunchKernelGGL((attn_dkdv_kernel<T, NKG, SQ, KV>), dim3(grid), dim3(512), (size_t)lds, st,
+                     a);
 }
 template <typename T, int NKG>
-static void dkdv_launch(const AttnDkdvArgs& a, int grid, hipStream_t st, bool sq) {
-  if (sq) dkdv_launch_sq<T, NKG, true>(a, grid, st);
+static void dkdv_launch(const AttnDkdvArgs& a, int grid, hipStream_t st, bool sq, bool kv) {
+  if (kv) dkdv_launch_sq<T, NKG, true, true>(a, grid, st);
+  else if (sq) dkdv_launch_sq<T, NKG, true>(a, grid, st);
   else dkdv_launch_sq<T, NKG, false>(a, grid, st);
 }
 
@@ -534,7 +544,8 @@
                      int64_t sq_l, int64_t sq_n, const void* k, int64_t sk_l, int64_t sk_n,
                      void* dk, int64_t sdk_l, int64_t sdk_n, void* dv, int64_t sdv_l,
                      int64_t sdv_n, void* dq, int64_t sdq_l, int64_t sdq_n, const QShare* qs,
-                     const int* qtab, int npair, int merge, void* stream) {
+                     const int* qtab, int npair, int merge, void* stream,
+                     const QShare* ks = nullptr) {
   if (N == 0 || Lk == 0) return JMT_OK;
   if (!((dt == JMT_BF16 || dt == JMT_F16) && dh == AT_DH))
     return set_error(JMT_ERR_UNSUPPORTED, "jmt_attn_dkdv: dtype %d / head dim %d not supported",
@@ -558,12 +569,14 @@
   const int nqd = dq ? (Lq + kt - 1) / kt : 0;
   AttnDkdvArgs a = {};
   if (qs) a.qs = *qs;
+  if (ks) a.ks = *ks;
   a.p = p; a.ds = ds; a.go = go; a.q = q; a.k = k; a.dk = dk; a.dv = dv; a.dq = dq;
   a.ldp = ldp; a.sgo_l = sgo_l; a.sgo_n = sgo_n; a.sq_l = sq_l; a.sq_n = sq_n;
   a.sk_l = sk_l; a.sk_n = sk_n;
   a.sdk_l = sdk_l; a.sdk_n = sdk_n; a.sdv_l = sdv_l; a.sdv_n = sdv_n;
   a.sdq_l = sdq_l; a.sdq_n = sdq_n;
-  a.Lq = Lq; a.Lk = Lk; a.H = H; a.nkt = nkt; a.nqd = nqd; a.ipn = 2 * nkt + nqd;
+  const int np = ks ? 1 : 2;
+  a.Lq = Lq; a.Lk = Lk; a.H = H; a.nkt = nkt; a.nqd = nqd; a.ipn = np * nkt + nqd;
   a.nitems = N * H * a.ipn;
   if (merge) {
     int ng = 0;
@@ -581,17 +594,17 @@
       ++ng;
     }
     a.mrg = 1;
-    a.ipn = nqd + 4 * nkt;
+    a.ipn = nqd + 2 * np * nkt;
     a.nitems = ng * a.qs.spp * H * a.ipn;
   }
   const int grid = dkdv_grid(a.nitems);
   hipStream_t st = as_stream(stream);
   if (kt == 160) {
-    if (dt == JMT_BF16) dkdv_launch<__bf16, 10>(a, grid, st, qs != nullptr);
-    else dkdv_launch<_Float16, 10>(a, grid, st, qs != nullptr);
+    if (dt == JMT_BF16) dkdv_launch<__bf16, 10>(a, grid, st, qs != nullptr, ks != nullptr);
+    else dkdv_launch<_Float16, 10>(a, grid, st, qs != nullptr, ks != nullptr);
   } else {
-    if (dt == JMT_BF16) dkdv_launch<__bf16, 8>(a, grid, st, qs != nullptr);
-    else dkdv_launch<_Float16, 8>(a, grid, st, qs != nullptr);
+    if (dt == JMT_BF16) dkdv_launch<__bf16, 8>(a, grid, st, qs != nullptr, ks != nullptr);
+    else dkdv_launch<_Float16, 8>(a, grid, st, qs != nullptr, ks != nullptr);
   }
   JMT_LAUNCH_CHECK("jmt_attn_dkdv");
   return JMT_OK;
@@ -629,3 +642,28 @@
                    sk_n, dk, sdk_l, sdk_n, dv, sdv_l, sdv_n, dq, sdq_l, sdq_n, &qs, qtab, npair,
                    merge_dq != 0, stream);
 }
+
+extern "C" int jmt_attn_dkdv_kt(int dt, int N, int H, int Lq, int Lk, int dh, const void* p,
+                                const void* ds, int64_t ldp, const void* go, int64_t sgo_l,
+                                int64_t sgo_n, const void* q, int64_t sq_l, int64_t sq_n,
+                                const void* k, int64_t sk_l, int64_t sk_n, void* t,
+                                int64_t st_l, int64_t st_n, void* dq, int64_t sdq_l,
+                                int64_t sdq_n, int spp, const int* qtab, const int* ktab,
+                                int npair, int kgroups, int merge_dq, void* stream) {
+  if (N == 0 || Lk == 0) return JMT_OK;
+  if (!((dt == JMT_BF16 || dt == JMT_F16) && dh == AT_DH && H == 1 && Lq > 64))
+    return set_error(JMT_ERR_UNSUPPORTED, "jmt_attn_dkdv_kt: 16-bit, one head of dim %d and "
+                                          "Lq > 64 only (dtype %d, H %d, dh %d, Lq %d)",
+                     AT_DH, dt, H, dh, Lq);
+  if (dq == nullptr)
+    return set_error(JMT_ERR_UNSUPPORTED, "jmt_attn_dkdv_kt: the tile-major form only (dq != "
+                                          "NULL: P / dS from jmt_attn_bwd_kt)");
+  QShare qs = {}, ks = {};
+  int rc = kshare_pack("jmt_attn_dkdv_kt", N, spp, ktab, npair, kgroups, &ks);
+  if (rc != JMT_OK) return rc;
+  rc = qshare_pack("jmt_attn_dkdv_kt", N, spp, qtab, npair, &qs);
+  if (rc != JMT_OK) return rc;
+  return dkdv_impl(dt, N, H, Lq, Lk, dh, p, ds, ldp, go, sgo_l, sgo_n, q, sq_l, sq_n, k, sk_l,
+                   sk_n, t, st_l, st_n, t, st_l, st_n, dq, sdq_l, sdq_n, &qs, qtab, npair,
+                   merge_dq != 0, stream, &ks);
+}
diff --git a/joint-multimodal-transformer-6th-abaw_amd/jmt/_lib.py b/joint-multimodal-transformer-6th-abaw_amd/jmt/_lib.py
--- a/joint-multimodal-transformer-6th-abaw_amd/jmt/_lib.py
+++ b/joint-multimodal-transformer-6th-abaw_amd/jmt/_lib.py
@@ -107,6 +107,19 @@
                                  c_vp, c_i64, c_i64, c_vp, c_i64, c_i64, c_vp, c_i64, c_i64, c_vp,
                                  c_i64, c_i64, c_vp, c_i64, c_i64, c_vp, c_i64, c_i64, c_int,
                                  C.POINTER(c_int), c_int, c_int, c_vp]),
+    "jmt_attn_fwd_kt": (c_int, [c_int, c_int, c_int, c_int, c_int, c_int, c_vp, c_i64, c_i64,
+                                c_vp, c_i64, c_i64, c_vp, c_i64, c_i64, c_f, c_vp, c_int,
+                                C.POINTER(c_int), C.POINTER(c_int), c_int, c_int, c_vp]),
+    "jmt_attn_bwd_kt": (c_int, [c_int, c_int, c_int, c_int, c_int, c_int, c_vp, c_i64, c_i64,
+                                c_vp, c_i64, c_i64, c_vp, c_i64, c_i64, c_vp, c_i64, c_i64, c_vp,
+                                c_vp, c_vp, c_i64, c_f, c_int, C.POINTER(c_int),
+                                C.POINTER(c_int), c_int, c_int, c_vp]),
+    "jmt_attn_dkdv_kt": (c_int, [c_int, c_int, c_int, c_int, c_int, c_int, c_vp, c_vp, c_i64,
+                                 c_vp, c_i64, c_i64, c_vp, c_i64, c_i64, c_vp, c_i64, c_i64, c_vp,
+                                 c_i64, c_i64, c_vp, c_i64, c_i64, c_int, C.POINTER(c_int),
+                                 C.POINTER(c_int), c_int, c_int, c_int, c_vp]),
+    "jmt_attn_kt_ok": (c_int, [c_int, c_int, c_int, c_int, c_int, c_int, c_i64, c_i64, c_int,
+                               c_int]),
     "jmt_attn_dkdv_plan": (c_int, [c_int, c_int, c_int, c_i64, c_i64, c_i64, c_int]),
     "jmt_attn_fwd_rows_ok": (c_int, [c_int, c_int, c_int, c_int, c_i64, c_i64]),
     "jmt_attn_bwd_pds_ok": (c_int, [c_int, c_int, c_int, c_int, c_i64, c_i64, c_i64]),
diff --git a/joint-multimodal-transformer-6th-abaw_amd/jmt/functional.py b/joint-multimodal-transformer-6th-abaw_amd/jmt/functional.py
--- a/joint-multimodal-transformer-6th-abaw_amd/jmt/functional.py
+++ b/joint-multimodal-transformer-6th-abaw_amd/jmt/functional.py
@@ -677,13 +677,15 @@
     rows: bool
     bwd: Optional[str]
     shared_q: bool
-
-
-AttnMeta = collections.namedtuple("AttnMeta", "E H qcol kcol vcol ldS scale cd fwd")
+    key_table: bool = False
+
+
+AttnMeta = collections.namedtuple("AttnMeta", "E H qcol kcol vcol ldS scale cd fwd ktable",
+                                  defaults=(None,))
 
 
 def attn_plan(cd, N, H, Lq, Lk, E, q, k, v, o, go=None, dq=None, dk=None, dv=None,
-              fwd=None) -> AttnPlan:
+              fwd=None, ktable=None) -> AttnPlan:
     dh = E // H
     half = cd != torch.float32
     if fwd is None:
@@ -712,10 +714,13 @@
                         ops.attn_dkdv_ok(N, H, Lq, Lk, ldp, go.stride, q.stride, dk.stride,
                                          dv.stride, k.stride, dq.stride)):
                     bwd = "pds_dkdv"
-    return AttnPlan(fwd, rows, bwd, rows and bwd == "pds_dkdv")
-
-
-def attn_forward(q_src, k_src, v_src, E, H, qcol, kcol, vcol, qshare=None):
+    shared = rows and bwd == "pds_dkdv"
+    kt = (shared and ktable is not None and
+          ops.attn_kt_ok(_dc(cd), N, H, Lq, Lk, dh, ops.attn_dkdv_ldp(Lk), k.stride, *ktable))
+    return AttnPlan(fwd, rows, bwd, shared, kt)
+
+
+def attn_forward(q_src, k_src, v_src, E, H, qcol, kcol, vcol, qshare=None, ktable=None):
     cd = compute_dtype()
     for t in (q_src, k_src, v_src):
         assert t.dtype == cd and t.stride(-1) == 1
@@ -731,6 +736,16 @@
                      _operand(v_src, vcol, cd), _operand(o, 0, cd))
     if qshare is not None and not (plan.fwd == "fused" and plan.rows):
         raise JMTError("attn_forward: qshare on an unsupported shape")
+    if ktable is not None:
+        if qshare is None or k_src is not v_src or kcol != vcol:
+            raise JMTError("attn_forward: a key table needs qshare and v_src = k_src")
+        lse = torch.empty(N * H * Lq, dtype=torch.float32, device=dev)
+        ops.attn_fwd_kt(_dc(cd), N, H, Lq, Lk, dh, _ptr(q_src, qcol),
+                        (q_src.stride(0), q_src.stride(1)), _ptr(k_src, kcol),
+                        (k_src.stride(0), k_src.stride(1)), o.data_ptr(),
+                        (o.stride(0), o.stride(1)), scale, lse, *qshare, *ktable)
+        return o, ((q_src, k_src, v_src, None, o, lse),
+                   AttnMeta(E, H, qcol, kcol, vcol, ldS, scale, cd, plan.fwd, tuple(ktable)))
     if plan.fwd == "small":
         P = torch.empty(N * H * Lq * Lk, dtype=torch.float32, device=dev)
         ops.small_attn_fwd(_dc(cd), N, H, Lq, Lk, E,
@@ -764,7 +779,7 @@
 
 def attn_backward(saved, go, dq, dk, dv, qshare=None, merge_dq=False):
     (q_src, k_src, v_src, *_), meta = saved
-    E, H, qcol, kcol, vcol, _, _, cd, fwd = meta
+    E, H, qcol, kcol, vcol, _, _, cd, fwd, ktable = meta
     Lq, N = q_src.shape[0], q_src.shape[1]
     Lk = k_src.shape[0]
     v8 = _vec(cd)
@@ -775,6 +790,8 @@
     bwd = attn_plan(cd, N, H, Lq, Lk, E, _operand(q_src, qcol, cd), _operand(k_src, kcol, cd),
                     _operand(v_src, vcol, cd), None, _operand(go, 0, cd), _operand(dq, qcol, cd),
                     _operand(dk, kcol, cd), _operand(dv, vcol, cd), fwd=fwd).bwd
+    if ktable is not None and not (dk is dv and qshare is not None):
+        raise JMTError("attn_backward: a key-table call writes one key-side gradient (dk is dv)")
     if qshare is not None and bwd != "pds_dkdv":
         raise JMTError("attn_backward: qshare with buffers the P / dS + dK / dV / dQ kernels "
                        f"do not take (attn_plan: {bwd})")
@@ -794,7 +811,7 @@
 
 def _attn_backward_launch(bwd, saved, go, dq, dk, dv, qshare, merge_dq):
     (q_src, k_src, v_src, P, o, lse), meta = saved
-    E, H, qcol, kcol, vcol, ldS, scale, cd, _ = meta
+    E, H, qcol, kcol, vcol, ldS, scale, cd, _, ktable = meta
     Lq, N = q_src.shape[0], q_src.shape[1]
     Lk = k_src.shape[0]
     dh = E // H
@@ -822,6 +839,16 @@
         dS = torch.empty(N * H * Lq * ldp, dtype=cd, device=dev)
         pds = bwd == "pds_dkdv"
         dq_args = (_ptr(dq, qcol), (dq.stride(0), dq.stride(1)))
+        if ktable is not None:
+            ops.attn_bwd_kt(_dc(cd), N, H, Lq, Lk, dh, go.data_ptr(), (so_l, so_n),
+                            o.data_ptr(), (o.stride(0), o.stride(1)),
+                            _ptr(q_src, qcol), (sq_l, sq_n), _ptr(k_src, kcol), (sk_l, sk_n),
+                            lse, P, dS, ldp, scale, *qshare, *ktable)
+            ops.attn_dkdv_kt(_dc(cd), N, H, Lq, Lk, dh, P, dS, ldp, go.data_ptr(), (so_l, so_n),
+                             _ptr(q_src, qcol), (sq_l, sq_n), _ptr(dk, kcol),
+                             (dk.stride(0), dk.stride(1)), _ptr(k_src, kcol), (sk_l, sk_n),
+                             *dq_args, *qshare, *ktable, merge_dq)
+            return
         if qshare is not None:
             ops.attn_bwd_sq(_dc(cd), N, H, Lq, Lk, dh, go.data_ptr(), (so_l, so_n),
                             o.data_ptr(), (o.stride(0), o.stride(1)),
diff --git a/joint-multimodal-transformer-6th-abaw_amd/jmt/grouped.py b/joint-multimodal-transformer-6th-abaw_amd/jmt/grouped.py
--- a/joint-multimodal-transformer-6th-abaw_amd/jmt/grouped.py
+++ b/joint-multimodal-transformer-6th-abaw_amd/jmt/grouped.py
@@ -38,6 +38,113 @@
     if t.dtype != cd:
         t = ops.cast(t.contiguous(), cd)
     return t if t.is_contiguous() else t.contiguous()
+
+
+_fold = {"on": os.environ.get("JMT_ATTN_FOLD", "0") == "1"}
+
+
+def attn_fold_enabled() -> bool:
+    return _fold["on"]
+
+
+def set_attn_fold(on: bool) -> None:
+    _fold["on"] = bool(on)
+
+
+class FoldedMHA:
+
+    def __init__(self, mods, cd, dev):
+        self.mods, self.cd = list(mods), cd
+        nm, E = len(self.mods), self.mods[0][2].shape[0]
+        self.E = E
+        f32 = dict(dtype=torch.float32, device=dev)
+        W32 = torch.empty(2, nm, E, E, **f32)
+        b32 = torch.empty(2, nm, E, **f32)
+        win = lambda r: [_ptr(m[0], r * E * E) for m in self.mods]
+        bin_ = lambda r: [_ptr(m[1], r * E) for m in self.mods]
+        wout = [m[2].data_ptr() for m in self.mods]
+        kw = dict(N=E, K=E, ab_dtype=ops.F32, c_dtype=ops.F32, lda=E, ldb=E, ldc=E, a_mode=lg.TABLE,
+                  b_mode=lg.TABLE, batch0=nm, splits=1, device=dev)
+        ops.gemm(M=E, a=win(1), a_kmajor=False, b=win(0), b_kmajor=False,
+                 c=[W32[0].data_ptr()], sC=(E * E, 0), **kw)
+        ops.gemm(M=E, a=wout, a_kmajor=True, b=win(2), b_kmajor=False,
+                 c=[W32[1].data_ptr()], sC=(E * E, 0), **kw)
+        ops.gemm(M=1, a=bin_(0), a_kmajor=True, b=win(1), b_kmajor=False,
+                 c=[b32[0].data_ptr()], sC=(E, 0), **kw)
+        ops.gemm(M=1, a=bin_(2), a_kmajor=True, b=wout, b_kmajor=True,
+                 c=[b32[1].data_ptr()], sC=(E, 0), bias_tab=[m[3] for m in self.mods], **kw)
+        W16 = ops.cast(W32, cd)
+        leaf = lambda t: t.detach().requires_grad_(True)
+        self.WA, self.WB = ([leaf(W32[j, m]) for m in range(nm)] for j in (0, 1))
+        self.cA, self.eB = ([leaf(b32[j, m]) for m in range(nm)] for j in (0, 1))
+        for j, ws in enumerate((self.WA, self.WB)):
+            for m, w in enumerate(ws):
+                w._jmt_shadow = (w._version, cd, w.data_ptr(), W16[j, m])
+        self._keep = (W32, b32, W16)
+        self.G32 = self.g32 = None
+
+    def begin_backward(self):
+        nm, E, dev = len(self.mods), self.E, self.WA[0].device
+        self.G32 = torch.zeros(2, nm, E, E, dtype=torch.float32, device=dev)
+        self.g32 = torch.zeros(2, nm, E, dtype=torch.float32, device=dev)
+        for j, (ws, bs) in enumerate(((self.WA, self.cA), (self.WB, self.eB))):
+            for m in range(nm):
+                ws[m].grad, bs[m].grad = self.G32[j, m], self.g32[j, m]
+
+    def backward(self):
+        streams.wait_side()
+        nm, E, dev = len(self.mods), self.E, self.WA[0].device
+        G32, g32 = self.G32, self.g32
+
+        def buf(p):
+            g = _grad_buffer(p)
+            return g if g is not None else torch.zeros_like(p)
+
+        gWi, gbi, gWo, gbo = ([buf(m[k]) for m in self.mods] for k in range(4))
+        win = lambda r: [_ptr(m[0], r * E * E) for m in self.mods]
+        wout = [m[2].data_ptr() for m in self.mods]
+        kw = dict(N=E, K=E, ab_dtype=ops.F32, c_dtype=ops.F32, lda=E, ldb=E, ldc=E, c_mode=lg.TABLE,
+                  batch0=nm, beta=1.0, splits=1, device=dev)
+        tab = dict(a_mode=lg.TABLE)
+        sA = lambda j: dict(a=[G32[j].data_ptr()], sA=(E * E, 0))
+        sB = lambda j: dict(b=[G32[j].data_ptr()], sB=(E * E, 0))
+        tb = dict(b_mode=lg.TABLE)
+        ops.gemm(M=E, a=win(1), a_kmajor=True, b_kmajor=False, c=[_ptr(g, 0) for g in gWi],
+                 **tab, **sB(0), **kw)
+        ops.gemm(M=E, a=win(0), a_kmajor=True, b_kmajor=True, c=[_ptr(g, E * E) for g in gWi],
+                 **tab, **sB(0), **kw)
+        ops.gemm(M=E, a=wout, a_kmajor=False, b_kmajor=False,
+                 c=[_ptr(g, 2 * E * E) for g in gWi], **tab, **sB(1), **kw)
+        ops.gemm(M=E, a_kmajor=True, b=win(2), b_kmajor=True, c=[g.data_ptr() for g in gWo],
+                 **tb, **sA(1), **kw)
+        ops.gemm(M=1, a=[g32[0].data_ptr()], sA=(E, 0), a_kmajor=True, b=win(1), b_kmajor=True,
+                 c=[g.data_ptr() for g in gbi], **tb, **kw)
+        ops.gemm(M=1, a=[g32[1].data_ptr()], sA=(E, 0), a_kmajor=True, b=wout, b_kmajor=False,
+                 c=[_ptr(g, 2 * E) for g in gbi], **tb, **kw)
+        for m, mod in enumerate(self.mods):
+            bq, bv = mod[1].detach()[:E], mod[1].detach()[2 * E:]
+            gWi[m][E:2 * E].addr_(bq, g32[0, m])
+            gWo[m].addr_(g32[1, m], bv)
+            gbo[m].add_(g32[1, m])
+        for mod in self.mods:
+            _grad_done(*mod)
+        self.G32 = self.g32 = None
+
+    def after_weight_grads(self, held: bool):
+        if held and torch._C._current_graph_task_id() >= 0:
+            torch.autograd.Variable._execution_engine.queue_callback(self.backward)
+        else:
+            self.backward()
+
+
+_eye = {}
+
+
+def _identity(E: int, cd, dev) -> torch.Tensor:
+    key = (E, cd, dev)
+    if key not in _eye:
+        _eye[key] = torch.eye(E, dtype=cd, device=dev)
+    return _eye[key]
 
 
 class StackGroupsFn(Function):
@@ -211,9 +318,26 @@
         hid = P[0][4].shape[0]
         col = lambda k: [p[k] for p in P]
         sd = lambda t: lg.strided(t, t.shape[-1], R * t.shape[-1])
-        QKV = torch.empty(G, B, T, 3 * E, dtype=cd, device=dev)
-        lg.fwd(sd(X), R, col(0), col(1), sd(QKV), cd)
-        if batch_axis:
+        fold = None
+        if _fold["on"] and H == 1 and cd != torch.float32 and not batch_axis and G <= 8:
+            od = AttnOperand(True, E)
+            if attn_plan(cd, G * B, H, T, T, E, od, od, od, od, od, od, od, od,
+                         ktable=(G, G)).key_table:
+                fold = FoldedMHA([p[:4] for p in P], cd, dev)
+        if fold is not None:
+            QKV = torch.empty(G, B, T, E, dtype=cd, device=dev)
+            lg.fwd(sd(X), R, fold.WA, fold.cA, sd(QKV), cd)
+            ident = list(range(G))
+            o, asaved = attn_forward(QKV.view(G * B, T, E).permute(1, 0, 2),
+                                     *(X.view(G * B, T, E).permute(1, 0, 2),) * 2, E, H, 0, 0, 0,
+                                     qshare=(B, ident), ktable=(ident, G))
+            O = o.permute(1, 0, 2)
+        else:
+            QKV = torch.empty(G, B, T, 3 * E, dtype=cd, device=dev)
+            lg.fwd(sd(X), R, col(0), col(1), sd(QKV), cd)
+        if fold is not None:
+            pass
+        elif batch_axis:
             outs = [attn_forward(QKV[g], QKV[g], QKV[g], E, H, 0, E, 2 * E) for g in range(G)]
             O = [o for o, _ in outs]
             asaved = [sv for _, sv in outs]
@@ -222,7 +346,8 @@
             o, asaved = attn_forward(sf, sf, sf, E, H, 0, E, 2 * E)
             O = o.permute(1, 0, 2)
         A1 = torch.empty(G, B, T, E, dtype=cd, device=dev)
-        lg.fwd(lg.table(O, E) if batch_axis else lg.strided(O, E, R * E), R, col(2), col(3),
+        lg.fwd(lg.table(O, E) if batch_axis else lg.strided(O, E, R * E), R,
+               fold.WB if fold is not None else col(2), fold.eB if fold is not None else col(3),
                sd(A1), cd)
         H1 = torch.empty_like(A1)
         st1 = torch.empty(2, G * R, dtype=torch.float32, device=dev)
@@ -245,6 +370,7 @@
         ctx.params = params
         ctx.state = (X, QKV, asaved, O, A1, H1, st1, F1, F2, st2)
         ctx.meta = (G, B, T, E, hid, cd, batch_axis)
+        ctx.fold = fold
         return Y
 
     @staticmethod
@@ -254,6 +380,11 @@
         o_reads = tuple(O) if batch_axis else (O,)
         params = ctx.params
         P = [params[12 * g:12 * g + 12] for g in range(G)]
+        fold = ctx.fold
+        if fold is not None:
+            fold.begin_backward()
+        out_w = fold.WB if fold is not None else [p[2] for p in P]
+        out_b = fold.eB if fold is not None else [p[3] for p in P]
         R = B * T
         dev = X.device
         col = lambda k: [p[k] for p in P]
@@ -324,15 +455,45 @@
             streams.run_side(w1_grads, reads=(dF1, H1))
         dS1 = torch.empty_like(dS)
         bo_done = ln_bwd(X, A1, dH1, st1, [p[8] for p in P], [p[9] for p in P], dS1,
-                         bias=[p[3] for p in P])
+                         bias=out_b)
         dO = dH1
-        lg.dgrad(sd(dS1), R, E, col(2), sd(dO), cd)
+        lg.dgrad(sd(dS1), R, E, out_w, sd(dO), cd)
 
         def out_proj_grads():
             lg.wgrad(sd(dS1), lg.table(O, E) if batch_axis else lg.strided(O, E, R * E), R, E,
-                     col(2), cd, None if bo_done else col(3), intact=late)
+                     out_w, cd, None if bo_done else out_b, intact=late)
 
         streams.run_side(out_proj_grads, reads=(dS1,) + o_reads)
+        if fold is not None:
+            dQp = torch.empty(G, B, T, E, dtype=cd, device=dev)
+            Tk = torch.empty(G, B, T, E, dtype=cd, device=dev)
+            tsf = Tk.view(G * B, T, E).permute(1, 0, 2)
+            attn_backward(asaved, dO.view(G * B, T, E).permute(1, 0, 2),
+                          dQp.view(G * B, T, E).permute(1, 0, 2), tsf, tsf,
+                          qshare=(B, list(range(G))))
+            streams.wait_side()
+            eye = _identity(E, cd, dev)
+            blk = lambda t, g: (t, g * R * E)
+            a = lg.ksegs([[blk(dQp, g), blk(Tk, g)] for g in range(G)], E, E)
+            b = lg.ksegs([[weight_as(fold.WA[g], cd), eye] for g in range(G)], E, E)
+            dX = torch.empty_like(dS1) if late else dS1
+            cin = None
+            if late and ops.auto_splits(R, E, 2 * E, G, ops.dt(cd)) > 1:
+                ops.copy2d(dS1.data_ptr(), ops.dt(dS1), dX.data_ptr(), ops.dt(dX), G * R, E, E, 1,
+                           E, 1)
+            elif late:
+                cin = [dS1.data_ptr()]
+            ops.gemm(M=R, N=E, K=2 * E, ab_dtype=ops.dt(cd), c_dtype=ops.dt(cd), a_kmajor=True,
+                     b_kmajor=False, batch0=G, beta=1.0, c_in=cin, ldcin=E if cin else 0,
+                     device=dev, **a.args("a"), **b.args("b"), **sd(dX).args("c"))
+
+            def in_proj_grads():
+                lg.wgrad(sd(dQp), sd(X), R, E, fold.WA, cd, fold.cA, intact=late)
+
+            streams.run_side(in_proj_grads, reads=(dQp, X))
+            fold.after_weight_grads(late)
+            ctx.state = ctx.fold = None
+            return (dX, None) + (None,) * len(params)
         dQKV = torch.empty(G, B, T, 3 * E, dtype=cd, device=dev)
         if batch_axis:
             for g in range(G):
diff --git a/joint-multimodal-transformer-6th-abaw_amd/jmt/ops.py b/joint-multimodal-transformer-6th-abaw_amd/jmt/ops.py
--- a/joint-multimodal-transformer-6th-abaw_amd/jmt/ops.py
+++ b/joint-multimodal-transformer-6th-abaw_amd/jmt/ops.py
@@ -541,6 +541,58 @@
                       float((N - nq) * H) * Lq * dh * es}, launch)
 
 
+def attn_kt_ok(dtype, N, H, Lq, Lk, dh, ldp, sk_l, npair, kgroups) -> bool:
+    return bool(_lib.load().jmt_attn_kt_ok(dtype, N, H, Lq, Lk, dh, ldp, sk_l, npair, kgroups))
+
+
+def attn_fwd_kt(dtype, N, H, Lq, Lk, dh, q_ptr, sq, k_ptr, sk, o_ptr, so, scale, lse, spp, qtab,
+                ktab, kgroups):
+    tab, npair = _qtab(qtab)
+    ktb, _ = _qtab(ktab)
+    launch = lambda: _lib.call("jmt_attn_fwd_kt", dtype, N, H, Lq, Lk, dh, q_ptr, sq[0], sq[1],
+                               k_ptr, sk[0], sk[1], o_ptr, so[0], so[1], scale,
+                               lse.data_ptr() if lse is not None else None, spp, tab, ktb, npair,
+                               kgroups, stream())
+    es = 2
+    _hooked({"family": "attn_fwd", "flops": 4.0 * N * H * Lq * Lk * dh, "shared_q": True,
+             "key_table": True,
+             "bytes": float(N * H) * ((2 * Lq + Lk) * dh * es + 4 * Lq)}, launch)
+
+
+def attn_bwd_kt(dtype, N, H, Lq, Lk, dh, go_ptr, sgo, o_ptr, so, q_ptr, sq, k_ptr, sk, lse, p, ds,
+                ldp, scale, spp, qtab, ktab, kgroups):
+    tab, npair = _qtab(qtab)
+    ktb, _ = _qtab(ktab)
+    launch = lambda: _lib.call("jmt_attn_bwd_kt", dtype, N, H, Lq, Lk, dh, go_ptr, sgo[0],
+                               sgo[1], o_ptr, so[0], so[1], q_ptr, sq[0], sq[1], k_ptr, sk[0],
+                               sk[1], lse.data_ptr(), p.data_ptr(), ds.data_ptr(), ldp, scale,
+                               spp, tab, ktb, npair, kgroups, stream())
+    es = 2
+    lw = -(-Lk // 32) * 32
+    _hooked({"family": "attn_bwd", "flops": 4.0 * N * H * Lq * Lk * dh, "shared_q": True,
+             "key_table": True,
+             "bytes": float(N * H) * ((3 * Lq + Lk) * dh * es + 4 * Lq + 2 * Lq * lw * es)},
+            launch)
+
+
+def attn_dkdv_kt(dtype, N, H, Lq, Lk, dh, p, ds, ldp, go_ptr, sgo, q_ptr, sq, t_ptr, st, k_ptr,
+                 sk, dq_ptr, sdq, spp, qtab, ktab, kgroups, merge_dq):
+    tab, npair = _qtab(qtab)
+    ktb, _ = _qtab(ktab)
+    launch = lambda: _lib.call("jmt_attn_dkdv_kt", dtype, N, H, Lq, Lk, dh, p.data_ptr(),
+                               ds.data_ptr(), ldp, go_ptr, sgo[0], sgo[1], q_ptr, sq[0], sq[1],
+                               k_ptr, sk[0], sk[1], t_ptr, st[0], st[1], dq_ptr, sdq[0], sdq[1],
+                               spp, tab, ktb, npair, kgroups, int(merge_dq), stream())
+    es = 2
+    nq = N // 2 if merge_dq else N
+    extra = (Lk + Lq) * dh * es + Lq * (-(-Lk // 32) * 32) * es
+    _hooked({"family": "attn_dkdv", "flops": 6.0 * N * H * Lq * Lk * dh, "shared_q": True,
+             "key_table": True, "merge_dq": bool(merge_dq),
+             "bytes": float(N * H) * ((2 * Lq + Lk) * dh * es +
+                                      2 * Lq * attn_dkdv_ldp(Lk) * es + extra) -
+                      float((N - nq) * H) * Lq * dh * es}, launch)
+
+
 def attn_short_ok(dtype: int, dh: int, Lq: int, Lk: int) -> bool:
     return (_attn_fused["on"] and _attn_short["on"] and
             bool(_lib.load().jmt_attn_short_supported(dtype, dh, Lq, Lk)))
```

Result: no change. 18060 windows/s, median of 6 (+0.2%).
